# bootphon/abnet3

Measured on AMD Instinct MI355X. Metric: frame-pairs/sec (Siamese train step: fwd both towers + coscos2 + bwd + Adadelta), higher is better.
Workload: dtype f16x2; 1 GPU; C2: SiameseNetwork 40->500x2->100 sigmoid, coscos2(avg=False), Adadelta(0.1), 4096 frame pairs per GPU per step, 40-d N(0,1) frames; pairs_per_gpu=4096, global_pairs=4096, parallelism=dp1, graph_replay=False, dp_gradient_buckets=1

## Files before the change

### abnet3_amd/_lib.py

```python
import ctypes as C
import os

import torch

HERE = os.path.dirname(os.path.abspath(__file__))
LIB_PATH = os.environ.get('ABNET3_HIP_LIB') or os.path.join(HERE, 'lib', 'libabnet3_hip.so')
ABI_VERSION = 20
MAX_LAYERS = 16

ACT = {'none': 0, None: 0, 'sigmoid': 1, 'relu': 2, 'tanh': 3}
LOSS = {'coscos2': 0, 'cosmargin': 1, 'KLLoss': 2}
ACT_SOFTMAX = 4
PRECISION = {'fp32': 0, 'bf16': 1, 'bf16x3': 2, 'f16x2': 3}
OPT = {'sgd': 0, 'adadelta': 1, 'adam': 2, 'adagrad': 3, 'RMSprop': 4}
Y_DTYPE = {torch.int8: 0, torch.int32: 1, torch.int64: 2, torch.float32: 3,
           torch.float64: 4}

_i64, _i32, _f32, _vp = C.c_int64, C.c_int32, C.c_float, C.c_void_p
SYMBOLS = {
    'abn_abi_version': (C.c_int, []),
    'abn_last_error': (C.c_char_p, []),
    'abn_tower_ws_floats': (_i64, [_vp, _i64, _i64]),
    'abn_tower_out_offset': (_i64, [_vp, _i64, _i64]),
    'abn_tower_bwd_scratch_floats': (_i64, [_vp, _i64]),
    'abn_tower_forward': (C.c_int, [_vp, _vp, _vp, _i64, _i64, C.c_int, _vp, _vp]),
    'abn_tower_backward': (C.c_int, [_vp, _vp, _vp, _vp, _i64, _i64, _vp, _vp,
                                      _i64, _vp, _vp]),
    'abn_tower_wpack_floats': (_i64, [_vp]),
    'abn_tower_uses_planes': (C.c_int, [_vp, _i64, _vp, _vp, _vp, C.c_int]),
    'abn_tower_path': (C.c_int, [_vp, _vp, _vp, _i64, _i64, C.c_int, _vp, C.c_int, _vp]),
    'abn_tower_image_offset': (_i64, [_vp, _i64, _i64, C.c_int, C.c_int]),
    'abn_reload_switches': (None, []),
    'abn_rccl_allreduce_f64': (C.c_int, [_vp, _vp, _i64, _vp]),
    'abn_tower_backward_launch': (C.c_int, [_vp, _vp, _vp, _vp, _i64, _i64, _vp, _vp, _i64, C.c_int, _vp]),
    'abn_tower_backward_loss_ws_bytes': (_i64, [_i64]),
    'abn_tower_backward_loss': (C.c_int, [_vp, _vp, _vp, _vp, C.c_int, C.c_int, _f32, C.c_int, _i64, _vp, _vp, _i64, _vp, _vp, _vp, _vp, _vp]),
    'abn_tower_reduce_step': (C.c_int, [_vp, _i64, _vp, _i64, C.c_int, _vp, _vp, _vp, _vp, _i64, _f32, _f32, _f32,
                                         _f32, _i64, _f32, _vp]),
    'abn_linear_forward': (C.c_int, [_vp, _vp, _vp, _i64, _i64, _i64, C.c_int, _vp, _vp]),
    'abn_linear_dgrad': (C.c_int, [_vp, _vp, _i64, _i64, _i64, _vp, C.c_int, _vp, _vp]),
    'abn_linear_wgrad_scratch_floats': (_i64, [_i64, _i64, _i64]),
    'abn_linear_wgrad': (C.c_int, [_vp, _vp, _i64, _i64, _i64, _vp, _vp, _vp, _i64, _vp]),
    'abn_linear_backward': (C.c_int, [_vp, _vp, _vp, _i64, _i64, _i64, C.c_int, _vp, _vp, _vp, _vp, _i64, _vp]),
    'abn_linear_backward_prec': (C.c_int, [_vp, _vp, _vp, _i64, _i64, _i64, C.c_int, C.c_int, _vp, _vp, _vp, _vp, _i64, _vp]),
    'abn_softmax_rows': (C.c_int, [_vp, _i64, _i64, _vp, _vp]),
    'abn_softmax_rows_backward': (C.c_int, [_vp, _vp, _i64, _i64, _vp, _vp]),
    'abn_pair_loss_ws_bytes': (_i64, [_i64]),
    'abn_pair_loss': (C.c_int, [_vp, _vp, _vp, C.c_int, _i64, _i64, C.c_int,
                                 _f32, C.c_int, _vp, _vp, _vp, _vp, _vp]),
    'abn_pair_loss_padded': (C.c_int, [_vp, _vp, _vp, C.c_int, _i64, _i64, C.c_int, _f32, C.c_int, _vp, _vp, _vp, _vp, _vp, _vp, _vp]),
    'abn_pair_loss_dz': (C.c_int, [_vp, _vp, _vp, C.c_int, _i64, _i64, C.c_int, _f32, C.c_int, C.c_int,
                                    _vp, _vp, _vp, _vp, _vp, _vp, _vp]),
    'abn_optimizer_step': (C.c_int, [C.c_int, _vp, _vp, _vp, _vp, _i64, _f32,
                                      _f32, _f32, _f32, _i64, _f32, _vp]),
    'abn_tower_sync_ws_bytes': (_i64, []),
    'abn_oneshot_mail_bytes': (_i64, [_i32, _i64]),
    'abn_allreduce_oneshot': (C.c_int, [_vp, _vp, _i64, _vp]),
    'abn_dtw_ws_bytes': (_i64, [_vp, _vp, _i64, _i64, _i64]),
    'abn_dtw_host_stage_bytes': (_i64, [_vp, _vp, _i64]),
    'abn_dtw_batched': (C.c_int, [_vp, _i64, _vp, _i64, _vp, _vp, _vp, _vp, _i64,
                                   _i64, _vp, _vp, _vp, _i64, _vp, _vp, _i64, _vp,
                                   _i64, _vp]),
    'abn_dtw_batched_overlap': (C.c_int, [_vp, _i64, _vp, _i64, _vp, _vp, _vp, _vp, _i64,
                                           _i64, _vp, _vp, _vp, _i64, _vp, _vp, _i64, _vp,
                                           _i64, _vp, _vp]),
    'abn_dtw_cost_max_n2': (_i64, []),
    'abn_dtw_cost_batched': (C.c_int, [_vp, _i64, _vp, _i64, _vp, _vp, _vp, _vp, _i64, _i64, _vp, _vp, _vp]),
    'abn_kl_tables': (C.c_int, [_vp, _i64, _i64, _f32, _vp, _vp, _vp, _vp]),
    'abn_dtw_cost_kl_batched': (C.c_int, [_vp, _vp, _i64, _vp, _vp, _i64, _vp, _vp, _vp, _vp, _i64, _i64, _vp, _vp, _vp, _vp,
                                           _vp]),
    'abn_abx_score': (C.c_int, [_vp, _i64, _vp, _vp, _vp, _vp, _vp, _i64, _i64, _vp, _vp, _vp, _vp]),
    'abn_cosine_distance': (C.c_int, [_vp, _i64, _vp, _i64, _i64, _vp, _vp, _vp]),
    'abn_cosine_distance_f64': (C.c_int, [_vp, _i64, _vp, _i64, _i64, _vp, _vp, _vp]),
    'abn_arccos_f32': (C.c_int, [_vp, _i64, C.c_int, _vp, _vp]),
    'abn_gather_rows': (C.c_int, [_vp, _vp, _i64, _i64, _vp, _vp]),
    'abn_gather_pairs': (C.c_int, [_vp, _i64, _i64, _vp, _vp, _i64, _i64, _i64, _vp, _i32, _vp, _vp, _vp, _vp]),
    'abn_stack_frames': (C.c_int, [_vp, _i64, _i64, _i32, _vp, _vp]),
    'abn_stack_frames_batched': (C.c_int, [_vp, _vp, _i64, _i64, _i64, _i32, _vp, _vp]),
    'abn_mvn_ws_bytes': (_i64, [_i64, _i64]),
    'abn_mvn_stats': (C.c_int, [_vp, _i64, _i64, C.c_int, _vp, _vp, _vp, _vp]),
    'abn_mvn_apply': (C.c_int, [_vp, _i64, _i64, _vp, _vp, C.c_int, _f32, _vp, _vp]),
    'abn_fbank': (C.c_int, [_vp, C.c_int, _i64, _i32, C.c_double, _i32, _i32,
                             _f32, _vp, _vp, _vp, _i64, _vp, _vp]),
    'abn_fbank_batched': (C.c_int, [_vp, C.c_int, _vp, _vp, _i64, _i32, C.c_double, _i32, _i32,
                                     _f32, _vp, _vp, _vp, _i64, _vp, _vp]),
    'abn_deltas': (C.c_int, [_vp, _i64, _i64, _vp, _vp]),
    'abn_deltas_batched': (C.c_int, [_vp, _i64, _vp, _i64, _i64, _i64, _vp, _i64, _vp]),
    'abn_mfcc': (C.c_int, [_vp, C.c_int, _i64, _i32, C.c_double, _i32, _i32, _i32, _f32, _vp, _vp, _vp, _vp,
                            _i64, _vp, _i64, _vp]),
    'abn_mfcc_batched': (C.c_int, [_vp, C.c_int, _vp, _vp, _i64, _i32, C.c_double, _i32, _i32, _i32, _f32, _vp, _vp,
                                    _vp, _vp, _i64, _vp, _i64, _vp]),
    'abn_mfcc_path': (C.c_int, [_i32, _i32, _i32]),
    'abn_integrate_ws_bytes': (_i64, [_i64]),
    'abn_integrate_forward': (C.c_int, [_vp, _i64, _vp, _i64, _i64, C.c_int, C.c_int, _f32, _f32, _vp, _vp, _vp, _i64,
                                         C.c_int, _vp, _vp, _vp]),
    'abn_integrate_backward': (C.c_int, [_vp, _i64, _vp, _i64, _i64, C.c_int, C.c_int, _f32, _f32, _vp, _vp, _i64,
                                          C.c_int, _vp, _vp, _vp, _vp, _vp, _vp, _vp]),
    'abn_knn_ws_bytes': (_i64, [_i64, _i64, C.c_int]),
    'abn_knn_topk': (C.c_int, [_vp, _i64, _vp, _i64, C.c_int, _vp, _vp, C.c_int, _vp, _vp, _vp, _i64, _vp]),
    'abn_segment_vectors': (C.c_int, [_vp, _i64, _vp, _vp, _i64, C.c_int, _vp, _vp, _vp]),
}
INTEGRATE_MODE = {'sum': 0, 'concat': 1}
W_NONE, W_FIXED, W_SCALAR, W_ATTENTION = range(4)


class TowerDesc(C.Structure):
    _fields_ = [('n_layers', _i32), ('act', _i32), ('last_act', _i32),
                ('batch_norm', _i32), ('dims', _i64 * (MAX_LAYERS + 1))] + [
        (name, _vp * MAX_LAYERS)
        for name in ('W', 'b', 'bn_w', 'bn_b', 'bn_rm', 'bn_rv', 'dW', 'db',
                     'dbn_w', 'dbn_b', 'drop_mask')] + [('precision', _i32), ('d_out_is_dz', _i32), ('defer_reduce', _i32), ('wpack_valid', _i32), ('forward_only', _i32), ('wgrad_part', _i32), ('wpack', _vp), ('drop_seed', _vp), ('drop_p', _f32), ('reserved2_', _i32),
                     ('bn_sync_world', _i32), ('wgrad_split', _i32), ('bn_sync_fn', _vp), ('bn_sync_ctx', _vp), ('n_valid', _vp),
                     ('bn_nbt', _vp * MAX_LAYERS), ('sync_ws', _vp), ('fwd_ws', _vp), ('fwd_calls', _i64), ('source', _vp)]


class StepSource(C.Structure):
    _fields_ = [('table', _vp), ('table_rows', _i64), ('idx1', _vp), ('idx2', _vp), ('labels', _vp), ('steps', _vp), ('step_ctr', _vp)]


class OneShotCtx(C.Structure):
    _fields_ = [('rank', _i32), ('world', _i32), ('mail', _vp * 8), ('cap_floats', _i64)]


class RcclCtx(C.Structure):
    _fields_ = [('comm', _vp), ('all_reduce', _vp), ('calls', _i64)]


ALLREDUCE_FN = C.CFUNCTYPE(C.c_int, C.c_void_p, C.c_void_p, C.c_int64, C.c_void_p)


class HipLibraryError(RuntimeError):
    pass


_lib = None


def load():
    global _lib
    if _lib is not None:
        return _lib
    if not os.path.exists(LIB_PATH):
        raise HipLibraryError(
            'abnet3_amd: %s is missing. Build it with `python -m abnet3_amd.build` '
            '(hipcc, gfx950). There is no CPU fallback.' % LIB_PATH)
    lib = C.CDLL(LIB_PATH)
    for name, (res, args) in SYMBOLS.items():
        try:
            fn = getattr(lib, name)
        except AttributeError:
            raise HipLibraryError('abnet3_amd: %s does not export %s '
                                  '(stale build?)' % (LIB_PATH, name))
        fn.restype = res
        fn.argtypes = args
    if lib.abn_abi_version() != ABI_VERSION:
        raise HipLibraryError('abnet3_amd: ABI version mismatch (library %d, '
                              'binding %d)' % (lib.abn_abi_version(), ABI_VERSION))
    _lib = lib
    return lib


def reload_switches():
    load().abn_reload_switches()


E_ARG = -1
E_WORKSPACE = -3
E_UNSUPPORTED = -4

PATH_PER_LAYER, PATH_FUSED_F32, PATH_PLANES, PATH_PLANES_INFER, PATH_PLANES_INFER_BN, PATH_BN_LAYERS, PATH_WIDE, PATH_BN_TOWER = range(8)
PRECISION_NAMES = {0: 'fp32', 1: 'bf16', 2: 'bf16x3', 3: 'f16x2'}
MFCC_GENERAL, MFCC_WAVE512 = 0, 1

trace_paths = False
last_path = {'forward': -1, 'backward': -1, 'forward_precision': -1, 'backward_precision': -1}


def note_path(desc, x1, x2, rows, n_calls, train, ws, backward):
    if not trace_paths:
        return
    prec = C.c_int32(-1)
    path = load().abn_tower_path(C.byref(desc), ptr(x1), ptr(x2), rows, n_calls, int(train), ptr(ws), int(backward),
                                 C.byref(prec))
    key = 'backward' if backward else 'forward'
    last_path[key] = path
    last_path[key + '_precision'] = prec.value


def last_forward_path():
    return last_path['forward']


def last_backward_path():
    return last_path['backward']


_ON_ERROR = []


def check(rc, what):
    if rc != 0:
        for hook in _ON_ERROR:
            hook()
        msg = load().abn_last_error()
        raise HipLibraryError('%s failed (%d): %s' % (
            what, rc, msg.decode('utf-8', 'replace') if msg else ''))


def require_device(*tensors):
    for t in tensors:
        if t is None:
            continue
        if not t.is_cuda:
            raise HipLibraryError(
                'abnet3_amd: expected a tensor on the MI355X (HIP) device, got '
                'device=%s. The accelerated path has no CPU fallback; move the '
                'module and its inputs to the GPU (.cuda()).' % t.device)
        if not t.is_contiguous():
            raise HipLibraryError('abnet3_amd: tensor must be contiguous')


def ptr(t):
    return C.c_void_p(t.data_ptr()) if t is not None else C.c_void_p(0)


def stream():
    return C.c_void_p(torch.cuda.current_stream().cuda_stream)
```

### abnet3_amd/csrc/tower.hip

```cpp
#include <stdarg.h>
#include <stdlib.h>
#include <string.h>

#include <math.h>
#include <atomic>

#include "common.h"
#include "gemm_f32.h"
#include "opt_rule.h"
#include "tower_fused.h"
#include "tower_planes.h"
#include "tower_bn_persist.h"
#include "tower_wide.h"
#include "tower_wgrad_step.h"

namespace abn {

static thread_local char g_err[512] = "";
void set_error(const char* fmt, ...)
{
    va_list ap;
    va_start(ap, fmt);
    vsnprintf(g_err, sizeof(g_err), fmt, ap);
    va_end(ap);
}

static Switches read_switches()
{
    auto off = [](const char* name) { const char* v = getenv(name); return v && atoi(v) == 0; };
    Switches s;
    s.planes = !off("ABN_PLANES");
    s.fused = !off("ABN_FUSED");
    s.fused_min_rows = getenv("ABN_FUSED_MIN_ROWS") ? atoll(getenv("ABN_FUSED_MIN_ROWS")) : -1;
    s.bn_planes = !off("ABN_BN_PLANES");
    s.bn_persist = !off("ABN_BN_PERSIST");
    s.wgrad_xcd = !off("ABN_WGRAD_XCD");
    s.bf16x3_planes = !off("ABN_BF16X3_PLANES");
    s.bwd_pair = !off("ABN_BWD_PAIR");
    s.gemm_tile = getenv("ABN_GEMM_TILE") ? atoi(getenv("ABN_GEMM_TILE")) : -1;
    s.wgrad_rows_per_slab = getenv("ABN_WGRAD_ROWS_PER_SLAB") ? atoll(getenv("ABN_WGRAD_ROWS_PER_SLAB")) : -1;
    s.wide = !off("ABN_WIDE");
    s.wide_max_rows = getenv("ABN_WIDE_MAX_ROWS") ? atoll(getenv("ABN_WIDE_MAX_ROWS")) : -1;
    s.wide_max_groups = getenv("ABN_WIDE_MAXG") ? atoi(getenv("ABN_WIDE_MAXG")) : WD_MAXG;
    if (s.wide_max_groups < 1 || s.wide_max_groups > WD_MAXG) s.wide_max_groups = WD_MAXG;
    s.dtw_f40 = !off("ABN_DTW_F40");
    s.dtw_pc = !off("ABN_DTW_PC");
    s.wgrad_wgs_heavy = getenv("ABN_WGRAD_WGS_HEAVY") ? atoi(getenv("ABN_WGRAD_WGS_HEAVY")) : 128;
    s.wgrad_wgs_light = getenv("ABN_WGRAD_WGS_LIGHT") ? atoi(getenv("ABN_WGRAD_WGS_LIGHT")) : 128;
    s.wgrad_tile128 = getenv("ABN_WGRAD_TILE128") ? atoi(getenv("ABN_WGRAD_TILE128")) : -1;
    s.dtw_wgs_per_cu = getenv("ABN_DTW_WGS") ? atoi(getenv("ABN_DTW_WGS")) : 6;
    if (s.dtw_wgs_per_cu < 1 || s.dtw_wgs_per_cu > 9) s.dtw_wgs_per_cu = 6;
    s.wgrad_step = !off("ABN_WGRAD_STEP");
    s.dtw_dealt = !off("ABN_DTW_SCHED");
    s.oneshot_wgs = getenv("ABN_ONESHOT_WGS") ? atoi(getenv("ABN_ONESHOT_WGS")) : 32;
    if (s.oneshot_wgs < 1 || s.oneshot_wgs > 256) s.oneshot_wgs = 32;
    s.knn_split = getenv("ABN_KNN_SPLIT") ? atoi(getenv("ABN_KNN_SPLIT")) : 0;
    if (s.knn_split < 0) s.knn_split = 0;
    return s;
}
static Switches g_switches = read_switches();
const Switches& switches() { return g_switches; }
void reload_switches() { g_switches = read_switches(); }

template <int BM, int BN, bool A_KC, bool B_KC, int EPI, bool VEC, int BF16>
static void launch_one(const GemmP& p, int splits, hipStream_t st)
{
    const int tiles = ((p.M + BM - 1) / BM) * ((p.N + BN - 1) / BN);
    constexpr size_t lds = BF16 == 3 ? gemm_lds_bytes3<BM, BN>() : gemm_lds_bytes<BM, BN, A_KC, B_KC>();
    auto k = gemm_f32_kernel<BM, BN, A_KC, B_KC, EPI, VEC, BF16>;
    static bool attr_set[16] = {};
    int dev = 0;
    (void)hipGetDevice(&dev);
    dev = (dev >= 0 && dev < 16) ? dev : 0;
    if (!attr_set[dev]) {
        (void)hipFuncSetAttribute(reinterpret_cast<const void*>(k),
                                  hipFuncAttributeMaxDynamicSharedMemorySize, (int)lds);
        attr_set[dev] = true;
    }
    GemmP q = p;
    q.splits = splits;
    hipLaunchKernelGGL(k, dim3(tiles * splits), dim3(256), lds, st, q);
}

template <int BM, int BN, bool A_KC, bool B_KC, int EPI>
static void launch_cfg(const GemmP& p, int splits, hipStream_t st)
{
    if (p.bf16 == 1) {
        if (p.a_vec && p.b_vec) launch_one<BM, BN, A_KC, B_KC, EPI, true, 1>(p, splits, st);
        else launch_one<BM, BN, A_KC, B_KC, EPI, false, 1>(p, splits, st);
        return;
    }
    if (p.bf16 == 2) {
        const bool planes = switches().bf16x3_planes;
        if (p.a_vec && p.b_vec && planes) launch_one<BM, BN, A_KC, B_KC, EPI, true, 3>(p, splits, st);
        else if (p.a_vec && p.b_vec) launch_one<BM, BN, A_KC, B_KC, EPI, true, 2>(p, splits, st);
        else launch_one<BM, BN, A_KC, B_KC, EPI, false, 2>(p, splits, st);
        return;
    }
    if (p.a_vec && p.b_vec) launch_one<BM, BN, A_KC, B_KC, EPI, true, 0>(p, splits, st);
    else launch_one<BM, BN, A_KC, B_KC, EPI, false, 0>(p, splits, st);
}

template <bool A_KC, bool B_KC, int EPI>
static int prepare_gemm(GemmP& p, int splits)
{
    if (p.M <= 0 || p.N <= 0) return -1;
    if (p.K <= 0) { set_error("gemm: empty reduction"); return -100 + ABN_E_ARG; }
    {
        const int64_t span_a = (int64_t)(A_KC ? p.M : p.K) * p.lda, span_b = (int64_t)(B_KC ? p.N : p.K) * p.ldb;
        if (span_a >= (1LL << 31) || span_b >= (1LL << 31)) { set_error("gemm: operand larger than 2^31 floats"); return -100 + ABN_E_ARG; }
    }
    auto tiles = [&](int bm, int bn) {
        return (int64_t)((p.M + bm - 1) / bm) * ((p.N + bn - 1) / bn) * splits;
    };
    const int64_t want = 2 * 256;
    {
        const bool slab_ok = (EPI != EPI_WGRAD) || (p.slab_stride % 4 == 0);
        p.c_vec = aligned16(p.C) && (p.ldc % 4 == 0) && slab_ok && (!p.bias || aligned16(p.bias)) &&
                  (!p.aux || (aligned16(p.aux) && p.ldaux % 4 == 0)) &&
                  (!p.mask || (aligned16(p.mask) && (EPI == EPI_DGRAD ? p.ldaux : p.ldc) % 4 == 0));
    }
    p.splits = splits;
#ifdef ABN_STAMPS
    p.stamps = getenv("ABN_STAMP_BUF") ? (unsigned long long*)strtoull(getenv("ABN_STAMP_BUF"), nullptr, 0) : nullptr;
#endif
    const int force = switches().gemm_tile;
    if (force >= 0 && force <= 3) return force;
    const int64_t pad_a = (int64_t)((p.M + 127) / 128 * 128) * ((p.N + 63) / 64 * 64);
    const int64_t pad_b = (int64_t)((p.M + 63) / 64 * 64) * ((p.N + 127) / 128 * 128);
    if (p.M > 64 && p.N > 64 && tiles(128, 128) >= want) return 0;
    if (p.M > 64 && tiles(128, 64) >= want && (pad_a <= pad_b || !(p.N > 64 && tiles(64, 128) >= want))) return 1;
    if (p.N > 64 && tiles(64, 128) >= want) return 2;
    return 3;
}

template <bool A_KC, bool B_KC, int EPI>
static int launch_gemm(GemmP p, int splits, hipStream_t st)
{
    const int tile = prepare_gemm<A_KC, B_KC, EPI>(p, splits);
    if (tile == -1) return ABN_OK;
    if (tile < -1) return tile + 100;
    if (tile == 0) launch_cfg<128, 128, A_KC, B_KC, EPI>(p, splits, st);
    else if (tile == 1) launch_cfg<128, 64, A_KC, B_KC, EPI>(p, splits, st);
    else if (tile == 2) launch_cfg<64, 128, A_KC, B_KC, EPI>(p, splits, st);
    else launch_cfg<64, 64, A_KC, B_KC, EPI>(p, splits, st);
    ABN_CHECK_LAUNCH("gemm_f32");
    return ABN_OK;
}

static bool bf16x3_planes()
{
    return switches().bf16x3_planes;
}

template <int WM, int WN, int BF16>
static void launch_pair_one(const GemmP& pw, int n0, const GemmP& pd, int n1, hipStream_t st)
{
    constexpr size_t lw = BF16 == 3 ? gemm_lds_bytes3<WM, WN>() : gemm_lds_bytes<WM, WN, false, false>();
    constexpr size_t ld = BF16 == 3 ? gemm_lds_bytes3<128, 64>() : gemm_lds_bytes<128, 64, true, false>();
    constexpr size_t lds = lw > ld ? lw : ld;
    auto k = gemm_bwd_pair_kernel<WM, WN, BF16>;
    static bool attr_set[16] = {};
    int dev = 0;
    (void)hipGetDevice(&dev);
// ... 1043 lines not shown
{
    const int nl = t->n_layers;
    const int np = planes_of(t);
    const int64_t rpc = rows / n_calls;
    ABN_REQUIRE(aligned16(d_out) && aligned16(scratch) && (!dx || aligned16(dx)), "tower_backward: d_out / scratch / dx must be 16-byte aligned");
    ABN_REQUIRE(!t->d_out_is_dz || loss, "tower_backward: d_out_is_dz cannot be combined with batch_norm");
    ABN_REQUIRE(!loss || n_calls == 2, "tower_backward_loss: two forward_once calls");
    BwdLayout B = B0;
    for (int l = 0; l < nl; ++l) B.splits[l] = B0.psplits[l];
    const PackLayout PL = make_pack_layout(t);
    const char* const image = t->wpack ? reinterpret_cast<const char*>(t->wpack) : reinterpret_cast<const char*>(ws + L.wpack);
    static bool attr_set[16] = {};
    int dev = 0;
    (void)hipGetDevice(&dev);
    dev = (dev >= 0 && dev < 16) ? dev : 0;
    if (!attr_set[dev]) {
        PL_LDS_ATTR(bn_bwd_layer_kernel, pl_lds_bytes);
        PL_LDS_ATTR(wgrad_planes_kernel, wgrad_lds_of);
        attr_set[dev] = true;
    }
    const int wgs_per_call = (int)bn_wgs_per_call(rows, n_calls);
    const dim3 cgrid((unsigned)(n_calls * wgs_per_call));
    const int64_t tp_steps = 2 * n_calls * wgs_per_call;
    float* const part = scratch + B.bn_wg;
    float* const s1 = scratch + B.bn_s1, * const s2 = scratch + B.bn_s2;
    const bool sync = bn_sync_on(t);
    ABN_REQUIRE(!sync || t->bn_sync_fn, "tower_backward: bn_sync_world = %d without bn_sync_fn", t->bn_sync_world);
    ABN_REQUIRE(!loss || !loss->n_valid || !t->n_valid || loss->n_valid == t->n_valid, "tower_backward_loss: two different n_valid");
    const int32_t* const nvp = t->n_valid ? t->n_valid : (loss ? loss->n_valid : nullptr);
    if (sync && nvp) { set_error("tower_backward: n_valid (a padded batch) cannot be combined with cross-replica BatchNorm statistics"); return ABN_E_UNSUPPORTED; }
    double* const sums = reinterpret_cast<double*>(scratch + B.bn_part);
    auto finish_sums = [&](int C, float* dgamma, float* dbeta) -> int {
        hipLaunchKernelGGL(bn_bwd_finish_wg_kernel, dim3((unsigned)((C + 63) / 64)), dim3(64 * BN_WG_GROUPS), 0, st, part, wgs_per_call, C,
                           (int)n_calls, s1, s2, dgamma, dbeta, sync ? sums : static_cast<double*>(nullptr));
        if (!sync) return ABN_OK;
        if (t->bn_sync_fn(t->bn_sync_ctx, sums, n_calls * 2 * C, st) != 0) { set_error("tower_backward: bn_sync_fn failed"); return ABN_E_LAUNCH; }
        hipLaunchKernelGGL(bn_bwd_from_sums_kernel, dim3(grid_for(n_calls * C)), dim3(256), 0, st, sums, C, (int)n_calls, s1, s2);
        return ABN_OK;
    };
    if (bn_persist_path(t, rows, n_calls)) {
        static bool bt_attr_set[16] = {};
        if (!bt_attr_set[dev]) {
            PL_LDS_ATTR(bn_bwd_tower_kernel, bnp_lds_bytes);
            bt_attr_set[dev] = true;
        }
        BnBwdTowerP q = {};
        q.n_layers = nl; q.rows = (int)rows; q.rows_call = (int)rpc; q.n_calls = (int)n_calls;
        for (int l = 0; l <= nl; ++l) q.dims[l] = (int)t->dims[l];
        for (int l = 0; l < nl; ++l) {
            q.act[l] = (l == nl - 1) ? t->last_act : t->act;
            q.z[l] = ws + L.xhat[l];
            q.mean[l] = ws + L.mean[l]; q.invstd[l] = ws + L.invstd[l];
            q.gamma[l] = t->bn_w[l]; q.beta[l] = t->bn_b[l];
            q.dgamma[l] = t->dbn_w[l]; q.dbeta[l] = t->dbn_b[l];
            q.mask[l] = t->drop_mask[l];
            q.wpt[l] = image + PL.wpt[l];
            q.dzp[l] = reinterpret_cast<char*>(scratch + B.dzp[l]);
            q.amax_dz[l] = B.amax_dz[l] >= 0 ? scratch + B.amax_dz[l] : nullptr;
        }
        q.drop_seed = reinterpret_cast<const unsigned long long*>(t->drop_seed);
        q.drop_p = t->drop_p;
        q.wbase = image; q.wbytes = PL.bytes;
        q.tp_steps = tp_steps;
        q.dx = dx;
        q.d_out = loss ? nullptr : d_out;
        q.a_top = ws + L.a[nl - 1];
        q.sync_ws = t->sync_ws;
        q.sync_bytes = bnp_sync_bytes(BNP_MAX_WGS);
        q.n_valid = nvp;
        q.n_stat = (float)rpc;
        q.loss_kind = -1;
        if (loss) {
            q.loss_kind = loss->kind; q.y = loss->y; q.y_dtype = loss->y_dtype;
            q.margin = (double)loss->margin;
            q.scale = loss->avg ? 1.0 / (double)rpc : 1.0;
            q.loss_counter = reinterpret_cast<unsigned*>(loss->ws);
            q.loss_partial = reinterpret_cast<double*>(reinterpret_cast<char*>(loss->ws) + 8);
            q.loss_out = loss->loss_out;
            q.loss_accum = loss->loss_accum;
        }
        PL_LAUNCH(np, bn_bwd_tower_kernel, cgrid, dim3(PL_NT), bnp_lds_bytes(np), st, q);
    } else {
    const float* da_top = d_out;
    {
        const int N = (int)t->dims[nl];
        BnLossP lp = {};
        lp.n_valid = nvp;
        if (loss) {
            lp.y = loss->y; lp.y_dtype = loss->y_dtype; lp.kind = loss->kind; lp.B = (int)rpc;
            lp.margin = (double)loss->margin;
            lp.scale = loss->avg ? 1.0 / (double)rpc : 1.0;
            lp.loss_counter = reinterpret_cast<unsigned*>(loss->ws);
            lp.loss_partial = reinterpret_cast<double*>(reinterpret_cast<char*>(loss->ws) + 8);
            lp.loss_out = loss->loss_out;
            lp.loss_accum = loss->loss_accum;
            lp.a_top = ws + L.a[nl - 1];
            lp.da_out = scratch + B.dz[0];
            da_top = lp.da_out;
            hipLaunchKernelGGL(bn_bwd_sums_wg_kernel<true>, cgrid, dim3(512), 0, st, static_cast<const float*>(nullptr), ws + L.xhat[nl - 1],
                               ws + L.mean[nl - 1], ws + L.invstd[nl - 1], t->bn_w[nl - 1], t->bn_b[nl - 1], t->last_act, N, rpc, part, lp);
        } else {
            hipLaunchKernelGGL(bn_bwd_sums_wg_kernel<false>, cgrid, dim3(512), 0, st, d_out, ws + L.xhat[nl - 1], ws + L.mean[nl - 1],
                               ws + L.invstd[nl - 1], t->bn_w[nl - 1], t->bn_b[nl - 1], t->last_act, N, rpc, part, lp);
        }
        const int rc = finish_sums(N, t->dbn_w[nl - 1], t->dbn_b[nl - 1]);
        if (rc != ABN_OK) return rc;
    }
    int cur = 0;
    for (int l = nl - 1; l >= 0; --l) {
        BnBwdP q = {};
        q.l = l; q.rows = (int)rows; q.rows_call = (int)rpc;
        q.n_stat = (float)rpc;
        q.n_stat_dev = sync ? ws + L.bn_nstat + 8 * l : nullptr;
        q.N = (int)t->dims[l + 1]; q.K = (int)t->dims[l];
        q.act_l = (l == nl - 1) ? t->last_act : t->act;
        q.act_prev = t->act;
        q.da = (l == nl - 1) ? da_top : scratch + B.dz[cur];
        q.z = ws + L.xhat[l];
        q.mean = ws + L.mean[l];
        q.invstd = ws + L.invstd[l];
        q.gamma = t->bn_w[l]; q.beta = t->bn_b[l];
        q.s1 = s1; q.s2 = s2;
        q.mask = t->drop_mask[l];
        q.drop_seed = reinterpret_cast<const unsigned long long*>(t->drop_seed);
        q.drop_p = t->drop_p;
        q.dzp = reinterpret_cast<char*>(scratch + B.dzp[l]);
        q.amax_dz = B.amax_dz[l] >= 0 ? scratch + B.amax_dz[l] : nullptr;
        q.tp_steps = tp_steps;
        q.wpt = (l >= 1 || dx) ? image + PL.wpt[l] : nullptr;
        q.da_prev = l >= 1 ? scratch + B.dz[cur ^ 1] : dx;
        if (l >= 1) { q.z_prev = ws + L.xhat[l - 1]; q.mean_prev = ws + L.mean[l - 1]; q.invstd_prev = ws + L.invstd[l - 1];
                      q.gamma_prev = t->bn_w[l - 1]; q.beta_prev = t->bn_b[l - 1]; q.part_out = part; }
        q.n_valid = nvp;
        PL_LAUNCH(np, bn_bwd_layer_kernel, cgrid, dim3(PL_NT), pl_lds_bytes(np), st, q);
        if (l >= 1) {
            const int rc = finish_sums(q.K, t->dbn_w[l - 1], t->dbn_b[l - 1]);
            if (rc != ABN_OK) return rc;
            cur ^= 1;
        }
    }
    }
    int n_wg = 0;
    WgradP w = make_wgrad(t, rows, L, B, ws, scratch, &n_wg);
    w.tp_steps = tp_steps;
    launch_wgrad(np, w, n_wg, st);
    ABN_CHECK_LAUNCH("tower_backward (BatchNorm, planes)");
    if (t->defer_reduce) return ABN_OK;
    const ReduceTable rt = make_reduce_table(t, B);
    hipLaunchKernelGGL(slab_reduce_kernel, dim3(grid_for((rt.total + 3) / 4)), dim3(256), 0, st, scratch + B.slabs, rt);
    ABN_CHECK_LAUNCH("slab_reduce");
    return ABN_OK;
}

enum { PLANES_BWD_ALL = 0, PLANES_BWD_DGRAD = 1, PLANES_BWD_WGRAD = 2 };
static int planes_backward(const abn_tower_desc* t, const float* d_out, const LossArgs* loss, int64_t rows, const Layout& L,
                           const BwdLayout& B, const float* ws, float* scratch, float* dx, hipStream_t st, int part = PLANES_BWD_ALL)
{
    const int nl = t->n_layers;
    const int np = planes_of(t);
    PlanesBwdP b = {};
#ifdef ABN_STAMPS
    b.stamps = getenv("ABN_DSTAMP_BUF") ? (unsigned long long*)strtoull(getenv("ABN_DSTAMP_BUF"), nullptr, 0) : nullptr;
#endif
    b.n_layers = nl;
    b.rows = (int)rows;
    b.d_out = d_out;
    b.d_out_is_dz = t->d_out_is_dz;
    b.tp_steps = pl_row_steps(rows);
    ABN_REQUIRE((loss || t->wgrad_part == 2 || aligned16(d_out)) && aligned16(scratch) && (!dx || aligned16(dx)),
                "tower_backward: d_out / scratch / dx must be 16-byte aligned");
    b.loss_kind = -1;
    b.B = (int)rows;
    if (loss) {
        b.loss_kind = loss->kind;
        b.y = loss->y; b.y_dtype = loss->y_dtype;
        b.B = (int)(rows / 2);
        b.margin = (double)loss->margin;
        b.scale = loss->avg ? 1.0 / (double)(rows / 2) : 1.0;
        b.loss_counter = reinterpret_cast<unsigned*>(loss->ws);
        b.loss_partial = reinterpret_cast<double*>(reinterpret_cast<char*>(loss->ws) + 8);
        b.loss_out = loss->loss_out;
        b.n_valid = loss->n_valid;
        b.loss_accum = loss->loss_accum;
    }
    b.a_top = ws + L.a[nl - 1];
    b.dx = dx;
    b.drop_seed = reinterpret_cast<const unsigned long long*>(t->drop_seed);
    b.drop_p = t->drop_p;
    const PackLayout PL = make_pack_layout(t);
    const char* const image = t->wpack ? reinterpret_cast<const char*>(t->wpack) : reinterpret_cast<const char*>(ws + L.wpack);
    for (int l = 0; l <= nl; ++l) b.dims[l] = (int)t->dims[l];
    for (int l = 0; l < nl; ++l) {
        b.act[l] = (l == nl - 1) ? t->last_act : t->act;
        b.tp[l] = reinterpret_cast<const char*>(ws + L.tp[l]);
        b.mask[l] = t->drop_mask[l];
        b.wpt[l] = image + PL.wpt[l];
        b.dzp[l] = reinterpret_cast<char*>(scratch + B.dzp[l]);
        b.amax_dz[l] = B.amax_dz[l] >= 0 ? scratch + B.amax_dz[l] : nullptr;
    }
    b.wbase = image; b.wbytes = PL.bytes;
    int l_first, l_end;
    { const int rc = wgrad_range(t, &l_first, &l_end); if (rc != ABN_OK) return rc; }
    if (t->wgrad_part == 2) part = PLANES_BWD_WGRAD;
    int n_wg = 0;
    const WgradP w = make_wgrad(t, rows, L, B, ws, scratch, &n_wg, l_first, l_end);
    static bool bw_attr_set[16] = {};
    int dev = 0;
    (void)hipGetDevice(&dev);
    dev = (dev >= 0 && dev < 16) ? dev : 0;
    if (!bw_attr_set[dev]) {
        PL_LDS_ATTR(tower_dgrad_planes_kernel, pl_lds_bytes);
        PL_LDS_ATTR(wgrad_planes_kernel, wgrad_lds_of);
        bw_attr_set[dev] = true;
    }
    const dim3 cgrid((unsigned)((rows + PL_ROWS - 1) / PL_ROWS));
    const bool do_dgrad = part != PLANES_BWD_WGRAD, do_wgrad = part != PLANES_BWD_DGRAD;
    if (do_dgrad) PL_LAUNCH(np, tower_dgrad_planes_kernel, cgrid, dim3(PL_NT), pl_lds_bytes(np), st, b);
    if (do_wgrad && n_wg > 0) launch_wgrad(np, w, n_wg, st);
    ABN_CHECK_LAUNCH("tower_backward (planes)");
    if (t->defer_reduce) return ABN_OK;
    ReduceTable rt = make_reduce_table(t, B);
    reduce_range(rt, t, B, l_first, l_end);
    if (rt.total > rt.begin)
        hipLaunchKernelGGL(slab_reduce_kernel, dim3(grid_for((rt.total - rt.begin + 3) / 4)), dim3(256), 0, st, scratch + B.slabs, rt);
    ABN_CHECK_LAUNCH("slab_reduce");
    return ABN_OK;
}

static bool wgrad_step_small_ok(const abn_tower_desc* t, int64_t rows, int64_t n_calls)
{
    if (!switches().wgrad_step || !t->defer_reduce || !t->fwd_ws || t->batch_norm || t->wgrad_part != 0 || planes_of(t) != 2) return false;
    if (n_calls < 1 || rows % n_calls != 0 || !aligned16(t->fwd_ws)) return false;
    const int64_t vrows = bn_vrows(rows, n_calls);
    if (wide_groups_for(t, vrows) <= 0 || !planes_shape_ok(t)) return false;
    return vrows <= 2048;
}

static int wide_backward(const abn_tower_desc* t, const float* d_out, const LossArgs* loss, int64_t rows, int64_t n_calls,
                         const Layout& L, const BwdLayout& B, const float* ws, float* scratch, float* dx, hipStream_t st)
{
    const int nl = t->n_layers, top = nl - 1;
    const int np = planes_of(t);
    ABN_REQUIRE((loss || t->wgrad_part == 2 || aligned16(d_out)) && aligned16(scratch) && (!dx || aligned16(dx)),
                "tower_backward: d_out / scratch / dx must be 16-byte aligned");
    ABN_REQUIRE(!loss || n_calls == 2, "tower_backward_loss: two forward_once calls");
    const PackLayout PL = make_pack_layout(t);
    const char* const image = t->wpack ? reinterpret_cast<const char*>(t->wpack) : reinterpret_cast<const char*>(ws + L.wpack);
    static bool attr_set[16] = {};
    int dev = 0;
    (void)hipGetDevice(&dev);
    dev = (dev >= 0 && dev < 16) ? dev : 0;
    if (!attr_set[dev]) {
        PL_LDS_ATTR(wide_dgrad_layer_kernel, wd_lds_bytes);
        PL_LDS_ATTR(wgrad_planes_kernel, wgrad_lds_of);
        attr_set[dev] = true;
    }
    const int64_t rpc = rows / n_calls;
    const int64_t wpc = bn_wgs_per_call(rows, n_calls), nrb = n_calls * wpc;
    const int G = wide_groups_for(t, nrb * PL_ROWS);
    ABN_REQUIRE(G > 0, "tower_backward: too many rows for the layer-per-launch kernels");
    int l_first, l_end;
    { const int rc = wgrad_range(t, &l_first, &l_end); if (rc != ABN_OK) return rc; }
    const int last = dx ? 0 : 1;
    int cur = 0;
    for (int l = top; (l >= last || l == top) && t->wgrad_part != 2; --l) {
        WideBwdP q = {};
        q.l = l; q.top = top;
        q.N = (int)t->dims[l + 1]; q.K = (int)t->dims[l];
        q.act_prev = t->act;
        q.rows_call = (int)rpc; q.n_calls = (int)n_calls; q.wpc = (int)wpc;
        const int nblk = pl_blocks(q.K);
        q.G = G < nblk ? G : nblk;
        q.dz_in = l < top ? scratch + B.dz[cur] : nullptr;
        q.wpt = (l >= 1 || dx) ? image + PL.wpt[l] : nullptr;
        q.a_prev = l >= 1 ? ws + L.a[l - 1] : nullptr;
        q.dz_out = (l >= 1 && l - 1 >= last) ? scratch + B.dz[cur ^ 1] : nullptr;
        q.dzp_top = reinterpret_cast<char*>(scratch + B.dzp[top]);
        q.dzp_out = l >= 1 ? reinterpret_cast<char*>(scratch + B.dzp[l - 1]) : nullptr;
        if (np == 2) { q.amax_top = scratch + B.amax_dz[top]; q.amax_out = l >= 1 ? scratch + B.amax_dz[l - 1] : nullptr; }
        q.tp_steps = 2 * nrb;
        q.dx = dx;
        q.drop_seed = reinterpret_cast<const unsigned long long*>(t->drop_seed);
        q.drop_p = t->drop_p;
        if (l == top) {
            q.d_out = loss ? nullptr : d_out;
            q.d_out_is_dz = t->d_out_is_dz;
            q.a_top = ws + L.a[top];
            q.act_top = t->last_act;
            if (loss) {
                q.loss_kind = loss->kind; q.y_dtype = loss->y_dtype; q.y = loss->y;
                q.margin = (double)loss->margin;
                q.scale = loss->avg ? 1.0 / (double)rpc : 1.0;
                q.loss_counter = reinterpret_cast<unsigned*>(loss->ws);
                q.loss_partial = reinterpret_cast<double*>(reinterpret_cast<char*>(loss->ws) + 8);
                q.loss_out = loss->loss_out;
                q.n_valid = loss->n_valid;
                q.loss_accum = loss->loss_accum;
                if (t->source) {
                    q.y = t->source->labels;
                    q.g_steps = t->source->steps; q.g_ctr = t->source->step_ctr;
                }
            }
        }
        const dim3 grid((unsigned)(nrb * q.G));
        PL_LAUNCH(np, wide_dgrad_layer_kernel, grid, dim3(PL_NT), wd_lds_bytes(np), st, q);
        if (l < top || q.dz_out) cur ^= (q.dz_out ? 1 : 0);
        if (l == 0) break;
    }
    if (wgrad_step_small_ok(t, rows, n_calls)) {
        ABN_REQUIRE(t->fwd_ws == ws && t->fwd_calls == n_calls, "tower_backward: abn_tower_desc.fwd_ws / fwd_calls are not this call's");
        ABN_CHECK_LAUNCH("tower_backward (layer per launch)");
        return ABN_OK;
    }
    int n_wg = 0;
    WgradP w = make_wgrad(t, rows, L, B, ws, scratch, &n_wg, l_first, l_end);
    w.tp_steps = 2 * nrb;
    if (n_wg > 0) launch_wgrad(np, w, n_wg, st);
    ABN_CHECK_LAUNCH("tower_backward (layer per launch)");
    if (t->defer_reduce) return ABN_OK;
    ReduceTable rt = make_reduce_table(t, B);
    reduce_range(rt, t, B, l_first, l_end);
    if (rt.total > rt.begin)
        hipLaunchKernelGGL(slab_reduce_kernel, dim3(grid_for((rt.total - rt.begin + 3) / 4)), dim3(256), 0, st, scratch + B.slabs, rt);
    ABN_CHECK_LAUNCH("slab_reduce");
    return ABN_OK;
}

}

using namespace abn;

extern "C" {

int abn_abi_version(void) { return ABN_ABI_VERSION; }
const char* abn_last_error(void) { return abn::g_err; }

int64_t abn_tower_ws_floats(const abn_tower_desc* t, int64_t rows, int64_t n_calls)
{
    if (check_desc(t, rows, n_calls) != ABN_OK) return -1;
    return make_layout(t, rows, n_calls).total;
}

int64_t abn_tower_out_offset(const abn_tower_desc* t, int64_t rows, int64_t n_calls)
{
    if (check_desc(t, rows, n_calls) != ABN_OK) return -1;
    return make_layout(t, rows, n_calls).a[t->n_layers - 1];
}

int64_t abn_tower_image_offset(const abn_tower_desc* t, int64_t rows, int64_t n_calls, int which, int l)
{
    if (check_desc(t, rows, n_calls) != ABN_OK || l < 0 || l >= t->n_layers) return -1;
    if (which == 3) return make_bwd_layout(t, rows).dzp[l];
    const Layout L = make_layout(t, rows, n_calls);
    if (which == 2) return L.tp[l];
    if (which == 4) return L.xhat[l];
    if (which == 5) return L.a[l];
    if (which != 0 && which != 1) return -1;
    const PackLayout P = make_pack_layout(t);
    return (t->wpack ? 0 : L.wpack) + (which == 0 ? P.wp[l] : P.wpt[l]) / 4;
}

static bool fused_f32_ok(const abn_tower_desc* t, const float* x1, const float* x2, int64_t rows, int train, const float* ws)
{
    const int64_t fused_min_rows = switches().fused_min_rows >= 0 ? switches().fused_min_rows : 6144;
    bool fusable = switches().fused && rows >= fused_min_rows && !t->batch_norm && aligned16(x1) && (!x2 || aligned16(x2)) &&
                   aligned16(ws);
    for (int l = 0; l <= t->n_layers && fusable; ++l)
        fusable = t->dims[l] >= 4 && t->dims[l] <= FUSED_MAXW && t->dims[l] % 4 == 0;
    for (int l = 0; l < t->n_layers && fusable; ++l)
        fusable = aligned16(t->W[l]) && (!t->drop_mask[l] || !train || aligned16(t->drop_mask[l]));
    return fusable;
}
static int forward_path(const abn_tower_desc* t, const float* x1, const float* x2, int64_t rows, int64_t n_calls, int train,
                        const float* ws)
{
    const bool bn_train = train && bn_train_planes_path(t, rows, n_calls, x1, x2, ws);
    const int kind = planes_kind(t, rows, n_calls, x1, x2, ws, train ? PLANES_TRAIN : PLANES_EVAL_FORWARD);
    if (!bn_train && kind == PLANES_WIDE) return ABN_PATH_WIDE;
    if (bn_train) return bn_persist_path(t, rows, n_calls) ? ABN_PATH_BN_TOWER : ABN_PATH_BN_LAYERS;
    if (kind != PLANES_NONE) {
        if (t->batch_norm) return ABN_PATH_PLANES_INFER_BN;
        return (t->forward_only && !(train && t->drop_seed) && !train) ? ABN_PATH_PLANES_INFER : ABN_PATH_PLANES;
    }
    return fused_f32_ok(t, x1, x2, rows, train, ws) ? ABN_PATH_FUSED_F32 : ABN_PATH_PER_LAYER;
}
static int backward_path(const abn_tower_desc* t, const float* x1, const float* x2, int64_t rows, int64_t n_calls, const float* ws)
{
    const int kind = planes_kind(t, rows, n_calls, x1, x2, ws);
    if (kind == PLANES_WIDE) return ABN_PATH_WIDE;
    if (kind == PLANES_CHAIN) return ABN_PATH_PLANES;
    if (bn_train_planes_path(t, rows, n_calls, x1, x2, ws)) return bn_persist_path(t, rows, n_calls) ? ABN_PATH_BN_TOWER : ABN_PATH_BN_LAYERS;
    return ABN_PATH_PER_LAYER;
}

int abn_tower_path(const abn_tower_desc* t, const float* x1, const float* x2, int64_t rows, int64_t n_calls, int train,
                   const float* ws, int backward, int32_t* precision_out)
{
    if (check_desc(t, rows, n_calls) != ABN_OK) return -1;
    const int path = backward ? backward_path(t, x1, x2, rows, n_calls, ws) : forward_path(t, x1, x2, rows, n_calls, train, ws);
    if (precision_out) *precision_out = (path == ABN_PATH_PER_LAYER || path == ABN_PATH_FUSED_F32) ? gemm_prec(t->precision) : t->precision;
    return path;
}

int abn_tower_uses_planes(const abn_tower_desc* t, int64_t rows, const float* x1, const float* x2, const float* ws, int train)
{
    if (check_desc(t, rows, 1) != ABN_OK) return -1;
    if (train && t->batch_norm) return bn_train_planes_path(t, rows, 1, x1, x2, ws) ? 1 : 0;
    return planes_path(t, rows, x1, x2, ws, train ? PLANES_TRAIN : PLANES_EVAL_FORWARD) ? 1 : 0;
}

int64_t abn_tower_sync_ws_bytes(void) { return bnp_sync_bytes(BNP_MAX_WGS); }

int64_t abn_tower_wpack_floats(const abn_tower_desc* t)
{
    if (check_desc(t, 0, 1) != ABN_OK) return -1;
    return make_pack_layout(t).bytes / 4;
}

int64_t abn_tower_bwd_scratch_floats(const abn_tower_desc* t, int64_t rows)
{
    if (check_desc(t, rows, 1) != ABN_OK) return -1;
    return make_bwd_layout(t, rows).total;
}

int abn_tower_forward(const abn_tower_desc* t, const float* x1, const float* x2, int64_t rows,
                      int64_t n_calls, int train, float* ws, void* stream)
{
    int rc = check_desc(t, rows, n_calls);
    if (rc != ABN_OK) return rc;
    ABN_REQUIRE(x1 && ws, "tower_forward: null input/workspace");
    ABN_REQUIRE(x2 == nullptr || n_calls == 2, "tower_forward: x2 given but n_calls=%lld", (long long)n_calls);
    ABN_REQUIRE(n_calls <= 8, "tower_forward: at most 8 calls per launch");
    if (rows == 0) return ABN_OK;
    hipStream_t st = (hipStream_t)stream;
    const Layout L = make_layout(t, rows, n_calls);
    const int64_t rpc = rows / n_calls;

    const int path = forward_path(t, x1, x2, rows, n_calls, train, ws);
    const bool fusable = path == ABN_PATH_FUSED_F32;
    const int pmode = train ? PLANES_TRAIN : PLANES_EVAL_FORWARD;
    const bool bn_train = train && bn_train_planes_path(t, rows, n_calls, x1, x2, ws);
    if (train && t->batch_norm && bn_sync_on(t) && !bn_train) {
        set_error("tower_forward: cross-replica BatchNorm statistics (bn_sync_world) need the operand-plane launches");
        return ABN_E_UNSUPPORTED;
    }
    if (train && t->batch_norm && t->n_valid && !bn_train) {
        set_error("tower_forward: a padded batch (n_valid) through a BatchNorm tower in training needs the BatchNorm layer launches");
        return ABN_E_UNSUPPORTED;
    }
    const int kind = planes_kind(t, rows, n_calls, x1, x2, ws, pmode);
    if (t->source && !(train && !bn_train && kind == PLANES_WIDE && n_calls == 2 && x2 && !t->forward_only)) {
        set_error("tower_forward: a step source (abn_tower_desc.source) needs the layer-per-launch kernels in training, two calls");
        return ABN_E_UNSUPPORTED;
    }
    if (t->source) ABN_REQUIRE(t->source->table && t->source->idx1 && t->source->idx2 && t->source->steps && t->source->step_ctr &&
                                   aligned16(t->source->table) && t->dims[0] % 4 == 0,
                               "tower_forward: abn_step_source: null or misaligned array");
    if (t->drop_seed && train && !bn_train && kind == PLANES_NONE) {
        for (int l = 0; l < t->n_layers; ++l)
            if (!t->drop_mask[l]) { set_error("tower_forward: in-kernel dropout (drop_seed) needs the operand-plane kernels: pass drop_mask tensors"); return ABN_E_UNSUPPORTED; }
    }
    if (bn_train || kind != PLANES_NONE) {
        const int np = planes_of(t);
        PackTable pk = {};
        PlanesFwdP f = {};
        f.n_layers = t->n_layers;
        f.rows = (int)rows;
        f.rows_call = (int)rpc;
        f.x1 = x1; f.x2 = x2;
        f.x_copy = nullptr;
        const PackLayout PL = make_pack_layout(t);
        char* const image = t->wpack ? reinterpret_cast<char*>(t->wpack) : reinterpret_cast<char*>(ws + L.wpack);
        const bool repack = !(t->wpack && t->wpack_valid);
        ABN_REQUIRE(aligned16(image), "tower_forward: wpack must be 16-byte aligned");
        pk.base = image;
        f.wbase = image; f.wbytes = PL.bytes;
        for (int l = 0; l <= t->n_layers; ++l) f.dims[l] = (int)t->dims[l];
        for (int l = 0; l < t->n_layers; ++l) {
            f.act[l] = (l == t->n_layers - 1) ? t->last_act : t->act;
            f.b[l] = t->b[l];
            f.mask[l] = train ? t->drop_mask[l] : nullptr;
            f.out[l] = l == t->n_layers - 1 ? ws + L.a[l] : nullptr;
            f.wp[l] = image + PL.wp[l];
            PackJob& J = pk.job[pk.n_jobs++];
            J.W = t->W[l]; J.N = (int)t->dims[l + 1]; J.K = (int)t->dims[l]; J.transposed = 0;
            J.nblk = pl_blocks(J.N); J.nsteps = pl_steps(J.K);
            J.tile0 = pk.n_tiles; J.dst = PL.wp[l];
            J.blk0 = pk.n_blocks;
            pk.n_tiles += J.nblk * J.nsteps;
            pk.n_blocks += J.nblk;
            {
                PackJob& T = pk.job[pk.n_jobs++];
                T.W = t->W[l]; T.N = J.N; T.K = J.K; T.transposed = 1;
                T.nblk = pl_blocks(T.K); T.nsteps = pl_steps(T.N);
                T.tile0 = pk.n_tiles; T.dst = PL.wpt[l];
                T.blk0 = pk.n_blocks;
                pk.n_tiles += T.nblk * T.nsteps;
                pk.n_blocks += T.nblk;
            }
            f.tp[l] = (t->forward_only || t->batch_norm) ? nullptr : reinterpret_cast<char*>(ws + L.tp[l]);
            f.amax[l] = f.tp[l] && L.amax[l] >= 0 ? ws + L.amax[l] : nullptr;
            if (t->batch_norm) { f.bn_rm[l] = t->bn_rm[l]; f.bn_rv[l] = t->bn_rv[l]; f.bn_w[l] = t->bn_w[l]; f.bn_b[l] = t->bn_b[l]; }
        }
        f.tp_steps = pl_row_steps(rows);
        f.drop_seed = train ? reinterpret_cast<const unsigned long long*>(t->drop_seed) : nullptr;
        f.drop_p = t->drop_p;
        f.bn_eps = BN_EPS;
#ifdef ABN_STAMPS
        f.stamps = getenv("ABN_STAMP_BUF") ? (unsigned long long*)strtoull(getenv("ABN_STAMP_BUF"), nullptr, 0) : nullptr;
#endif
        static bool pl_attr_set[16] = {};
        int dev = 0;
        (void)hipGetDevice(&dev);
        dev = (dev >= 0 && dev < 16) ? dev : 0;
        const dim3 pgrid((unsigned)((pk.n_tiles + 3) / 4));
        const dim3 fgrid((unsigned)((rows + PL_ROWS - 1) / PL_ROWS));
        if (repack) {
            if (np == 3) hipLaunchKernelGGL(pack_planes_kernel<3>, pgrid, dim3(256), 0, st, pk);
            else if (np == 2) hipLaunchKernelGGL(pack_planes_scaled_kernel, dim3((unsigned)pk.n_blocks), dim3(PL_NT), 0, st, pk);
            else hipLaunchKernelGGL(pack_planes_kernel<1>, pgrid, dim3(256), 0, st, pk);
        }
        if (!bn_train && kind == PLANES_WIDE) {
            static bool wd_attr_set[16] = {};
            if (!wd_attr_set[dev]) {
                PL_LDS_ATTR(wide_fwd_layer_kernel, wd_lds_bytes);
                wd_attr_set[dev] = true;
            }
            const int nl = t->n_layers;
            const int64_t wpc = bn_wgs_per_call(rows, n_calls), nrb = n_calls * wpc;
            const int G = wide_groups_for(t, nrb * PL_ROWS);
            const bool keep = !t->forward_only;
            for (int l = 0; l < nl; ++l) {
                WideFwdP q = {};
                q.l = l; q.last = l == nl - 1;
                q.K = (int)t->dims[l]; q.N = (int)t->dims[l + 1];
                q.act = f.act[l];
                q.rows_call = (int)rpc; q.n_calls = (int)n_calls; q.wpc = (int)wpc;
                const int nblk = pl_blocks(q.N);
                q.G = G < nblk ? G : nblk;
                q.x1 = x1; q.x2 = x2;
                q.a_prev = l >= 1 ? ws + L.a[l - 1] : nullptr;
                q.wp = f.wp[l];
                q.b = t->b[l];
                q.a_out = q.last ? nullptr : ws + L.a[l];
                q.out = q.last ? ws + L.a[l] : nullptr;
                q.tp_in = keep && l == 0 ? reinterpret_cast<char*>(ws + L.tp[0]) : nullptr;
                q.tp_out = keep && !q.last ? reinterpret_cast<char*>(ws + L.tp[l + 1]) : nullptr;
                if (np == 2 && keep) { q.amax_in = ws + L.amax[0]; q.amax_out = q.last ? nullptr : ws + L.amax[l + 1]; }
                q.tp_steps = 2 * nrb;
                q.drop_seed = f.drop_seed; q.drop_p = f.drop_p;
                if (t->source && l == 0) {
                    q.g_table = t->source->table; q.g_rows = t->source->table_rows;
                    q.g_idx1 = t->source->idx1; q.g_idx2 = t->source->idx2;
                    q.g_steps = t->source->steps; q.g_ctr = t->source->step_ctr;
                }
#ifdef ABN_STAMPS
                q.stamps = getenv("ABN_STAMP_BUF") ? (unsigned long long*)strtoull(getenv("ABN_STAMP_BUF"), nullptr, 0) : nullptr;
#endif
                const dim3 wgrid((unsigned)(nrb * q.G));
                PL_LAUNCH(np, wide_fwd_layer_kernel, wgrid, dim3(PL_NT), wd_lds_bytes(np), st, q);
            }
            ABN_CHECK_LAUNCH("tower_forward (layer per launch)");
            return ABN_OK;
        }
        if (bn_train) {
            static bool bn_attr_set[16] = {};
            if (!bn_attr_set[dev]) {
                PL_LDS_ATTR(bn_fwd_layer_kernel, pl_lds_bytes);
                bn_attr_set[dev] = true;
            }
            f.bn_part = ws + L.bn_wg;
            const int nl = t->n_layers;
            const int64_t wpc = bn_wgs_per_call(rows, n_calls);
            const dim3 bgrid((unsigned)(n_calls * wpc));
            f.tp_steps = 2 * n_calls * wpc;
            if (bn_persist_path(t, rows, n_calls)) {
                static bool bt_attr_set[16] = {};
                if (!bt_attr_set[dev]) {
                    PL_LDS_ATTR(bn_fwd_tower_kernel, bnp_lds_bytes);
                    bt_attr_set[dev] = true;
                }
                PlanesFwdP fl = f;
                BnPersistP q = {};
                for (int l = 0; l < nl; ++l) {
                    fl.tp[l] = reinterpret_cast<char*>(ws + L.tp[l]);
                    fl.amax[l] = L.amax[l] >= 0 ? ws + L.amax[l] : nullptr;
                    fl.out[l] = nullptr;
                    q.z[l] = ws + L.xhat[l];
                    q.mean[l] = ws + L.mean[l]; q.invstd[l] = ws + L.invstd[l]; q.var[l] = ws + L.var[l];
                    q.rm[l] = t->bn_rm[l]; q.rv[l] = t->bn_rv[l];
                    q.nbt[l] = reinterpret_cast<long long*>(t->bn_nbt[l]);
                }
                q.sync_ws = t->sync_ws;
                q.sync_bytes = bnp_sync_bytes(BNP_MAX_WGS);
                q.n_valid = t->n_valid;
                q.n_calls = (int)n_calls;
                q.a_top = ws + L.a[nl - 1];
                PL_LAUNCH(np, bn_fwd_tower_kernel, bgrid, dim3(PL_NT), bnp_lds_bytes(np), st, fl, q);
                ABN_CHECK_LAUNCH("tower_forward (BatchNorm, resident tower)");
                return ABN_OK;
            }
            for (int l = 0; l < nl; ++l) {
                PlanesFwdP fl = f;
                for (int i = 0; i < nl; ++i) { fl.tp[i] = nullptr; fl.out[i] = nullptr; }
                fl.tp[l] = reinterpret_cast<char*>(ws + L.tp[l]);
                fl.amax[l] = L.amax[l] >= 0 ? ws + L.amax[l] : nullptr;
                fl.act[l] = ACT_NONE;
                fl.out[l] = ws + L.xhat[l];
                BnTrainP q = {};
                q.l = l;
                if (l > 0) { q.mean = ws + L.mean[l - 1]; q.invstd = ws + L.invstd[l - 1]; q.z_prev = ws + L.xhat[l - 1]; q.a_prev = nullptr; }
                q.n_valid = t->n_valid;
                PL_LAUNCH(np, bn_fwd_layer_kernel, bgrid, dim3(PL_NT), pl_lds_bytes(np), st, fl, q);
                const int N = (int)t->dims[l + 1];
                const bool sync = bn_sync_on(t);
                ABN_REQUIRE(!sync || t->bn_sync_fn, "tower_forward: bn_sync_world = %d without bn_sync_fn", t->bn_sync_world);
                if (sync && t->n_valid) { set_error("tower_forward: n_valid (a padded batch) cannot be combined with cross-replica BatchNorm statistics"); return ABN_E_UNSUPPORTED; }
                double* const sums = reinterpret_cast<double*>(ws + L.bn_part);
                hipLaunchKernelGGL(bn_stats_finish_wg_kernel, dim3((unsigned)((N + 63) / 64)), dim3(64 * BN_WG_GROUPS), 0, st, ws + L.bn_wg,
                                   (int)wpc, rpc, N, (int)n_calls, ws + L.mean[l], ws + L.invstd[l], ws + L.var[l],
                                   t->bn_rm[l], t->bn_rv[l], sync ? sums : static_cast<double*>(nullptr), t->n_valid);
                if (sync) {
                    if (t->bn_sync_fn(t->bn_sync_ctx, sums, n_calls * 2 * N + n_calls, st) != 0) { set_error("tower_forward: bn_sync_fn failed"); return ABN_E_LAUNCH; }
                    hipLaunchKernelGGL(bn_stats_from_sums_kernel, dim3((unsigned)((N + 255) / 256)), dim3(256), 0, st, sums,
                                       N, (int)n_calls, ws + L.mean[l], ws + L.invstd[l], ws + L.var[l],
                                       t->bn_rm[l], t->bn_rv[l], ws + L.bn_nstat + 8 * l);
                }
            }
            const int N = (int)t->dims[nl];
            const float* z = ws + L.xhat[nl - 1];
            hipLaunchKernelGGL(bn_apply_kernel, dim3(grid_for(rows * N)), dim3(256), 0, st, z, rows, rpc, N, ws + L.mean[nl - 1],
                               ws + L.invstd[nl - 1], t->bn_rm[nl - 1], t->bn_rv[nl - 1], 1, t->bn_w[nl - 1], t->bn_b[nl - 1],
                               t->last_act, static_cast<float*>(nullptr), ws + L.a[nl - 1], t->n_valid);
            launch_nbt(t, n_calls, st);
            ABN_CHECK_LAUNCH("tower_forward (BatchNorm, planes)");
            return ABN_OK;
        }
        const bool infer = t->batch_norm || (t->forward_only && !f.drop_seed && !train);
        const int mode = t->batch_norm ? PL_INFER_BN : infer ? PL_INFER : PL_TRAIN;
        const size_t lds = t->batch_norm ? pl_lds_bytes_bn(np) : pl_lds_bytes_stag(np);
        const void* kernels[3][3] = {
            {reinterpret_cast<const void*>(tower_fwd_planes_kernel<1, PL_TRAIN>), reinterpret_cast<const void*>(tower_fwd_planes_kernel<1, PL_INFER>),
             reinterpret_cast<const void*>(tower_fwd_planes_kernel<1, PL_INFER_BN>)},
            {reinterpret_cast<const void*>(tower_fwd_planes_kernel<2, PL_TRAIN>), reinterpret_cast<const void*>(tower_fwd_planes_kernel<2, PL_INFER>),
             reinterpret_cast<const void*>(tower_fwd_planes_kernel<2, PL_INFER_BN>)},
            {reinterpret_cast<const void*>(tower_fwd_planes_kernel<3, PL_TRAIN>), reinterpret_cast<const void*>(tower_fwd_planes_kernel<3, PL_INFER>),
             reinterpret_cast<const void*>(tower_fwd_planes_kernel<3, PL_INFER_BN>)}};
        if (!pl_attr_set[dev]) {
            for (int a = 0; a < 3; ++a)
                for (int m = 0; m < 3; ++m)
                    if (kernels[a][m])
                        (void)hipFuncSetAttribute(kernels[a][m], hipFuncAttributeMaxDynamicSharedMemorySize,
                                                  (int)(m == PL_INFER_BN ? pl_lds_bytes_bn(a + 1) : pl_lds_bytes_stag(a + 1)));
            pl_attr_set[dev] = true;
        }
        void* kargs[] = {&f};
        (void)hipLaunchKernel(kernels[np - 1][mode], fgrid, dim3(PL_NT), kargs, lds, st);
        ABN_CHECK_LAUNCH("tower_fwd_planes");
        return ABN_OK;
    }
    if (fusable) {
        FusedFwdP f = {};
        f.n_layers = t->n_layers;
        f.rows = (int)rows;
        f.rows_call = (int)rpc;
        f.bf16 = gemm_prec(t->precision);
        f.x1 = x1; f.x2 = x2;
        f.x_copy = x2 ? ws + L.x : nullptr;
        for (int l = 0; l <= t->n_layers; ++l) f.dims[l] = (int)t->dims[l];
        for (int l = 0; l < t->n_layers; ++l) {
            f.act[l] = (l == t->n_layers - 1) ? t->last_act : t->act;
            f.W[l] = t->W[l]; f.b[l] = t->b[l];
            f.mask[l] = train ? t->drop_mask[l] : nullptr;
            f.out[l] = ws + L.a[l];
// ... 125 lines not shown
        const int N = (int)t->dims[nl];
        const float* a = ws + L.a[nl - 1];
        float* dz = scratch + B.dz[cur];
        if (t->d_out_is_dz) {
            ABN_REQUIRE(!t->batch_norm, "tower_backward: d_out_is_dz cannot be combined with batch_norm");
            dz_in = d_out;
        } else if (!t->batch_norm) {
            hipLaunchKernelGGL(act_bwd_kernel, dim3(grid_for(rows * N)), dim3(256), 0, st, a, d_out,
                               t->drop_mask[nl - 1], dz, rows * N, t->last_act);
        } else {
            const int nch = bn_chunks(rpc);
            double* part = reinterpret_cast<double*>(scratch + B.bn_part);
            hipLaunchKernelGGL(bn_partial_kernel<true>, dim3((N + 63) / 64, nch, (int)n_calls), dim3(256), 0, st, d_out, a,
                               ws + L.xhat[nl - 1], rpc, N, bn_chunk_rows(rpc), t->last_act, part);
            hipLaunchKernelGGL(bn_bwd_finish_kernel, dim3((unsigned)((n_calls * N + 63) / 64)), dim3(64), 0, st, part,
                               nch, N, (int)n_calls, scratch + B.bn_s1, scratch + B.bn_s2);
            hipLaunchKernelGGL(bn_bwd_apply_kernel, dim3(grid_for(rows * N)), dim3(256), 0, st, a, d_out,
                               ws + L.xhat[nl - 1], rows, rpc, N, t->last_act, t->bn_w[nl - 1],
                               ws + L.invstd[nl - 1], scratch + B.bn_s1, scratch + B.bn_s2, (int)n_calls,
                               t->drop_mask[nl - 1], dz, t->dbn_w[nl - 1], t->dbn_b[nl - 1]);
        }
        ABN_CHECK_LAUNCH("output-layer dz");
    }

    float* slabs = scratch + B.slabs;
    for (int l = nl - 1; l >= 0; --l) {
        const int Kin = (int)t->dims[l], Nout = (int)t->dims[l + 1];
        const float* dz = (l == nl - 1 && dz_in) ? dz_in : scratch + B.dz[cur];
        const float* a_in = (l == 0) ? xin : ws + L.a[l - 1];
        GemmP pw = {};
        pw.A = dz; pw.lda = Nout;
        pw.B = a_in; pw.ldb = Kin;
        pw.C = slabs + B.off[l]; pw.ldc = Kin;
        pw.C2 = slabs + B.off[l] + (int64_t)Nout * Kin;
        pw.slab_stride = B.slab_stride;
        pw.M = Nout; pw.N = Kin + 1; pw.K = (int)rows;
        pw.k_chunk = (int)align_up((rows + B.splits[l] - 1) / B.splits[l], BK);
        pw.ones_col = Kin;
        pw.bf16 = gemm_prec(t->precision);
        pw.a_vec = aligned16(dz) && (Nout % 4 == 0);
        pw.b_vec = aligned16(a_in) && (Kin % 4 == 0);
        if (!(l > 0 || dx)) {
            rc = launch_gemm<false, false, EPI_WGRAD>(pw, B.splits[l], st);
            if (rc != ABN_OK) return rc;
        }
        if (l > 0 || dx) {
            float* dst = (l == 0) ? dx : scratch + B.dz[cur ^ 1];
            GemmP p = {};
            p.A = dz; p.lda = Nout;
            p.B = t->W[l]; p.ldb = Kin;
            p.C = dst; p.ldc = Kin;
            p.M = (int)rows; p.N = Kin; p.K = Nout; p.k_chunk = Nout;
            p.a_vec = aligned16(dz) && (Nout % 4 == 0);
            p.b_vec = aligned16(t->W[l]) && (Kin % 4 == 0);
            p.ones_col = -1;
            p.bf16 = gemm_prec(t->precision);
            if (l > 0 && !t->batch_norm) { p.aux = ws + L.a[l - 1]; p.ldaux = Kin; p.act = t->act; p.mask = t->drop_mask[l - 1]; }
            rc = launch_bwd_pair(pw, B.splits[l], p, st);
            if (rc != ABN_OK) return rc;
            if (l > 0 && t->batch_norm) {
                const float* a = ws + L.a[l - 1];
                const int nch = bn_chunks(rpc);
                double* part = reinterpret_cast<double*>(scratch + B.bn_part);
                hipLaunchKernelGGL(bn_partial_kernel<true>, dim3((Kin + 63) / 64, nch, (int)n_calls), dim3(256), 0, st,
                                   dst, a, ws + L.xhat[l - 1], rpc, Kin, bn_chunk_rows(rpc), t->act, part);
                hipLaunchKernelGGL(bn_bwd_finish_kernel, dim3((unsigned)((n_calls * Kin + 63) / 64)), dim3(64), 0, st,
                                   part, nch, Kin, (int)n_calls, scratch + B.bn_s1, scratch + B.bn_s2);
                hipLaunchKernelGGL(bn_bwd_apply_kernel, dim3(grid_for(rows * Kin)), dim3(256), 0, st, a, dst,
                                   ws + L.xhat[l - 1], rows, rpc, Kin, t->act, t->bn_w[l - 1], ws + L.invstd[l - 1],
                                   scratch + B.bn_s1, scratch + B.bn_s2, (int)n_calls, t->drop_mask[l - 1], dst,
                                   t->dbn_w[l - 1], t->dbn_b[l - 1]);
                ABN_CHECK_LAUNCH("batch_norm backward");
            }
            cur ^= 1;
        }
    }
    if (t->defer_reduce) return ABN_OK;
    const ReduceTable rt = make_reduce_table(t, B);
    hipLaunchKernelGGL(slab_reduce_kernel, dim3(grid_for((rt.total + 3) / 4)), dim3(256), 0, st, slabs, rt);
    ABN_CHECK_LAUNCH("slab_reduce");
    return ABN_OK;
}

int abn_tower_backward_launch(const abn_tower_desc* t, const float* x1, const float* x2, const float* d_out,
                                  int64_t rows, int64_t n_calls, const float* ws, float* scratch,
                                  int64_t scratch_floats, int part, void* stream)
{
    int rc = check_desc(t, rows, n_calls);
    if (rc != ABN_OK) return rc;
    ABN_REQUIRE(x1 && d_out && ws && scratch && (part == PLANES_BWD_DGRAD || part == PLANES_BWD_WGRAD), "tower_backward_launch: bad argument");
    if (rows == 0 || planes_kind(t, rows, n_calls, x1, x2, ws) != PLANES_CHAIN) { set_error("tower_backward_launch: single-launch operand-plane towers only"); return ABN_E_UNSUPPORTED; }
    const Layout L = make_layout(t, rows, n_calls);
    const BwdLayout B = make_bwd_layout(t, rows);
    if (scratch_floats < B.total) { set_error("tower_backward_launch: scratch too small"); return ABN_E_WORKSPACE; }
    abn_tower_desc u = *t;
    u.defer_reduce = 1;
    return planes_backward(&u, d_out, nullptr, rows, L, B, ws, scratch, nullptr, (hipStream_t)stream, part);
}

void abn_reload_switches(void) { abn::reload_switches(); }

int abn_rccl_allreduce_f64(void* ctx, void* device_doubles, int64_t n, void* stream)
{
    typedef int (*all_reduce_t)(const void*, void*, size_t, int, int, void*, hipStream_t);
    abn_rccl_ctx* c = static_cast<abn_rccl_ctx*>(ctx);
    if (!c || !c->comm || !c->all_reduce || !device_doubles || n < 0) { set_error("rccl_allreduce_f64: null context / buffer"); return 1; }
    constexpr int NCCL_FLOAT64 = 8, NCCL_SUM = 0;
    const int rc = reinterpret_cast<all_reduce_t>(c->all_reduce)(device_doubles, device_doubles, (size_t)n, NCCL_FLOAT64, NCCL_SUM, c->comm,
                                                                  (hipStream_t)stream);
    if (rc != 0) { set_error("rccl_allreduce_f64: ncclAllReduce returned %d", rc); return 1; }
    ++c->calls;
    return 0;
}

int64_t abn_tower_backward_loss_ws_bytes(int64_t rows) { return 8 + ((rows + PL_ROWS - 1) / PL_ROWS + 2) * (int64_t)sizeof(double); }

int abn_tower_backward_loss(const abn_tower_desc* t, const float* x1, const float* x2, const void* y, int y_dtype,
                            int loss_kind, float margin, int avg, int64_t rows, const float* ws, float* scratch,
                            int64_t scratch_floats, float* loss_out, void* loss_ws, const int32_t* n_valid, double* loss_accum,
                            void* stream)
{
    if (loss_kind == ABN_LOSS_KL) {
        set_error("tower_backward_loss: ABN_LOSS_KL is not computed inside the backward: use abn_pair_loss_dz + abn_tower_backward");
        return ABN_E_UNSUPPORTED;
    }
    int rc = check_desc(t, rows, 2);
    if (rc != ABN_OK) return rc;
    ABN_REQUIRE(x1 && y && ws && scratch && loss_out && loss_ws, "tower_backward_loss: null pointer");
    ABN_REQUIRE(loss_kind == ABN_LOSS_COSCOS2 || loss_kind == ABN_LOSS_COSMARGIN, "tower_backward_loss: unknown loss kind %d", loss_kind);
    ABN_REQUIRE(y_dtype >= ABN_Y_I8 && y_dtype <= ABN_Y_F64, "tower_backward_loss: unknown label dtype %d", y_dtype);
    ABN_REQUIRE(loss_kind != ABN_LOSS_COSMARGIN || (margin >= 0.0f && margin <= 1.0f), "tower_backward_loss: margin outside [0,1]");
    for (int l = 0; l < t->n_layers; ++l) ABN_REQUIRE(t->dW[l] && t->db[l], "tower_backward_loss: layer %d has null gradient buffers", l);
    const bool bn = rows > 0 && t->batch_norm && bn_train_planes_path(t, rows, 2, x1, x2, ws) && !bn_sync_on(t) && t->wgrad_part == 0 &&
                    t->dims[t->n_layers] % 4 == 0;
    const int kind = rows == 0 || t->batch_norm ? PLANES_NONE : planes_kind(t, rows, 2, x1, x2, ws);
    if (kind == PLANES_NONE && !bn) {
        set_error("tower_backward_loss: only for towers the operand-plane kernels take (the split arithmetics, "
                  "widths <= 512 and multiples of 4, enough rows; BatchNorm without cross-replica statistics): use abn_pair_loss_dz + abn_tower_backward");
        return ABN_E_UNSUPPORTED;
    }
    if (t->source && (kind != PLANES_WIDE || bn || !t->source->labels)) {
        set_error("tower_backward_loss: a step source (abn_tower_desc.source) needs the layer-per-launch kernels and its labels");
        return ABN_E_UNSUPPORTED;
    }
    const Layout L = make_layout(t, rows, 2);
    const BwdLayout B = make_bwd_layout(t, rows);
    if (scratch_floats < B.total) { set_error("tower_backward_loss: scratch too small"); return ABN_E_WORKSPACE; }
    LossArgs la = {y, y_dtype, loss_kind, avg, margin, loss_out, loss_ws, n_valid, loss_accum};
    if (bn) return bn_planes_backward(t, nullptr, &la, rows, 2, L, B, ws, scratch, nullptr, (hipStream_t)stream);
    if (kind == PLANES_WIDE) return wide_backward(t, nullptr, &la, rows, 2, L, B, ws, scratch, nullptr, (hipStream_t)stream);
    return planes_backward(t, nullptr, &la, rows, L, B, ws, scratch, nullptr, (hipStream_t)stream);
}

int abn_tower_reduce_step(const abn_tower_desc* t, int64_t rows, const float* scratch, int64_t scratch_floats, int kind,
                          float* params, float* grads, float* state1, float* state2, int64_t n, float lr, float hp0,
                          float hp1, float eps, int64_t step, float grad_scale, void* stream)
{
    int rc = check_desc(t, rows, 1);
    if (rc != ABN_OK) return rc;
    ABN_REQUIRE(kind >= ABN_OPT_SGD && kind <= ABN_OPT_RMSPROP, "tower_reduce_step: unknown optimizer %d", kind);
    ABN_REQUIRE(scratch && params && grads && state1, "tower_reduce_step: null pointer");
    ABN_REQUIRE(state2 || (kind != ABN_OPT_ADADELTA && kind != ABN_OPT_ADAM), "tower_reduce_step: state2 required");
    ABN_REQUIRE(step >= 1 && n >= 1, "tower_reduce_step: bad n/step");
    const BwdLayout B = make_bwd_layout(t, rows);
    if (scratch_floats < B.total) { set_error("tower_reduce_step: scratch too small"); return ABN_E_WORKSPACE; }
    if (t->defer_reduce && wgrad_step_small_ok(t, rows, t->fwd_calls)) {
        const Layout L = make_layout(t, rows, t->fwd_calls);
        const int64_t nrb = t->fwd_calls * bn_wgs_per_call(rows, t->fwd_calls);
        WgsP w = {};
        w.n_layers = t->n_layers;
        w.tp_steps = (int)(2 * nrb);
        int n_wg = 0;
        for (int l = 0; l < t->n_layers; ++l) {
            WgsLayer& W = w.L[l];
            W.N = (int)t->dims[l + 1]; W.K = (int)t->dims[l];
            W.nblk = pl_blocks(W.N); W.kblk = pl_blocks(W.K + 1);
            ABN_REQUIRE(t->dW[l] && t->db[l] && t->dW[l] >= grads && t->dW[l] + (int64_t)W.N * W.K <= grads + n && t->db[l] >= grads &&
                            t->db[l] + W.N <= grads + n,
                        "tower_reduce_step: layer %d's gradients are not inside the flat buffer", l);
            ABN_REQUIRE(B.amax_dz[l] >= 0 && L.amax[l] >= 0, "tower_reduce_step: the images' maxima are missing");
            W.dzp = reinterpret_cast<const char*>(scratch + B.dzp[l]);
            W.ap = reinterpret_cast<const char*>(t->fwd_ws + L.tp[l]);
            W.amax_dz = scratch + B.amax_dz[l];
            W.amax_a = t->fwd_ws + L.amax[l];
            W.tiles_k = (W.kblk + 1) / 2;
            W.first_wg = n_wg;
            W.w_off = t->dW[l] - grads; W.b_off = t->db[l] - grads;
            n_wg += ((W.nblk + 1) / 2) * W.tiles_k;
        }
        w.n_tiles = n_wg;
        w.per_xcd = (n_wg + 7) / 8;
        n_wg = 8 * w.per_xcd;
        w.o = make_optp(kind, lr, hp0, hp1, eps, step, grad_scale);
        w.params = params; w.grads = grads; w.s1 = state1; w.s2 = state2;
        w.fail_word = nullptr;
        w.step_ctr = t->source ? t->source->step_ctr : nullptr;
        static bool wgs_attr[16] = {};
        int dev = 0;
        (void)hipGetDevice(&dev);
        dev = (dev >= 0 && dev < 16) ? dev : 0;
        if (!wgs_attr[dev]) {
            if (hipFuncSetAttribute(reinterpret_cast<const void*>(wgrad_step_small_kernel), hipFuncAttributeMaxDynamicSharedMemorySize, (int)WGS_LDS_BYTES) != hipSuccess) {
                set_error("tower_reduce_step: cannot reserve %zu bytes of LDS", WGS_LDS_BYTES);
                return ABN_E_LAUNCH;
            }
            wgs_attr[dev] = true;
        }
        hipLaunchKernelGGL(wgrad_step_small_kernel, dim3((unsigned)n_wg), dim3(WGS_NT), WGS_LDS_BYTES, (hipStream_t)stream, w);
        ABN_CHECK_LAUNCH("tower_reduce_step (weight gradients + step)");
        return ABN_OK;
    }
    ReduceTable rt = make_reduce_table(t, B);
    for (int l = 0; l < t->n_layers; ++l) {
        ABN_REQUIRE(t->dW[l] && t->db[l] && t->dW[l] >= grads && t->dW[l] + rt.nW[l] <= grads + n && t->db[l] >= grads &&
                        t->db[l] + rt.nb[l] <= grads + n,
                    "tower_reduce_step: layer %d's gradients are not inside the flat buffer", l);
        if (t->batch_norm) {
            ABN_REQUIRE(t->dbn_w[l] && t->dbn_b[l] && t->dbn_w[l] >= grads && t->dbn_w[l] + rt.nb[l] <= grads + n &&
                            t->dbn_b[l] >= grads && t->dbn_b[l] + rt.nb[l] <= grads + n,
                        "tower_reduce_step: layer %d's BatchNorm gradients are not inside the flat buffer", l);
            rt.extra_off[rt.n_extra] = t->dbn_w[l] - grads; rt.extra_n[rt.n_extra++] = (int32_t)rt.nb[l];
            rt.extra_off[rt.n_extra] = t->dbn_b[l] - grads; rt.extra_n[rt.n_extra++] = (int32_t)rt.nb[l];
        }
    }
    hipLaunchKernelGGL(slab_reduce_step_kernel, dim3(grid_for((rt.total + 3) / 4)), dim3(256), 0, (hipStream_t)stream,
                       scratch + B.slabs, rt, make_optp(kind, lr, hp0, hp1, eps, step, grad_scale), params, grads, state1,
                       state2, t->batch_norm && t->sync_ws ? reinterpret_cast<const unsigned*>(t->sync_ws) + 16 : nullptr,
                       t->source ? t->source->step_ctr : nullptr);
    ABN_CHECK_LAUNCH("tower_reduce_step");
    return ABN_OK;
}


int abn_linear_forward(const float* x, const float* W, const float* b, int64_t rows, int64_t in_dim,
                       int64_t out_dim, int act, float* y, void* stream)
{
    ABN_REQUIRE(x && W && y, "linear_forward: null pointer");
    ABN_REQUIRE(rows >= 0 && rows < (1LL << 30) && in_dim >= 1 && out_dim >= 1 && in_dim < (1 << 24) && out_dim < (1 << 24),
                "linear_forward: bad shape");
    ABN_REQUIRE(act >= ABN_ACT_NONE && act <= ABN_ACT_TANH, "linear_forward: unsupported activation %d", act);
    GemmP p = {};
    p.A = x; p.lda = in_dim;
    p.B = W; p.ldb = in_dim;
    p.C = y; p.ldc = out_dim;
    p.M = (int)rows; p.N = (int)out_dim; p.K = (int)in_dim; p.k_chunk = (int)in_dim;
    p.bias = b; p.act = act; p.ones_col = -1;
    p.a_vec = aligned16(x) && (in_dim % 4 == 0);
    p.b_vec = aligned16(W) && (in_dim % 4 == 0);
    return launch_gemm<true, true, EPI_FWD>(p, 1, (hipStream_t)stream);
}

int abn_linear_dgrad(const float* dz, const float* W, int64_t rows, int64_t in_dim, int64_t out_dim,
                     const float* a_prev, int act_prev, float* dx, void* stream)
{
    ABN_REQUIRE(dz && W && dx, "linear_dgrad: null pointer");
    ABN_REQUIRE(rows >= 0 && rows < (1LL << 30) && in_dim >= 1 && out_dim >= 1 && in_dim < (1 << 24) && out_dim < (1 << 24),
                "linear_dgrad: bad shape");
    ABN_REQUIRE(act_prev >= ABN_ACT_NONE && act_prev <= ABN_ACT_TANH, "linear_dgrad: unsupported activation %d", act_prev);
    GemmP p = {};
    p.A = dz; p.lda = out_dim;
    p.B = W; p.ldb = in_dim;
    p.C = dx; p.ldc = in_dim;
    p.M = (int)rows; p.N = (int)in_dim; p.K = (int)out_dim; p.k_chunk = (int)out_dim;
    p.aux = a_prev; p.ldaux = in_dim; p.act = act_prev; p.ones_col = -1;
    p.a_vec = aligned16(dz) && (out_dim % 4 == 0);
    p.b_vec = aligned16(W) && (in_dim % 4 == 0);
    return launch_gemm<true, false, EPI_DGRAD>(p, 1, (hipStream_t)stream);
}

int64_t abn_linear_wgrad_scratch_floats(int64_t rows, int64_t in_dim, int64_t out_dim)
{
    if (rows < 0 || in_dim < 1 || out_dim < 1) return -1;
    return align_up(out_dim * in_dim + out_dim, 64) * split_count(rows, out_dim, in_dim);
}

int abn_linear_wgrad(const float* dz, const float* a_in, int64_t rows, int64_t in_dim, int64_t out_dim, float* dW,
                     float* db, float* scratch, int64_t scratch_floats, void* stream)
{
    ABN_REQUIRE(dz && a_in && dW && db && scratch, "linear_wgrad: null pointer");
    ABN_REQUIRE(rows >= 1 && rows < (1LL << 30) && in_dim >= 1 && out_dim >= 1 && in_dim < (1 << 24) && out_dim < (1 << 24),
                "linear_wgrad: bad shape");
    const int splits = split_count(rows, out_dim, in_dim);
    const int64_t stride = align_up(out_dim * in_dim + out_dim, 64);
    if (scratch_floats < stride * splits) { set_error("linear_wgrad: scratch too small"); return ABN_E_WORKSPACE; }
    hipStream_t st = (hipStream_t)stream;
    GemmP p = {};
    p.A = dz; p.lda = out_dim;
    p.B = a_in; p.ldb = in_dim;
    p.C = scratch; p.ldc = in_dim;
    p.C2 = scratch + out_dim * in_dim;
    p.slab_stride = stride;
    p.M = (int)out_dim; p.N = (int)in_dim + 1; p.K = (int)rows;
    p.k_chunk = (int)align_up((rows + splits - 1) / splits, BK);
    p.ones_col = (int)in_dim;
    p.a_vec = aligned16(dz) && (out_dim % 4 == 0);
    p.b_vec = aligned16(a_in) && (in_dim % 4 == 0);
    int rc = launch_gemm<false, false, EPI_WGRAD>(p, splits, st);
    if (rc != ABN_OK) return rc;
    ReduceTable rt = {};
    rt.n_layers = 1; rt.splits[0] = splits; rt.slab_stride = stride;
    rt.off[0] = 0; rt.nW[0] = out_dim * in_dim; rt.nb[0] = out_dim; rt.dW[0] = dW; rt.db[0] = db;
    rt.total = out_dim * in_dim + out_dim;
    hipLaunchKernelGGL(slab_reduce_kernel, dim3(grid_for((rt.total + 3) / 4)), dim3(256), 0, st, scratch, rt);
    ABN_CHECK_LAUNCH("linear_wgrad");
    return ABN_OK;
}
// ... 62 lines not shown
```

### abnet3_amd/csrc/tower_planes.h

```cpp
#pragma once
#include <type_traits>

#include "gemm_f32.h"

namespace abn {

typedef int v4i __attribute__((ext_vector_type(4)));

constexpr int PL_ROWS = 32;
constexpr int PL_WAVES = 8;
constexpr int PL_NT = 64 * PL_WAVES;
constexpr int PL_MAXW = 512;
constexpr int PL_MAXSTEPS = PL_MAXW / 16;
#ifdef PL_DEPTH_OVERRIDE
constexpr int PL_DEPTH = PL_DEPTH_OVERRIDE;
#else
constexpr int PL_DEPTH = 4;
#endif
constexpr int PL_PART_BYTES = 4 * 16 * 64 * 4;
constexpr int PL_SC_BYTES = PL_WAVES * 64 * 4 + PL_WAVES * 32 * 4;
constexpr int PL_AMAX = 32;

__host__ __device__ inline int pl_steps(int64_t contraction) { return ((int)((contraction + 15) / 16) + PL_DEPTH - 1) / PL_DEPTH * PL_DEPTH; }
__host__ __device__ inline int pl_blocks(int64_t features) { return (int)((features + 31) / 32); }
// ... 1239 lines not shown
    const int blk0 = ws.blk0;

    f32x16 acc[BPW];
#pragma unroll
    for (int j = 0; j < BPW; ++j)
#pragma unroll
        for (int q = 0; q < 16; ++q) acc[j][q] = 0.0f;
    float cinv[BPW];
#pragma unroll
    for (int j = 0; j < BPW; ++j) cinv[j] = NP == 2 && ws.active ? packed_inv(p.wpt[l], nblk, nsteps, blk0 + j) * ainv : 1.0f;
    {
        bool chain_next = false;
        int nblk2 = 1, nsteps2 = 0, ioff2 = 0;
        if constexpr (PL_HANDOVER && NP <= 2 && BPW == 2 && KS == 1) {
            if (l - 1 >= (p.dx ? 0 : 1)) {
                nblk2 = (p.dims[l - 1] + 31) / 32;
                nsteps2 = pl_steps(K);
                ioff2 = (int)(p.wpt[l - 1] - p.wbase);
                chain_next = nblk2 > PL_WAVES;
            }
        }
        if (!ws.active) ring.filled = false;
        const int ioff = (int)(p.wpt[l] - p.wbase);
        int wv[BPW], dnext[BPW];
#pragma unroll
        for (int j = 0; j < BPW; ++j) {
            const int blk = blk0 + j < nblk ? blk0 + j : nblk - 1;
            const int o = ioff + (blk * nsteps + ws.s_first) * (NP * 1024);
            const int blk2 = blk0 + j < nblk2 ? blk0 + j : nblk2 - 1;
            wv[j] = o + lane * 16;
            dnext[j] = ioff2 + blk2 * nsteps2 * (NP * 1024) - o;
        }
        if (ws.active) ring_kloop<NP, BPW>(acc, ring, wv, dnext, chain_next, img, ws.s_first, ws.my_steps, lane);
    }
    DSTAMP(4 + 4 * (p.n_layers - 1 - l));

    const float* __restrict__ mask = l >= 1 ? p.mask[l - 1] : nullptr;
    const DropGen drop = make_drop(l >= 1 && !mask ? p.drop_seed : nullptr, p.drop_p, l - 1);
    const bool masked = mask || drop.on;
    const int gr = row0 + r;
    const bool row_ok = gr < p.rows;
    const int grc = row_ok ? gr : p.rows - 1;
    f32x4 av[BPW][4], mv[BPW][4];
    if (ws.active && ws.khalf == 0 && l >= 1) {
        const int row_off = tgather_row_offset<NP>(r);
#pragma unroll
        for (int j = 0; j < BPW; ++j) {
            const int blk = blk0 + j < nblk ? blk0 + j : nblk - 1;
            const char* tile = p.tp[l] + ((int64_t)blk * p.tp_steps + 2 * blockIdx.x) * tile_bytes<NP>();
#pragma unroll
            for (int g = 0; g < 4; ++g) {
#pragma unroll
                for (int e = 0; e < 4; ++e) av[j][g][e] = tgather<NP>(tile, row_off, 8 * g + 4 * h + e);
                const int k = 32 * (blk0 + j) + 4 * h + 8 * g;
                if (mask) mv[j][g] = *reinterpret_cast<const f32x4*>(mask + (int64_t)grc * K + (k < K ? k : K - 4));
                else if (drop.on) mv[j][g] = drop4(drop, gr, k);
            }
        }
    }
    auto finish = [&]() {
        if constexpr (NP == 2) {
#pragma unroll
            for (int j = 0; j < BPW; ++j)
#pragma unroll
                for (int q = 0; q < 16; ++q) acc[j][q] *= cinv[j];
        }
        if (l == 0) return;
        with_act(p.act[l - 1], [&](auto tag) {
            constexpr int ACT = decltype(tag)::value;
#pragma unroll
            for (int j = 0; j < BPW; ++j)
#pragma unroll
                for (int g = 0; g < 4; ++g) {
                    const bool live = 32 * (blk0 + j) + 4 * h + 8 * g < K;
#pragma unroll
                    for (int e = 0; e < 4; ++e) {
                        float v = acc[j][4 * g + e] * act_grad(av[j][g][e], ACT);
                        if (masked) v *= mv[j][g][e];
                        acc[j][4 * g + e] = live ? v : 0.0f;
                    }
                }
        });
    };
    float* const sc = part + PL_PART_BYTES / 4;
    const bool rescale = NP == 2 && l >= 1;
    auto park_max = [&]() {
        float m = 0.0f;
        if (ws.active && ws.khalf == 0) {
#pragma unroll
            for (int j = 0; j < BPW; ++j)
#pragma unroll
                for (int q = 0; q < 16; ++q) m = fmaxf(m, fabsf(acc[j][q]));
        }
        sc[wave * 64 + lane] = m;
    };
    if (KS == 1) {
        if (ws.active) finish();
        if (rescale) park_max();
    } else if (ws.active && ws.khalf == 1) {
#pragma unroll
        for (int q = 0; q < 16; ++q) part[((wave & 3) * 16 + q) * 64 + lane] = acc[0][q];
    }
    DSTAMP(5 + 4 * (p.n_layers - 1 - l));
    __syncthreads();
    DSTAMP(6 + 4 * (p.n_layers - 1 - l));
    if (KS == 2 && ws.active && ws.khalf == 0) {
#pragma unroll
        for (int q = 0; q < 16; ++q) acc[0][q] += part[(wave * 16 + q) * 64 + lane];
        finish();
    }
    float osc = 1.0f;
    if (rescale) {
        if (KS == 2) { park_max(); __syncthreads(); }
        float oinv;
        const float m = row_scales(sc, wave, lane, osc, oinv);
        ainv = oinv;
        if (wave == 0) store_amax_rows(p.amax_dz[l - 1] + (int64_t)blockIdx.x * PL_AMAX, m, 0.0f, lane);
    }
    const float* const inv_tab = sc + PL_WAVES * 64 + wave * 32;
    if (ws.active && ws.khalf == 0) {
#pragma unroll
        for (int j = 0; j < BPW; ++j) {
            const int blk = blk0 + j;
            if (blk < nblk) {
                Frag<NP> f[2];
#pragma unroll
                for (int t2 = 0; t2 < 2; ++t2) {
                    const f32x4 v0 = {acc[j][8 * t2], acc[j][8 * t2 + 1], acc[j][8 * t2 + 2], acc[j][8 * t2 + 3]};
                    const f32x4 v1 = {acc[j][8 * t2 + 4], acc[j][8 * t2 + 5], acc[j][8 * t2 + 6], acc[j][8 * t2 + 7]};
                    if (l == 0) {
                        const int k = 32 * blk + 16 * t2 + 4 * h;
                        if (row_ok && k < K) *reinterpret_cast<f32x4*>(p.dx + (int64_t)gr * K + k) = v0;
                        if (row_ok && k + 8 < K) *reinterpret_cast<f32x4*>(p.dx + (int64_t)gr * K + k + 8) = v1;
                    } else {
                        f[t2] = make_frag<NP>(v0, v1, osc);
                        store_frag<NP>(img + (int64_t)(2 * blk + t2) * (NP * 1024) + lane * 16, f[t2]);
                    }
                }
                if (l >= 1) emit_planes<NP>(p.dzp[l - 1] + ((int64_t)blk * p.tp_steps + 2 * blockIdx.x) * tile_bytes<NP>(), f, idf, lane, -1, 0, inv_tab);
            }
        }
    }
    if (l - 1 >= 1 || (l == 1 && p.dx)) {
        const int next_steps = pl_steps(K);
        const bf16x8 z = {};
        for (int s = 2 * nblk + wave; s < next_steps; s += PL_WAVES)
#pragma unroll
            for (int pl = 0; pl < NP; ++pl) *reinterpret_cast<bf16x8*>(img + ((int64_t)s * NP + pl) * 1024 + lane * 16) = z;
    }
    __syncthreads();
    DSTAMP(7 + 4 * (p.n_layers - 1 - l));
}

template <int NP>
__global__ __launch_bounds__(PL_NT) void tower_dgrad_planes_kernel(PlanesBwdP p)
{
    extern __shared__ __attribute__((aligned(16))) char pl_smem[];
    char* const img = pl_smem;
    float* const part = reinterpret_cast<float*>(pl_smem + PL_MAXSTEPS * NP * 1024);
    const int lane = threadIdx.x & 63;
    const int wave = __builtin_amdgcn_readfirstlane(threadIdx.x >> 6);
    const int r = lane & 31, h = lane >> 5;
    const int row0 = blockIdx.x * PL_ROWS;
    const int top = p.n_layers - 1;
    const int NT = p.dims[top + 1];
    bf16x8 idf[2];
    make_identity<NP>(idf, lane);
#ifdef PL_EXP_PRIO
    if ((PL_EXP_PRIO == 1) == (wave >= 4)) __builtin_amdgcn_s_setprio(1);
#endif
    DSTAMP(0);

    double* const coef = reinterpret_cast<double*>(part);
    double* const term_s = coef + 64;
    int* const is_last_s = reinterpret_cast<int*>(term_s + 32);
    const bool with_loss = p.loss_kind >= 0;
    if (with_loss) {
        const int B = p.B;
        const int Bv = p.n_valid ? *p.n_valid : B;
        const double lscale = p.n_valid && p.scale != 1.0 ? 1.0 / (double)(Bv > 0 ? Bv : 1) : p.scale;
#pragma unroll
        for (int it = 0; it < 2; ++it) {
            const int lr = 4 * wave + 2 * it + (lane >> 5), l = lane & 31;
            const int g = row0 + lr;
            double inv = 0.0, kself = 0.0, term = 0.0;
            const int tower = g < p.rows && g >= B ? 1 : 0, pi_ = g < p.rows ? g - tower * B : 0;
            const bool ok = g < p.rows && pi_ < Bv;
            const float* a = p.a_top + (int64_t)pi_ * NT;
            const float* b = p.a_top + (int64_t)(B + pi_) * NT;
            double dot = 0.0, s11 = 0.0, s22 = 0.0;
            for (int c = l; c < NT / 4; c += 32) {
                const float4 u = reinterpret_cast<const float4*>(a)[c];
                const float4 v = reinterpret_cast<const float4*>(b)[c];
                dot += (double)u.x * v.x + (double)u.y * v.y + (double)u.z * v.z + (double)u.w * v.w;
                s11 += (double)u.x * u.x + (double)u.y * u.y + (double)u.z * u.z + (double)u.w * u.w;
                s22 += (double)v.x * v.x + (double)v.y * v.y + (double)v.z * v.z + (double)v.w * v.w;
            }
#pragma unroll
            for (int o = 16; o >= 1; o >>= 1) {
                dot += __shfl_xor(dot, o, 64);
                s11 += __shfl_xor(s11, o, 64);
                s22 += __shfl_xor(s22, o, 64);
            }
            if (ok) {
                constexpr double EPS = 1e-6;
                const double n1 = sqrt(s11), n2 = sqrt(s22);
                const double c1 = n1 > EPS ? n1 : EPS, c2 = n2 > EPS ? n2 : EPS;
                const double cs = dot / (c1 * c2);
                double v = 0.0;
                switch (p.y_dtype) {
                    case ABN_Y_I8: v = ((const int8_t*)p.y)[pi_]; break;
                    case ABN_Y_I32: v = ((const int32_t*)p.y)[pi_]; break;
                    case ABN_Y_I64: v = (double)((const int64_t*)p.y)[pi_]; break;
                    case ABN_Y_F32: v = ((const float*)p.y)[pi_]; break;
                    default: v = ((const double*)p.y)[pi_]; break;
                }
                const int code = v == 1.0 ? 1 : (v == -1.0 ? -1 : 0);
                double dcos;
                if (p.loss_kind == ABN_LOSS_COSCOS2) {
                    if (code == 1) { term = (1.0 - cs) * 0.5; dcos = -0.5; }
                    else if (code == -1) { term = cs * cs; dcos = 2.0 * cs; }
                    else { term = cs; dcos = 1.0; }
                } else {
                    if (code == 1) { term = 1.0 - cs; dcos = -1.0; }
                    else if (code == -1) { const double hh = cs - p.margin; term = hh > 0.0 ? hh : 0.0; dcos = hh >= 0.0 ? 1.0 : 0.0; }
                    else { term = cs; dcos = 1.0; }
                }
                dcos *= lscale;
                inv = dcos / (c1 * c2);
                const double k1 = n1 > 0.0 ? dcos * cs / (c1 * n1) : 0.0;
                const double k2 = n2 > 0.0 ? dcos * cs / (c2 * n2) : 0.0;
                kself = tower ? k2 : k1;
                if (tower) term = 0.0;
            }
            if (l == 0) { coef[2 * lr] = inv; coef[2 * lr + 1] = kself; term_s[lr] = term; }
        }
        __syncthreads();
        if (threadIdx.x == 0) {
            double sum = 0.0;
            for (int i = 0; i < 32; ++i) sum += term_s[i];
            *is_last_s = abn_ticket_publish(&p.loss_partial[blockIdx.x], sum, p.loss_counter, gridDim.x);
        }
        __syncthreads();
        if (*is_last_s && wave == 0) {
            double sum = 0.0;
            for (int i = lane; i < (int)gridDim.x; i += 64) sum += abn_ticket_partial(&p.loss_partial[i]);
#pragma unroll
            for (int o = 32; o >= 1; o >>= 1) sum += __shfl_xor(sum, o, 64);
            if (lane == 0) {
                const float lv = (float)(sum * lscale);
                *p.loss_out = lv;
                if (p.loss_accum) *p.loss_accum += (double)lv;
                __hip_atomic_store(p.loss_counter, 0u, __ATOMIC_RELAXED, __HIP_MEMORY_SCOPE_AGENT);
            }
        }
    }

    DSTAMP(1);
    const int steps_t = pl_steps(NT), blocks_t = steps_t / 2;
    const int gr = row0 + r;
    const bool row_ok = gr < p.rows;
    const float* __restrict__ mask = p.mask[top];
    const DropGen drop_top = make_drop(mask ? nullptr : p.drop_seed, p.drop_p, top);
    const int my_tower = gr >= p.B ? 1 : 0;
    const float* const self_row = p.a_top + (int64_t)(row_ok ? gr : 0) * NT;
    const float* const partner_row = p.a_top + (int64_t)(row_ok && with_loss ? (my_tower ? gr - p.B : gr + p.B) : 0) * NT;
    const double my_inv = with_loss ? coef[2 * r] : 0.0, my_k = with_loss ? coef[2 * r + 1] : 0.0;
    auto top_step = [&](int s, f32x4* v) {
        v[0] = v[1] = f32x4{0.f, 0.f, 0.f, 0.f};
#pragma unroll
        for (int u = 0; u < 2; ++u) {
            const int c = 16 * s + 4 * h + 8 * u;
            if (row_ok && c < NT) {
                if (with_loss) {
                    const f32x4 es = *reinterpret_cast<const f32x4*>(self_row + c);
                    const f32x4 ep = *reinterpret_cast<const f32x4*>(partner_row + c);
#pragma unroll
                    for (int e = 0; e < 4; ++e) {
                        float o = (float)(ep[e] * my_inv - es[e] * my_k);
                        if (p.act[top] != ACT_NONE) o *= act_grad(es[e], p.act[top]);
                        v[u][e] = o;
                    }
                    if (mask || drop_top.on) {
                        const f32x4 m = mask ? *reinterpret_cast<const f32x4*>(mask + (int64_t)gr * NT + c) : drop4(drop_top, gr, c);
#pragma unroll
                        for (int e = 0; e < 4; ++e) v[u][e] *= m[e];
                    }
                } else {
                    v[u] = *reinterpret_cast<const f32x4*>(p.d_out + (int64_t)gr * NT + c);
                    if (!p.d_out_is_dz) {
                        const f32x4 a = *reinterpret_cast<const f32x4*>(p.a_top + (int64_t)gr * NT + c);
#pragma unroll
                        for (int e = 0; e < 4; ++e) v[u][e] *= act_grad(a[e], p.act[top]);
                        if (mask || drop_top.on) {
                            const f32x4 m = mask ? *reinterpret_cast<const f32x4*>(mask + (int64_t)gr * NT + c) : drop4(drop_top, gr, c);
#pragma unroll
                            for (int e = 0; e < 4; ++e) v[u][e] *= m[e];
                        }
                    }
                }
            }
        }
    };
    float ainv = 1.0f;
    if constexpr (NP == 2) {
        float* const sc = part + PL_PART_BYTES / 4;
        f32x4 v[2][2][2];
        float m = 0.0f;
#pragma unroll
        for (int u = 0; u < 2; ++u)
#pragma unroll
            for (int t2 = 0; t2 < 2; ++t2) {
                const int kb = wave + PL_WAVES * u;
                v[u][t2][0] = v[u][t2][1] = f32x4{0.f, 0.f, 0.f, 0.f};
                if (kb < blocks_t) top_step(2 * kb + t2, v[u][t2]);
                m = fmaxf(m, absmax8(v[u][t2][0], v[u][t2][1]));
            }
        sc[wave * 64 + lane] = m;
        __syncthreads();
        float osc;
        m = row_scales(sc, wave, lane, osc, ainv);
        if (wave == 0) store_amax_rows(p.amax_dz[top] + (int64_t)blockIdx.x * PL_AMAX, m, 0.0f, lane);
#pragma unroll
        for (int u = 0; u < 2; ++u) {
            const int kb = wave + PL_WAVES * u;
            if (kb < blocks_t) {
                Frag<NP> f[2];
#pragma unroll
                for (int t2 = 0; t2 < 2; ++t2) {
                    f[t2] = make_frag<NP>(v[u][t2][0], v[u][t2][1], osc);
                    store_frag<NP>(img + (int64_t)(2 * kb + t2) * (NP * 1024) + lane * 16, f[t2]);
                }
                if (kb < pl_blocks(NT))
                    emit_planes<NP>(p.dzp[top] + ((int64_t)kb * p.tp_steps + 2 * blockIdx.x) * tile_bytes<NP>(), f, idf, lane, -1, 0,
                                    sc + PL_WAVES * 64 + wave * 32);
            }
        }
    } else {
        for (int kb = wave; kb < blocks_t; kb += PL_WAVES) {
            Frag<NP> f[2];
#pragma unroll
            for (int t2 = 0; t2 < 2; ++t2) {
                f32x4 v[2];
                top_step(2 * kb + t2, v);
                f[t2] = make_frag<NP>(v[0], v[1]);
                store_frag<NP>(img + (int64_t)(2 * kb + t2) * (NP * 1024) + lane * 16, f[t2]);
            }
            if (kb < pl_blocks(NT))
                emit_planes<NP>(p.dzp[top] + ((int64_t)kb * p.tp_steps + 2 * blockIdx.x) * tile_bytes<NP>(), f, idf, lane, -1, 0);
        }
    }
    __syncthreads();
    DSTAMP(2);

    WeightRing<NP> ring;
    ring_open(ring, p.wbase, p.wbytes);
    for (int l = top; l >= (p.dx ? 0 : 1); --l) {
        const int nblk = (p.dims[l] + 31) / 32;
        if (nblk > PL_WAVES) planes_dgrad_layer<NP, 2, 1>(p, l, img, part, idf, wave, lane, row0, ainv, ring);
        else if (nblk > PL_WAVES / 2 || pl_steps(p.dims[l + 1]) % (2 * PL_DEPTH) != 0) planes_dgrad_layer<NP, 1, 1>(p, l, img, part, idf, wave, lane, row0, ainv, ring);
        else planes_dgrad_layer<NP, 1, 2>(p, l, img, part, idf, wave, lane, row0, ainv, ring);
    }
}

struct BnBwdP {
    int l, rows, rows_call;
    float n_stat;
    const float* n_stat_dev;
    int N, K;
    int act_l, act_prev;
    const float* da;
    const float* z;
    const float* mean;
    const float* invstd;
    const float* gamma;
    const float* beta;
    const float* s1;
    const float* s2;
    const float* mask;
    const unsigned long long* drop_seed;
    float drop_p;
    char* dzp;
    float* amax_dz;
    int64_t tp_steps;
    const char* wpt;
    float* da_prev;
    const float* z_prev;
    const float* mean_prev;
    const float* invstd_prev;
    const float* gamma_prev;
    const float* beta_prev;
    float* part_out;
    const int* n_valid;
};

template <int NP, int BPW, int KS>
__device__ __forceinline__ void bn_dgrad_product(const BnBwdP& q, char* __restrict__ img, float* __restrict__ part, int wave,
                                                 int lane, int row0, int row_end, int call, float ainv)
{
    const int N = q.N, K = q.K;
    const int nsteps = pl_steps(N), nblk = (K + 31) / 32;
    const int r = lane & 31, h = lane >> 5;
    const WaveShare<BPW, KS> ws(wave, nblk, nsteps);
    const int blk0 = ws.blk0;
    f32x16 acc[BPW];
#pragma unroll
    for (int j = 0; j < BPW; ++j)
#pragma unroll
        for (int x = 0; x < 16; ++x) acc[j][x] = 0.0f;
    if (ws.active) planes_kloop<NP, BPW>(acc, q.wpt, nblk, nsteps, img, blk0, ws.s_first, ws.my_steps, lane);
    if (KS == 2 && ws.active && ws.khalf == 1) {
#pragma unroll
        for (int x = 0; x < 16; ++x) part[((wave & 3) * 16 + x) * 64 + lane] = acc[0][x];
    }
    if (KS == 2) __syncthreads();
    if (!(ws.active && ws.khalf == 0)) return;
    if (KS == 2) {
#pragma unroll
        for (int x = 0; x < 16; ++x) acc[0][x] += part[(wave * 16 + x) * 64 + lane];
    }
    if constexpr (NP == 2) {
#pragma unroll
        for (int j = 0; j < BPW; ++j) {
            const float cinv = packed_inv(q.wpt, nblk, nsteps, blk0 + j) * ainv;
#pragma unroll
            for (int x = 0; x < 16; ++x) acc[j][x] *= cinv;
        }
    }
    const int gr = row0 + r;
    const bool row_ok = gr < row_end;
    const int grc = row_ok ? gr : row0;
    float* const orow = q.da_prev + (int64_t)grc * K;
    float* const pw = q.l >= 1 ? q.part_out + (int64_t)blockIdx.x * (2 * PL_MAXW) : nullptr;
    with_act(q.act_prev, [&](auto tag) {
        constexpr int ACT = decltype(tag)::value;
#pragma unroll
        for (int j = 0; j < BPW; ++j)
#pragma unroll
            for (int g = 0; g < 4; ++g) {
                const int n = 32 * (blk0 + j) + 8 * g + 4 * h;
                const bool live = n < K;
                const f32x4 d4 = {acc[j][4 * g], acc[j][4 * g + 1], acc[j][4 * g + 2], acc[j][4 * g + 3]};
                if (live && row_ok) *reinterpret_cast<f32x4*>(orow + n) = d4;
                if (q.l >= 1) {
                    const int nc = live ? n : K - 4;
                    const f32x4 z4 = *reinterpret_cast<const f32x4*>(q.z_prev + (int64_t)grc * K + nc);
                    const f32x4 mu = *reinterpret_cast<const f32x4*>(q.mean_prev + (int64_t)call * K + nc);
                    const f32x4 is = *reinterpret_cast<const f32x4*>(q.invstd_prev + (int64_t)call * K + nc);
                    f32x4 xh;
#pragma unroll
                    for (int e = 0; e < 4; ++e) xh[e] = (z4[e] - mu[e]) * is[e];
                    const f32x4 ga = *reinterpret_cast<const f32x4*>(q.gamma_prev + nc), be = *reinterpret_cast<const f32x4*>(q.beta_prev + nc);
                    f32x4 sd, sq;
#pragma unroll
                    for (int e = 0; e < 4; ++e) {
                        const float a = act_apply(xh[e] * ga[e] + be[e], ACT);
                        const float dy = live && row_ok ? d4[e] * act_grad(a, ACT) : 0.0f;
                        sd[e] = dy;
                        sq[e] = dy * xh[e];
                    }
                    half_wave_sum4(sd);
                    half_wave_sum4(sq);
                    if (r == 16 && live) {
                        *reinterpret_cast<f32x4*>(pw + n) = sd;
                        *reinterpret_cast<f32x4*>(pw + PL_MAXW + n) = sq;
                    }
                }
            }
    });
}

template <int NP>
__global__ __launch_bounds__(PL_NT) void bn_bwd_layer_kernel(BnBwdP q)
{
    extern __shared__ __attribute__((aligned(16))) char pl_smem[];
    char* const img = pl_smem;
    float* const part = reinterpret_cast<float*>(pl_smem + PL_MAXSTEPS * NP * 1024);
    const int lane = threadIdx.x & 63;
    const int wave = __builtin_amdgcn_readfirstlane(threadIdx.x >> 6);
    const int r = lane & 31, h = lane >> 5;
    const int wpc = (q.rows_call + PL_ROWS - 1) / PL_ROWS;
    const int call = blockIdx.x / wpc;
    const int row0 = call * q.rows_call + (blockIdx.x - call * wpc) * PL_ROWS;
    const int nv = q.n_valid ? min(max(*q.n_valid, 0), q.rows_call) : q.rows_call;
    const int row_end = call * q.rows_call + nv;
    const int N = q.N;
    bf16x8 idf[2];
    make_identity<NP>(idf, lane);

    const float nf = q.n_valid ? (float)(nv > 0 ? nv : 1) : (q.n_stat_dev ? q.n_stat_dev[call] : q.n_stat);
    float* const k_s = part, * const ga_s = part + PL_MAXW, * const be_s = part + 2 * PL_MAXW, * const s1_s = part + 3 * PL_MAXW,
               * const s2_s = part + 4 * PL_MAXW, * const mu_s = part + 5 * PL_MAXW, * const is_s = part + 6 * PL_MAXW;
    for (int c = threadIdx.x; c < N; c += PL_NT) {
        const float ga = q.gamma[c];
        k_s[c] = ga * q.invstd[(int64_t)call * N + c] / nf;
        mu_s[c] = q.mean[(int64_t)call * N + c];
        is_s[c] = q.invstd[(int64_t)call * N + c];
        ga_s[c] = ga;
        be_s[c] = q.beta[c];
        s1_s[c] = q.s1[(int64_t)call * N + c];
        s2_s[c] = q.s2[(int64_t)call * N + c];
    }
    __syncthreads();
    const int steps = pl_steps(N), blocks = steps / 2;
    const int gr = row0 + r;
    const bool row_ok = gr < row_end;
// ... 480 lines not shown
```

### abnet3_amd/model.py

```python
import os

import torch
import torch.nn as nn

from . import _lib

activation_functions = {'relu': nn.ReLU,
                        'sigmoid': nn.Sigmoid,
                        'tanh': nn.Tanh,
                        'softmax': nn.Softmax,
                        }

init_functions = {'xavier_uni': nn.init.xavier_uniform_,
                  'xavier_normal': nn.init.xavier_normal_,
                  'orthogonal': nn.init.orthogonal_}

_ALIGN = 64


class NetworkBuilder(nn.Module):

    def __init__(self, *args, **kwargs):
        super(NetworkBuilder, self).__init__()

# ... 437 lines not shown

    def _init_hip_state(self):
        self._flat = None
        self._last_grad_flat = None
        self._offsets = None
        self._segs = None
        self._mask_override = None
        self._generation = getattr(self, '_generation', 0)
        self._live_cache = None
        self.precision = os.environ.get('ABNET3_PRECISION', 'f16x2')
        assert self.precision in _lib.PRECISION, self.precision

    def _segments(self):
        raise NotImplementedError

    def _segment_list(self):
        if self._segs is None:
            self._segs = self._segments()
        return self._segs

    def _blocks(self):
        return [b for seg in self._segment_list() for b in seg.blocks]

    def _bn_modules(self):
        return [bn for _, bn in self._blocks() if bn is not None]

    def live_parameters(self):
        return [p for seg in self._segment_list() for p in seg.params]

    def flatten_parameters(self):
        params = self.live_parameters()
        dev = params[0].device
        offs, o = [], 0
        for p in params:
            offs.append(o)
            o += (p.numel() + _ALIGN - 1) // _ALIGN * _ALIGN
        flat = torch.zeros(o, dtype=torch.float32, device=dev)
        for p, off in zip(params, offs):
            flat[off:off + p.numel()].copy_(p.data.reshape(-1))
            p.data = flat[off:off + p.numel()].view(p.shape)
        self._flat = flat
        self._offsets = offs
        self._live_cache = params
        return flat

    def _apply(self, fn, *args, **kwargs):
        out = super(_HipNetwork, self)._apply(fn, *args, **kwargs)
        if getattr(self, '_flat', None) is not None and self._live_cache is not None \
                and self._flat.device == self._live_cache[0].device and self._is_flat(full=True):
            return out
        self._flat = None
        self._generation = getattr(self, '_generation', 0) + 1
        return out

    def _is_flat(self, full=False):
        if self._flat is None:
            return False
        base = self._flat.data_ptr()
        params = self._live_cache
        if full:
            return all(p.data_ptr() == base + 4 * off for p, off in zip(params, self._offsets))
        return (params[0].data_ptr() == base + 4 * self._offsets[0] and
                params[-1].data_ptr() == base + 4 * self._offsets[-1])

    def flat_parameters(self):
        if not self._is_flat():
            self.flatten_parameters()
        return self._flat

    def grads_in_flat_buffer(self):
        buf = getattr(self, '_last_grad_flat', None)
        if buf is None or not self._is_flat():
            return False
        base = buf.data_ptr()
        return all(p.grad is not None and p.grad.data_ptr() == base + 4 * off
                   for p, off in zip(self.live_parameters(), self._offsets))

    def flat_grad(self):
        if self.grads_in_flat_buffer():
            return self._last_grad_flat
        self.flat_parameters()
        buf = torch.zeros_like(self._flat)
        for p, off in zip(self.live_parameters(), self._offsets):
            if p.grad is not None:
                buf[off:off + p.numel()].copy_(p.grad.reshape(-1))
                p.grad = buf[off:off + p.numel()].view(p.shape)
        self._last_grad_flat = buf
        return buf

    def _draw_dropout_masks(self, rows, device):
        if self._mask_override is not None:
            return self._mask_override
        p = float(self.p_dropout)
        if p <= 0.0:
            return None
        if os.environ.get('ABN_DROPOUT_IN_KERNEL') != '0':
            return _DropoutInKernel(p, self)
        return self._draw_mask_tensors(rows, device)

    def _draw_mask_tensors(self, rows, device):
        p = float(self.p_dropout)
        widths = [lin.out_features for lin, _ in self._blocks()]
        offs, o = [], 0
        for w in widths:
            offs.append(o)
            o += (rows * w + _ALIGN - 1) // _ALIGN * _ALIGN
        flat = torch.empty(o, dtype=torch.float32, device=device)
        if p < 1.0:
            flat.bernoulli_(1.0 - p).mul_(1.0 / (1.0 - p))
        else:
            flat.zero_()
        return [flat[off:off + rows * w].view(rows, w) for off, w in zip(offs, widths)]

    def resident_tower_failed(self):
        words = [(seg, seg.sync_fail_word()) for seg in self._segment_list()]
        words = [(seg, w) for seg, w in words if w is not None and not getattr(seg, '_sync_disabled', False)]
        if not words:
            return 0
        got = torch.cat([w for _, w in words]).cpu()
        hit = 0
        for (seg, _), v in zip(words, got.tolist()):
            if v != 0:
                seg.recover_sync()
                hit += 1
        if hit:
            import warnings
            warnings.warn('abnet3_amd: a resident BatchNorm tower launch gave up on a hand-over between workgroups (the '
                          'GPU is shared with another process, stream or resident kernel?).  The steps since were dropped '
                          '-- no parameter changed, their losses are not numbers --; the sync buffer is cleared and this '
                          'network trains on one launch per layer from here on (ABN_BN_PERSIST=0 does so from the start).',
                          RuntimeWarning, stacklevel=2)
        return hit

    def weights_changed_behind_torch(self):
        self._weights_epoch = getattr(self, '_weights_epoch', 0) + 1
        for seg in (getattr(self, '_segs', None) or ()):
            seg._wpack_key = None

    _weights_rewritten = weights_changed_behind_torch

    def _run(self, seg, grad_pass, masks, x1, x2, n_calls, split):
        if x1.shape[0] == 0:
            _lib.require_device(x1)
            if x1.dim() != 2 or x1.shape[1] != seg.input_dim:
                raise ValueError('abnet3_amd: expected input of shape [n, %d], got %s'
                                 % (seg.input_dim, tuple(x1.shape)))
            empty = x1.new_zeros((0, seg.output_dim))
            return (empty, empty.clone()) if split else empty
        return _TowerFunction.apply(seg, grad_pass, masks, n_calls, split, not torch.is_grad_enabled(), x1, x2,
                                    *seg.params)

    _HIP_STATE = ('_flat', '_last_grad_flat', '_offsets', '_segs', '_mask_override',
                  '_generation', '_live_cache', '_weights_epoch', '_pending_reduce', '_fused_loss_refused',
                  '_pending_lower', 'bn_sync', '_bn_sync_agreed')

    def whoami(self):
        params = {k: v for k, v in self.__dict__.items() if k not in self._HIP_STATE}
        return {'params': params, 'class_name': self.__class__.__name__}

    def load_network(self, network_path=None):
        self.load_state_dict(torch.load(network_path))


class SiameseNetwork(_HipNetwork):

    def __init__(self, input_dim=None, num_hidden_layers=None, hidden_dim=None,
                 output_dim=None, p_dropout=0.1, batch_norm=False,
                 type_init='xavier_uni', activation_layer=None,
                 output_path=None, last_non_linearity="default"):
        super(SiameseNetwork, self).__init__()
        assert activation_layer in ('relu', 'sigmoid', 'tanh')
        assert type_init in ('xavier_uni', 'xavier_normal', 'orthogonal')
        assert type(input_dim) == int, 'input dim should be int'
        assert type(hidden_dim) == int, 'hidden dim should be int'
        assert type(num_hidden_layers) == int, 'num hidden lay should be int'
        assert type(output_dim) == int, 'output dim should be int'
        assert num_hidden_layers + 2 <= _lib.MAX_LAYERS, 'too many layers'

        self.input_dim = input_dim
        self.num_hidden_layers = num_hidden_layers
        self.hidden_dim = hidden_dim
        self.output_dim = output_dim
        self.activation_layer = activation_layer
        self.batch_norm = batch_norm
        self.type_init = type_init
        self.last_non_linearity = last_non_linearity
        self.p_dropout = p_dropout

        activation = activation_functions[activation_layer]

        input_layer = [nn.Linear(input_dim, hidden_dim), nn.Dropout(p=p_dropout)]
        if self.batch_norm:
            input_layer.append(nn.BatchNorm1d(hidden_dim))
        input_layer.append(activation())
        self.input_emb = nn.Sequential(*input_layer)

        hidden = []
        for idx in range(self.num_hidden_layers):
            hidden.append(nn.Linear(hidden_dim, hidden_dim))
            hidden.append(nn.Dropout(p=p_dropout))
            if self.batch_norm:
                hidden.append(nn.BatchNorm1d(hidden_dim))
            hidden.append(activation())
        self.hidden_layers = nn.Sequential(*hidden)

        output_layer = [nn.Linear(hidden_dim, output_dim), nn.Dropout(p=p_dropout)]
        if self.batch_norm:
            output_layer.append(nn.BatchNorm1d(output_dim))
        if self.last_non_linearity == "default":
            output_layer.append(activation())
            self._last_act = activation_layer
        elif self.last_non_linearity is None:
            self._last_act = 'none'
        else:
            output_layer.append(activation_functions[self.last_non_linearity]())
            self._last_act = self.last_non_linearity
        self.output_layer = nn.Sequential(*output_layer)
        self.output_path = output_path
        self.apply(self.init_weight_method)
        self._init_hip_state()

    def init_weight_method(self, layer):
        if isinstance(layer, nn.Linear):
            init_func = init_functions[self.type_init]
            init_func(layer.weight.data,
                      gain=nn.init.calculate_gain(self.activation_layer))
            layer.bias.data.fill_(0.0)
            self._weights_rewritten()

    def _segments(self):
        last = 'none' if self._last_act == 'softmax' else self._last_act
        return [_Segment(self, _blocks_of(self.input_emb, self.hidden_layers, self.output_layer),
                         0, self.activation_layer, last, self.batch_norm)]

    def _run_tower(self, x1, x2, n_calls, split):
        seg = self._segment_list()[0]
        rows = x1.shape[0] * (2 if x2 is not None else 1)
        masks = self._draw_dropout_masks(rows, x1.device) if self.training else None
        out = self._run(seg, _GradPass(self), masks, x1, x2, n_calls, split)
        if self._last_act == 'softmax':
            out = tuple(_SoftmaxRows.apply(o) for o in out) if split else _SoftmaxRows.apply(out)
        return out

    def direct_ok(self, loss_type=None):
        if loss_type is None:
            return self._last_act != 'softmax'
        from .loss import coscos2, cosmargin, KLLoss
        if self._last_act == 'softmax':
            return loss_type is KLLoss
        return loss_type in (coscos2, cosmargin)

    def direct_forward(self, x1, x2, forward_only=False, n_valid=None, source=None):
        seg = self._segment_list()[0]
        rows = 2 * x1.shape[0]
        masks = self._draw_dropout_masks(rows, x1.device) if self.training else None
        out, sv = _segment_forward(seg, masks, 2, x1, x2, forward_only=forward_only, n_valid=n_valid, source=source)
        return out, (seg, sv, _GradPass(self))

    def takes_padded_batch_norm(self, x12, npad):
        seg = self._segment_list()[0]
        desc = seg.descriptor(with_grads=False)
        lib = _lib.load()
        return lib.abn_tower_path(_lib.C.byref(desc), _lib.ptr(x12[:npad]), _lib.ptr(x12[npad:]), 2 * npad, 2, 1, _lib.ptr(x12), 0,
                                  None) in (_lib.PATH_BN_LAYERS, _lib.PATH_BN_TOWER)

    def direct_dz_info(self, state):
        seg, sv, _ = state
        if seg.batch_norm or os.environ.get('ABN_LOSS_DZ') == '0':
            return None
        masks = None
        if isinstance(sv.masks, _DropSeed):
            return None
        if sv.masks is not None:
            m = sv.masks[-1]
            half = m.shape[0] // 2
            masks = (m[:half], m[half:])
        return seg.last_act, masks

    def direct_logits_info(self, state):
        if self._last_act != 'softmax':
            return None
        seg, sv, _ = state
        if seg.batch_norm or isinstance(sv.masks, _DropSeed):
            return None, False
        if sv.masks is None:
            return None, True
        m = sv.masks[-1]
        half = m.shape[0] // 2
        return (m[:half], m[half:]), True

    def can_defer_reduce(self, state):
        seg = state[0]
        return (os.environ.get('ABN_FUSED_STEP') != '0'
                and len(seg.params) == len(self.live_parameters()))

    def direct_backward(self, state, d_out, d_out_is_dz=False, defer_reduce=False):
        seg, sv, grad_pass = state
        self._pending_reduce = None
        if defer_reduce:
            grads, _, self._pending_reduce = _segment_backward(seg, sv, d_out, grad_pass, False, d_out_is_dz, True)
        else:
            grads, _ = _segment_backward(seg, sv, d_out, grad_pass, False, d_out_is_dz)
        for p, g in zip(seg.params, grads):
            p.grad = g

    def direct_backward_loss(self, state, y, loss_kind, margin, avg, defer_reduce=False, n_valid=None, loss_accum=None, loss_ws=None,
                             wgrad_split=None):
        if loss_kind not in ('coscos2', 'cosmargin'):
            return None
        seg, sv, grad_pass = state
        rows = sv.rows
        if (sv.n_calls != 2 or os.environ.get('ABN_LOSS_IN_BACKWARD') == '0'
                or self._fused_loss_refused == (rows, self.precision)):
            return None
        from .loss import _scratch
        lib = _lib.load()
        y = y.contiguous()
        _lib.require_device(y)
        source = getattr(sv, 'source', None)
        if y.dtype not in _lib.Y_DTYPE or (y.numel() * 2 != rows and source is None):
            return None
        grad_buf, grads = grad_pass.views(seg)
        desc = seg.descriptor(with_grads=True, grad_buf=grad_buf, masks=sv.masks, d_out_is_dz=True, defer_reduce=defer_reduce)
        if source is not None:
            desc.source = _lib.C.addressof(source)
        if wgrad_split is not None:
            desc.wgrad_part, desc.wgrad_split = 1, int(wgrad_split)
        elif defer_reduce:
            _lend_forward_workspace(desc, sv, rows)
        if sv.n_valid is not None:
            desc.n_valid = sv.n_valid.data_ptr()
            if n_valid is None:
                n_valid = sv.n_valid
        scratch_floats = lib.abn_tower_bwd_scratch_floats(_lib.C.byref(desc), rows)
        scratch = torch.empty(max(scratch_floats, 1), dtype=torch.float32, device=y.device)
        loss = torch.empty((), dtype=torch.float32, device=y.device)
        need = lib.abn_tower_backward_loss_ws_bytes(rows)
        lws = loss_ws if loss_ws is not None and loss_ws.numel() >= need else _scratch(need, y.device)
        rc = lib.abn_tower_backward_loss(
            _lib.C.byref(desc), _lib.ptr(sv.x1), _lib.ptr(sv.x2), _lib.ptr(y), _lib.Y_DTYPE[y.dtype], _lib.LOSS[loss_kind],
            float(margin), int(bool(avg)), rows, _lib.ptr(sv.ws), _lib.ptr(scratch), scratch_floats, _lib.ptr(loss),
            _lib.ptr(lws), _lib.ptr(n_valid), _lib.ptr(loss_accum), _lib.stream())
        if rc == _lib.E_UNSUPPORTED:
            self._fused_loss_refused = (rows, self.precision)
            grad_pass.buf = None
            grad_pass.used.discard(id(seg))
            return None
        _lib.check(rc, 'abn_tower_backward_loss')
        _lib.note_path(desc, sv.x1, sv.x2, rows, sv.n_calls, True, sv.ws, backward=True)
        self._pending_reduce = (desc, rows, scratch, scratch_floats, grad_buf, seg) if defer_reduce else None
        self._pending_lower = (desc, rows, scratch, scratch_floats, sv) if wgrad_split is not None else None
        for p, g in zip(seg.params, grads):
            p.grad = g
        return loss

    _fused_loss_refused = None

    def direct_backward_lower(self):
        desc, rows, scratch, scratch_floats, sv = self._pending_lower
        self._pending_lower = None
        desc.wgrad_part = 2
        _lib.check(_lib.load().abn_tower_backward(
            _lib.C.byref(desc), _lib.ptr(sv.x1), _lib.ptr(sv.x2), _lib.ptr(None), rows,
            sv.n_calls, _lib.ptr(sv.ws), _lib.ptr(scratch), scratch_floats, _lib.ptr(None), _lib.stream()), 'abn_tower_backward')

    def grad_split_offset(self, state, layer):
        seg = state[0]
        offs = seg.offsets()
        per_layer = len(seg.params) // len(seg.blocks)
        return int(offs[layer * per_layer])

    def take_pending_reduce(self):
        pending = getattr(self, '_pending_reduce', None)
        self._pending_reduce = None
        return pending

    def forward_once(self, x):
        return self._run_tower(x, None, 1, False)

    def forward(self, input1, input2):
        return self._run_tower(input1, input2, 2, True)

    def forward_pair_rows(self, x12):
        if x12.shape[0] % 2:
            raise ValueError('abnet3_amd: forward_pair_rows needs an even number of rows')
        return self._run_tower(x12, None, 2, True)

    def save_network(self, epoch=''):
        torch.save(self.state_dict(), self.output_path + str(epoch) + '.pth')

    def load_network(self, network_path=None):
        self.load_state_dict(torch.load(network_path))


class SiameseMultitaskNetwork(_HipNetwork):

    def __init__(self, input_dim=None, num_hidden_layers_shared=None,
                 num_hidden_layers_spk=None,
                 num_hidden_layers_phn=None,
                 hidden_dim=None,
                 output_dim=None, p_dropout=0.1, batch_norm=False,
                 type_init='xavier_uni', activation_layer=None,
                 output_path=None):
        super(SiameseMultitaskNetwork, self).__init__()
        assert activation_layer in ('relu', 'sigmoid', 'tanh')
        assert type_init in ('xavier_uni', 'xavier_normal', 'orthogonal')
        assert type(input_dim) == int, 'input dim should be int'
        assert type(hidden_dim) == int, 'hidden dim should be int'
        assert type(num_hidden_layers_shared) == int
        assert type(num_hidden_layers_spk) == int
        assert type(num_hidden_layers_phn) == int
        assert type(output_dim) == int, 'output dim should be int'
        assert num_hidden_layers_shared + 1 <= _lib.MAX_LAYERS, 'too many layers'

        self.input_dim = input_dim
        self.num_hidden_layers_shared = num_hidden_layers_shared
        self.num_hidden_layers_spk = num_hidden_layers_spk
        self.num_hidden_layers_phn = num_hidden_layers_phn
        self.hidden_dim = hidden_dim
        self.output_dim = output_dim
        self.activation_layer = activation_layer
        self.batch_norm = batch_norm
        self.type_init = type_init
        self.p_dropout = p_dropout

        activation = activation_functions[activation_layer]

        def block(n_in, n_out):
            layers = [nn.Linear(n_in, n_out), nn.Dropout(p=p_dropout)]
            if self.batch_norm:
                layers.append(nn.BatchNorm1d(n_out))
            layers.append(activation())
            return layers

        def stack(n):
            layers = []
            for idx in range(n):
                layers += block(hidden_dim, hidden_dim)
            return layers

        self.input_emb = nn.Sequential(*block(input_dim, hidden_dim))
        shared = stack(self.num_hidden_layers_shared)
        spk = stack(self.num_hidden_layers_spk)
        phn = stack(self.num_hidden_layers_phn)
        self.hidden_layers_shared = nn.Sequential(*shared)
        self.hidden_layers_spk = nn.Sequential(*spk)
        self.hidden_layers_phn = nn.Sequential(*phn)
        self.output_layer_spk = nn.Sequential(*block(hidden_dim, output_dim))
        self.output_layer_phn = nn.Sequential(*block(hidden_dim, output_dim))

        self.output_path = output_path
        self.apply(self.init_weight_method)
        self._init_hip_state()

    def init_weight_method(self, layer):
        if isinstance(layer, nn.Linear):
            init_func = init_functions[self.type_init]
            init_func(layer.weight.data,
                      gain=nn.init.calculate_gain(self.activation_layer))
            layer.bias.data.fill_(0.0)
            self._weights_rewritten()

    def _segments(self):
        act, bn = self.activation_layer, self.batch_norm
        trunk = _blocks_of(self.input_emb, self.hidden_layers_shared)
        return [_Segment(self, trunk, 0, act, act, bn),
                _Segment(self, _blocks_of(self.output_layer_spk), len(trunk), act, act, bn),
                _Segment(self, _blocks_of(self.output_layer_phn), len(trunk) + 1, act, act, bn)]

    def _forward(self, x1, x2):
        trunk, head_spk, head_phn = self._segment_list()
        n_calls = 1 if x2 is None else 2
        rows = x1.shape[0] * n_calls
        gp = _GradPass(self)
        masks = self._draw_dropout_masks(rows, x1.device) if self.training else None
        h = self._run(trunk, gp, masks, x1, x2, n_calls, False)
        split = x2 is not None
        return (self._run(head_spk, gp, masks, h, None, n_calls, split),
                self._run(head_phn, gp, masks, h, None, n_calls, split))

    def forward_once(self, x):
        return self._forward(x, None)

    def forward(self, input1, input2):
        (spk1, spk2), (phn1, phn2) = self._forward(input1, input2)
        return spk1, phn1, spk2, phn2

    def save_network(self, epoch=''):
        torch.save(self.state_dict(), self.output_path + epoch + '.pth')



class _WeightsHolder(object):
    __slots__ = ('w',)

    def __init__(self):
        self.w = None


class MultimodalSiameseNetwork(_HipNetwork):

    def __init__(self, integration_unit=None,
                 pre_integration_net_params=None,
                 post_integration_net_params=None,
                 attention_lr=None,
                 asynchronous_integration_index=None,
                 p_dropout=0, batch_norm=False,
                 type_init='xavier_uni', activation_layer=None,
                 output_path=None, *args, **kwargs):
# ... 245 lines not shown
```

### abnet3_amd/trainer.py

```python
import copy
import gc
import os
import pickle
import time
import warnings
from pathlib import Path

import torch
import torch.optim as optim

import weakref

import numpy as np

from . import _lib, parallel
from .loss import unit_grad
from .model import NetworkBuilder, SiameseMultitaskNetwork

try:
    from tensorboardX import SummaryWriter
except Exception:
    class SummaryWriter(object):
        def __init__(self, log_dir=None):
            self.log_dir = log_dir
# ... 169 lines not shown
        else:
            self.optimizer = FlatOptimizer(self.network, optimizer_type, self.lr,
                                           self.momentum)
        if self.dp:
            parallel.broadcast_parameters(self.network.flat_parameters())
            if hasattr(self.network, 'weights_changed_behind_torch'):
                self.network.weights_changed_behind_torch()
            parallel.seed_all(self.seed)
            if os.environ.get('ABN_ONESHOT_ALLREDUCE') == '1':
                try:
                    self.oneshot = parallel.OneShotAllReduce(self.network.flat_parameters().numel())
                except (RuntimeError, OSError, AttributeError) as e:
                    warnings.warn('abnet3_amd: ABN_ONESHOT_ALLREDUCE: falling back to torch.distributed.all_reduce (%s)' % (e,))
            if sync_batch_norm and getattr(self.network, 'batch_norm', False):
                self.network.bn_sync = parallel.bn_sync()
        self.sync_batch_norm = bool(sync_batch_norm)

    def params(self):
        return None

    def whoami(self):
        parts = {'network': self.network, 'loss': self.loss, 'dataloader': self.dataloader}
        if self.feature_generator is not None:
            parts['feature_generator'] = self.feature_generator
        description = {name: part.whoami() for name, part in parts.items()}
        description['params'] = self.params()
        description['class_name'] = type(self).__name__
        return description

    def save_whoami(self):
        with open(self.network.output_path + '.params', 'wb') as fh:
            pickle.dump(self.whoami(), fh)

    def optimize_model(self, do_training=True):
        raise NotImplementedError('Unimplemented optimize_model for class:',
                                  self.__class__.__name__)

    def _keep_best(self, epoch):
        if self.rank != 0:
            return
        print('Saving best model so far, epoch {}... '.format(epoch + 1), end='', flush=True)
        if self.checkpoints:
            self.network.save_network(epoch=epoch + 1)
        self.network.save_network()
        self.save_whoami()
        print('Done.')

    def train(self):
        master = self.rank == 0
        self.patience_dev, self.best_dev = 0, None
        self.train_losses, self.dev_losses = [], []
        self.num_batches_train = self.num_batches_dev = 0
        curves = {'train': SummaryWriter(log_dir=str(self.log_dir / 'train_loss')),
                  'dev': SummaryWriter(log_dir=str(self.log_dir / 'dev_loss'))}

        def plot(step):
            curves['train'].add_scalar('loss', self.train_losses[-1], step)
            curves['dev'].add_scalar('loss', self.dev_losses[-1], step)

        self.network.eval()
        if master:
            self.network.save_network()
        self.optimize_model(do_training=False)
        plot(0)
        if self.checkpoints and master:
            self.network.save_network(epoch=0)
        self.statistics_training = dict.fromkeys(self.statistics_training, 0)

        for epoch in range(self.num_epochs):
            dev_loss = self.optimize_model(do_training=True)
            plot(epoch + 1)
            if self.best_dev is None or dev_loss < self.best_dev:
                self.best_dev, self.best_epoch, self.patience_dev = dev_loss, epoch, 0
                self._keep_best(epoch)
                continue
            self.patience_dev += 1
            if self.patience_dev > self.patience:
                if master:
                    print('No improvements after {} iterations, stopping now'.format(self.patience))
                    print('Finished Training')
                break
        if master:
            print('Saving best checkpoint network')

    def plot_summary_statistics(self):
        print(" ***** Statistics for the training step ***** ")
        for key in self.statistics_training.keys():
            stats = self.statistics_training[key]
            print(" Number of {} pairs seen: {} \t\t".format(key, stats))

    def pretty_print_losses(self, train_loss, dev_loss):
        if self.rank == 0:
            print("  training loss:\t\t{:.6f}".format(train_loss))
            print("  dev loss:\t\t\t{:.6f}".format(dev_loss))


class TrainerSiamese(TrainerBuilder):

    def __init__(self, *args, **kwargs):
        super(TrainerSiamese, self).__init__(*args, **kwargs)
        assert isinstance(self.network, NetworkBuilder)

    def give_batch_to_network(self, batch):
        X_batch1, X_batch2, y_batch = batch
        X_batch1 = X_batch1.cuda(non_blocking=True)
        X_batch2 = X_batch2.cuda(non_blocking=True)
        y_batch = y_batch.cuda(non_blocking=True)
        emb_batch1, emb_batch2 = self.network(X_batch1, X_batch2)
        return self.loss(emb_batch1, emb_batch2, y_batch)

    def _direct_ok(self):
        if not getattr(self, 'direct_steps', True):
            return False
        ok = getattr(self, '_direct_cache', None)
        if ok is None:
            from .loss import coscos2, cosmargin, KLLoss
            from .model import SiameseNetwork
            ok = self._direct_cache = (
                type(self.network) is SiameseNetwork and type(self.loss) in (coscos2, cosmargin, KLLoss)
                and self.network.direct_ok(type(self.loss))
                and isinstance(self.optimizer, FlatOptimizer)
                and type(self).give_batch_to_network is TrainerSiamese.give_batch_to_network)
        return ok

    @staticmethod
    def _backward(loss_value):
        if loss_value.dim() == 0 and loss_value.dtype == torch.float32 and loss_value.is_cuda:
            torch.autograd.backward(loss_value, grad_tensors=unit_grad(loss_value.device))
        else:
            loss_value.backward()

    overlap_allreduce = True
    oneshot = None

    def _overlap_split(self, state):
        net = self.network
        seg = state[0]
        if not self.overlap_allreduce or self.oneshot is not None or getattr(net, 'batch_norm', False) or len(seg.blocks) < 3:
            return None
        one = getattr(self, '_one_segment', None)
        if one is None or one[0] is not seg:
            one = self._one_segment = (seg, len(seg.params) == 2 * len(seg.blocks) and len(list(net.parameters())) == len(seg.params))
        return (len(seg.blocks) + 1) // 2 if one[1] else None

    def _loss_is_mean(self):
        return bool(getattr(self.loss, 'avg', False))

    def train_step(self, batch, do_training=True):
        if do_training and self._direct_ok() and batch[0].shape[0] > 0:
            X_batch1, X_batch2, y_batch = batch
            X_batch1 = X_batch1.cuda(non_blocking=True)
            X_batch2 = X_batch2.cuda(non_blocking=True)
            y_batch = y_batch.cuda(non_blocking=True)
            emb, state = self.network.direct_forward(X_batch1, X_batch2)
            n = X_batch1.shape[0]
            info = self.network.direct_dz_info(state)
            self.optimizer.zero_grad()
            defer = not self.dp and self.network.can_defer_reduce(state)
            split = self._overlap_split(state) if self.dp else None
            loss_value = self.network.direct_backward_loss(
                state, y_batch, type(self.loss).__name__, getattr(self.loss, 'margin', 0.0), self.loss.avg, defer_reduce=defer,
                wgrad_split=split)
            if loss_value is not None and split is not None:
                flat = self.network.flat_grad()
                cut = self.network.grad_split_offset(state, split)
                work = [torch.distributed.all_reduce(flat[cut:], op=torch.distributed.ReduceOp.SUM, async_op=True)]
                self.network.direct_backward_lower()
                work.append(torch.distributed.all_reduce(flat[:cut], op=torch.distributed.ReduceOp.SUM, async_op=True))
                for w in work:
                    w.wait()
                self.optimizer.grad_scale = 1.0 / self.world_size if self._loss_is_mean() else 1.0
                self.optimizer.step()
                return loss_value.detach()
            logits = self.network.direct_logits_info(state)
            if loss_value is not None:
                pass
            elif logits is not None:
                loss_value, dz = self.loss.value_and_dz(emb[:n], emb[n:], y_batch, 'softmax', logits[0])
                self.network.direct_backward(state, dz.view(2 * n, -1), d_out_is_dz=logits[1], defer_reduce=defer)
            elif info is not None:
                loss_value, dz = self.loss.value_and_dz(emb[:n], emb[n:], y_batch, info[0], info[1])
                self.network.direct_backward(state, dz.view(2 * n, -1), d_out_is_dz=True, defer_reduce=defer)
            else:
                loss_value, de = self.loss.value_and_grad(emb[:n], emb[n:], y_batch)
                self.network.direct_backward(state, de.view(2 * n, -1), defer_reduce=defer)
            if self.dp:
                if split is not None:
                    flat = self.network.flat_grad()
                    cut = self.network.grad_split_offset(state, split)
                    torch.distributed.all_reduce(flat[cut:], op=torch.distributed.ReduceOp.SUM)
                    torch.distributed.all_reduce(flat[:cut], op=torch.distributed.ReduceOp.SUM)
                    self.optimizer.grad_scale = 1.0 / self.world_size if self._loss_is_mean() else 1.0
                else:
                    self.optimizer.grad_scale = parallel.all_reduce_gradients(
                        self.network.flat_grad(), self._loss_is_mean(), self.oneshot)
            self.optimizer.step()
        elif do_training:
            loss_value = self.give_batch_to_network(batch)
            self.optimizer.zero_grad()
            self._backward(loss_value)
            if self.dp:
                self.optimizer.grad_scale = parallel.all_reduce_gradients(
                    self.network.flat_grad(), self._loss_is_mean(), self.oneshot)
            self.optimizer.step()
        else:
            with torch.no_grad():
                loss_value = self.give_batch_to_network(batch)
            self.optimizer.zero_grad()
        return loss_value.detach()

    def make_graphed_step(self, example_batch, warmup=3):
        bs = getattr(self.network, 'bn_sync', None)
        if bs is not None and type(bs).__name__ != 'RcclBatchNormSync':
            raise NotImplementedError('abnet3_amd: a step with cross-replica BatchNorm statistics through the Python callback '
                                      '(parallel.BatchNormSync) calls back to the host between launches and cannot be captured '
                                      'into a graph')
        static, fwd_loss = self._graph_inputs(example_batch)
        opt = self.optimizer
        capture_opt = (not self.dp and isinstance(opt, FlatOptimizer)
                       and opt.kind != 'adam')
        side = torch.cuda.Stream()
        side.wait_stream(torch.cuda.current_stream())
        with torch.cuda.stream(side):
            for _ in range(max(1, warmup)):
                warmup_loss = self.train_step(tuple(static), True)
        torch.cuda.current_stream().wait_stream(side)
        torch.cuda.synchronize()
        graph = torch.cuda.CUDAGraph()
        steps_before = getattr(opt, 'step_count', 0)
        gc_was_enabled = gc.isenabled()
        gc.disable()
        try:
            with torch.cuda.graph(graph, capture_error_mode=_capture_mode()):
                loss_value = fwd_loss()
                opt.zero_grad()
                self._backward(loss_value)
                if capture_opt:
                    opt.step()
        finally:
            if gc_was_enabled:
                gc.enable()
        if capture_opt:
            opt.step_count = steps_before
        static_loss = loss_value.detach()
        net = self.network
        live = list(net.live_parameters()) if hasattr(net, 'live_parameters') else list(net.parameters())
        captured_grads = [p.grad for p in live]
        captured_flat = getattr(net, '_last_grad_flat', None)

        blob = getattr(self, '_static_blob', None)
        self._static_blob = None

        def step(batch):
            if isinstance(batch, torch.Tensor):
                blob.copy_(batch, non_blocking=True)
            else:
                for dst, src in zip(static, batch):
                    dst.copy_(src, non_blocking=True)
            graph.replay()
            if hasattr(net, 'weights_changed_behind_torch'):
                net.weights_changed_behind_torch()
            for p, g in zip(live, captured_grads):
                p.grad = g
            if captured_flat is not None:
                net._last_grad_flat = captured_flat
            if capture_opt:
                opt.step_count += 1
            else:
                if self.dp:
                    opt.grad_scale = parallel.all_reduce_gradients(
                        self.network.flat_grad(), self._loss_is_mean(), self.oneshot)
                opt.step()
            return static_loss
        step.graph = graph
        step.warmup_loss = warmup_loss
        step.flat_ptr = self.network.flat_parameters().data_ptr()
        return step

    GRAPH_AFTER = 3
    MAX_GRAPHS = 4

    def train_step_auto(self, batch):
        if (not getattr(self, 'graph_steps', False) or not isinstance(self.optimizer, FlatOptimizer)
                or getattr(self.network, 'bn_sync', None) is not None):
            return self.train_step(batch, True)
        if not hasattr(self, '_graphs'):
            self._graphs, self._shape_seen = {}, {}
        key = tuple((tuple(t.shape), str(t.dtype)) for t in batch)
        step = self._graphs.get(key)
        if step is not None:
            if step.flat_ptr == self.network.flat_parameters().data_ptr() and self.network.training:
                return step(batch)
            del self._graphs[key]
        n = self._shape_seen[key] = self._shape_seen.get(key, 0) + 1
        if n < self.GRAPH_AFTER or len(self._graphs) >= self.MAX_GRAPHS or batch[0].shape[0] == 0:
            return self.train_step(batch, True)
        step = self.make_graphed_step(batch, warmup=1)
        self._graphs[key] = step
        return step.warmup_loss

    BUCKET = 32
    MIN_BUCKET = 32
    MAX_BUCKET_GRAPHS = 96

    def _planned(self, train_mode):
        dl = self.dataloader
        if not getattr(self, 'planned_passes', True) or not hasattr(dl, 'plan'):
            return None
        if not self._direct_ok():
            return None
        if type(self.loss).__name__ == 'KLLoss':
            return None
        if getattr(self.network, 'batch_norm', False) and getattr(self.network, 'bn_sync', None) is not None:
            return None
        if getattr(self, '_plan_refused', False):
            return None
        return dl.plan(train_mode)

    def _bucket(self, n):
        return max(self.MIN_BUCKET, (n + self.BUCKET - 1) // self.BUCKET * self.BUCKET)

    def _bucket_state(self, npad, plan):
        st = getattr(self, '_buckets', None)
        flat_ptr = self.network.flat_parameters().data_ptr()
        if st is not None and self._bucket_flat_ptr != flat_ptr:
            st = None
        if st is None:
            self._bucket_flat_ptr = flat_ptr
            st = self._buckets = {}
            self._bucket_pool = torch.cuda.graph_pool_handle()
            self._loss_acc = torch.zeros((), dtype=torch.float64, device=plan.table.device)
            self._loss_ws = torch.zeros(1 << 16, dtype=torch.uint8, device=plan.table.device)
            _PLANNED_TRAINERS.add(self)
        key = (npad, plan.table.shape[1], plan.labels.dtype)
        b = st.get(key)
        if b is None:
            dev, D = plan.table.device, plan.table.shape[1]
            b = st[key] = dict(x12=torch.zeros(2 * npad, D, dtype=torch.float32, device=dev),
                               y=torch.zeros(npad, dtype=plan.labels.dtype, device=dev),
                               nv=torch.zeros(1, dtype=torch.int32, device=dev), graph=None, npad=npad)
        return b

    def _bucket_body(self, b):
        net, opt, npad = self.network, self.optimizer, b['npad']
        x12 = b['x12']
        src = b.get('source')
        emb, state = net.direct_forward(x12[:npad], x12[npad:], n_valid=b['nv'] if getattr(net, 'batch_norm', False) else None,
                                        source=src['src'] if src is not None else None)
        opt.zero_grad()
        defer = not self.dp and net.can_defer_reduce(state)
        loss_value = net.direct_backward_loss(state, src['labels'] if src is not None else b['y'], type(self.loss).__name__,
                                              getattr(self.loss, 'margin', 0.0), self.loss.avg, defer_reduce=defer, n_valid=b['nv'],
                                              loss_accum=self._loss_acc, loss_ws=self._loss_ws)
        return loss_value

    def _step_source(self, plan):
        opt = self.optimizer
        if (self.dp or os.environ.get('ABN_STEP_SOURCE') == '0' or not isinstance(opt, FlatOptimizer) or opt.kind == 'adam'
                or getattr(self.network, 'batch_norm', False) or not plan.order):
            return None
        key = (plan.table.data_ptr(), plan.idx1.data_ptr(), plan.idx2.data_ptr(), plan.labels.data_ptr(), plan.table.shape[0])
        st = getattr(self, '_src', None)
        if st is None or st['key'] != key or st['steps'].shape[0] < len(plan.order):
            if st is not None:
                self._forget_captured_steps()
            dev = plan.table.device
            steps = torch.zeros(max(len(plan.order), 1024), 2, dtype=torch.int64, device=dev)
            ctr = torch.zeros(1, dtype=torch.int32, device=dev)
            src = _lib.StepSource()
            src.table, src.table_rows = plan.table.data_ptr(), plan.table.shape[0]
            src.idx1, src.idx2, src.labels = plan.idx1.data_ptr(), plan.idx2.data_ptr(), plan.labels.data_ptr()
            src.steps, src.step_ctr = steps.data_ptr(), ctr.data_ptr()
            st = self._src = dict(key=key, steps=steps, ctr=ctr, src=src, labels=plan.labels, plan_arrays=(plan.table, plan.idx1, plan.idx2))
        spans = np.array([plan.span(b) for b in plan.order], dtype=np.int64).reshape(-1, 2)
        st['steps'][:len(spans)].copy_(torch.from_numpy(spans), non_blocking=False)
        st['ctr'].zero_()
        return st

    def _bucket_finish(self):
        opt = self.optimizer
        if self.dp:
            opt.grad_scale = parallel.all_reduce_gradients(self.network.flat_grad(), self._loss_is_mean(), self.oneshot)
        opt.step()

    def _planned_step(self, plan, bid, source=None):
        lib = _lib.load()
        first, n = plan.span(bid)
        if n == 0:
            self._loss_acc.add_(self.train_step(plan.materialise(bid), True))
            return 1
        b = self._bucket_state(self._bucket(n), plan)
        if 'source' not in b:
            b['source'] = None
            if source is not None:
                probe = self.network._segment_list()[0].descriptor(with_grads=False)
                x12 = b['x12']
                if lib.abn_tower_path(_lib.C.byref(probe), _lib.ptr(x12[:b['npad']]), _lib.ptr(x12[b['npad']:]), 2 * b['npad'], 2, 1,
                                      _lib.ptr(x12), 0, None) == _lib.PATH_WIDE and plan.table.shape[1] % 4 == 0:
                    b['source'] = source
        if b['source'] is not None and b['source'] is not source:
            return 0
        sourced = b['source'] is not None
        if not sourced:
            _lib.check(lib.abn_gather_pairs(_lib.ptr(plan.table), plan.table.shape[0], plan.table.shape[1], _lib.ptr(plan.idx1), _lib.ptr(plan.idx2),
                                            first, n, b['npad'], _lib.ptr(plan.labels), plan.labels.element_size(),
                                            _lib.ptr(b['x12']), _lib.ptr(b['y']), _lib.ptr(b['nv']), _lib.stream()),
                       'abn_gather_pairs')
        done = 2 if sourced else 1
        opt = self.optimizer
        in_graph_opt = not self.dp and opt.kind != 'adam'
        if b['graph'] is not None:
            g, grads, flat, pending = b['graph']
            g.replay()
            net = self.network
            net.weights_changed_behind_torch()
            for p_, g_ in zip(net.live_parameters(), grads):
                p_.grad = g_
            net._last_grad_flat = flat
            if in_graph_opt:
                opt.step_count += 1
            else:
                net._pending_reduce = pending
                self._bucket_finish()
            return done
        if getattr(self.network, 'batch_norm', False) and not self.network.takes_padded_batch_norm(b['x12'], b['npad']):
            return 0
        if self._bucket_body(b) is None:
            return 0
        self._bucket_finish()
        if len([1 for v in self._buckets.values() if v['graph'] is not None]) >= self.MAX_BUCKET_GRAPHS:
            return done
        steps_before = opt.step_count
        graph = torch.cuda.CUDAGraph()
        gc_was_enabled = gc.isenabled()
        gc.disable()
        try:
            torch.cuda.synchronize()
            with torch.cuda.graph(graph, pool=self._bucket_pool, capture_error_mode=_capture_mode()):
                self._bucket_body(b)
                pending = getattr(self.network, '_pending_reduce', None)
                if in_graph_opt:
                    opt.step()
        finally:
            if gc_was_enabled:
                gc.enable()
        opt.step_count = steps_before
        net = self.network
        b['graph'] = (graph, [p_.grad for p_ in net.live_parameters()], getattr(net, '_last_grad_flat', None), pending)
        return done

    def _planned_eval(self, plan, bid):
        lib = _lib.load()
        first, n = plan.span(bid)
        if n == 0:
            with torch.no_grad():
                self._loss_acc.add_(self.give_batch_to_network(plan.materialise(bid)))
            return
        b = self._bucket_state(self._bucket(n), plan)
        _lib.check(lib.abn_gather_pairs(_lib.ptr(plan.table), plan.table.shape[0], plan.table.shape[1], _lib.ptr(plan.idx1), _lib.ptr(plan.idx2),
                                        first, n, b['npad'], _lib.ptr(plan.labels), plan.labels.element_size(),
                                        _lib.ptr(b['x12']), _lib.ptr(b['y']), _lib.ptr(b['nv']), _lib.stream()),
                   'abn_gather_pairs')
        key = 'eval_train' if self.network.training else 'eval'
        if b.get(key) is not None:
            b[key].replay()
            return

        def body():
            net, npad = self.network, b['npad']
            emb, _ = net.direct_forward(b['x12'][:npad], b['x12'][npad:], forward_only=True)
            loss_value = torch.empty((), dtype=torch.float32, device=emb.device)
            D = emb.shape[1]
            _lib.check(lib.abn_pair_loss_padded(
                _lib.ptr(emb), _lib.ptr(emb[npad:]), _lib.ptr(b['y']), _lib.Y_DTYPE[b['y'].dtype], npad, D,
                _lib.LOSS[type(self.loss).__name__], float(getattr(self.loss, 'margin', 0.0)), int(bool(self.loss.avg)),
                _lib.ptr(b['nv']), _lib.ptr(loss_value), _lib.ptr(self._loss_acc), None, None, _lib.ptr(self._loss_ws),
                _lib.stream()), 'abn_pair_loss_padded')
        with torch.no_grad():
            body()
            if sum(1 for v in self._buckets.values() for k in ('graph', 'eval', 'eval_train') if v.get(k) is not None) >= 3 * self.MAX_BUCKET_GRAPHS:
                return
            graph = torch.cuda.CUDAGraph()
            gc_was_enabled = gc.isenabled()
            gc.disable()
            try:
                torch.cuda.synchronize()
                with torch.cuda.graph(graph, pool=self._bucket_pool, capture_error_mode=_capture_mode()):
                    body()
            finally:
                if gc_was_enabled:
                    gc.enable()
        b[key] = graph

    def _run_planned_eval(self, plan, loss_sum):
        if not plan.order:
            return 0
        self._bucket_state(self._bucket(plan.span(plan.order[0])[1]), plan)
        self._loss_acc.zero_()
        for bid in plan.order:
# ... 239 lines not shown
```

### include/abnet3_hip.h

```cpp
#ifndef ABNET3_HIP_H
#define ABNET3_HIP_H

#include <stdint.h>

#ifdef __cplusplus
extern "C" {
#endif

#define ABN_ABI_VERSION 20
#define ABN_MAX_LAYERS 16

enum { ABN_OK = 0, ABN_E_ARG = -1, ABN_E_LAUNCH = -2, ABN_E_WORKSPACE = -3,
       ABN_E_UNSUPPORTED = -4 };

enum { ABN_ACT_NONE = 0, ABN_ACT_SIGMOID = 1, ABN_ACT_RELU = 2, ABN_ACT_TANH = 3, ABN_ACT_SOFTMAX = 4 };

enum { ABN_LOSS_COSCOS2 = 0, ABN_LOSS_COSMARGIN = 1, ABN_LOSS_KL = 2 };

enum { ABN_Y_I8 = 0, ABN_Y_I32 = 1, ABN_Y_I64 = 2, ABN_Y_F32 = 3, ABN_Y_F64 = 4 };

enum { ABN_OPT_SGD = 0, ABN_OPT_ADADELTA = 1, ABN_OPT_ADAM = 2,
       ABN_OPT_ADAGRAD = 3, ABN_OPT_RMSPROP = 4 };

enum { ABN_PREC_F32 = 0, ABN_PREC_BF16 = 1, ABN_PREC_BF16X3 = 2, ABN_PREC_F16X2 = 3 };

typedef int (*abn_allreduce_fn)(void* ctx, void* device_doubles, int64_t n, void* stream);

int abn_abi_version(void);
const char* abn_last_error(void);

typedef struct abn_tower_desc {
    int32_t n_layers;
    int32_t act;
    int32_t last_act;
    int32_t batch_norm;
    int64_t dims[ABN_MAX_LAYERS + 1];
    const float* W[ABN_MAX_LAYERS];
    const float* b[ABN_MAX_LAYERS];
    const float* bn_w[ABN_MAX_LAYERS];
    const float* bn_b[ABN_MAX_LAYERS];
    float* bn_rm[ABN_MAX_LAYERS];
    float* bn_rv[ABN_MAX_LAYERS];
    float* dW[ABN_MAX_LAYERS];
    float* db[ABN_MAX_LAYERS];
    float* dbn_w[ABN_MAX_LAYERS];
    float* dbn_b[ABN_MAX_LAYERS];
    const float* drop_mask[ABN_MAX_LAYERS];
    int32_t precision;
    int32_t d_out_is_dz;
    int32_t defer_reduce;
    int32_t wpack_valid;
    int32_t forward_only;
    int32_t wgrad_part;
    void* wpack;
    const void* drop_seed;
    float drop_p;
    int32_t reserved2_;
    int32_t bn_sync_world;
    int32_t wgrad_split;
    abn_allreduce_fn bn_sync_fn;
    void* bn_sync_ctx;
    const int32_t* n_valid;
    void* bn_nbt[ABN_MAX_LAYERS];
    void* sync_ws;
    const float* fwd_ws;
    int64_t fwd_calls;
    const struct abn_step_source* source;
} abn_tower_desc;

typedef struct abn_step_source {
    const float* table;
    int64_t table_rows;
    const int64_t* idx1;
    const int64_t* idx2;
    const void* labels;
    const int64_t* steps;
    int32_t* step_ctr;
} abn_step_source;

typedef struct abn_rccl_ctx {
    void* comm;
    void* all_reduce;
    int64_t calls;
} abn_rccl_ctx;
int abn_rccl_allreduce_f64(void* ctx, void* device_doubles, int64_t n, void* stream);

int64_t abn_tower_ws_floats(const abn_tower_desc* t, int64_t rows, int64_t n_calls);
int64_t abn_tower_out_offset(const abn_tower_desc* t, int64_t rows, int64_t n_calls);
int64_t abn_tower_bwd_scratch_floats(const abn_tower_desc* t, int64_t rows);
int64_t abn_tower_sync_ws_bytes(void);
int64_t abn_tower_wpack_floats(const abn_tower_desc* t);
int abn_tower_uses_planes(const abn_tower_desc* t, int64_t rows, const float* x1, const float* x2,
                          const float* ws, int train);

enum {
    ABN_PATH_PER_LAYER = 0,
    ABN_PATH_FUSED_F32 = 1,
    ABN_PATH_PLANES = 2,
    ABN_PATH_PLANES_INFER = 3,
    ABN_PATH_PLANES_INFER_BN = 4,
    ABN_PATH_BN_LAYERS = 5,
    ABN_PATH_WIDE = 6,
    ABN_PATH_BN_TOWER = 7
};
int abn_tower_path(const abn_tower_desc* t, const float* x1, const float* x2, int64_t rows,
                   int64_t n_calls, int train, const float* ws, int backward,
                   int32_t* precision_out);

int64_t abn_tower_image_offset(const abn_tower_desc* t, int64_t rows, int64_t n_calls, int which,
                               int l);

void abn_reload_switches(void);

int abn_tower_forward(const abn_tower_desc* t, const float* x1, const float* x2,
                      int64_t rows, int64_t n_calls, int train, float* ws,
                      void* stream);

int abn_tower_backward(const abn_tower_desc* t, const float* x1, const float* x2,
                       const float* d_out, int64_t rows, int64_t n_calls,
                       const float* ws, float* scratch, int64_t scratch_floats,
                       float* dx, void* stream);

int abn_tower_backward_launch(const abn_tower_desc* t, const float* x1, const float* x2,
                              const float* d_out, int64_t rows, int64_t n_calls, const float* ws,
                              float* scratch, int64_t scratch_floats, int part, void* stream);

int64_t abn_tower_backward_loss_ws_bytes(int64_t rows);
int abn_tower_backward_loss(const abn_tower_desc* t, const float* x1, const float* x2, const void* y,
                            int y_dtype, int loss_kind, float margin, int avg, int64_t rows,
                            const float* ws, float* scratch, int64_t scratch_floats,
                            float* loss_out, void* loss_ws, const int32_t* n_valid,
                            double* loss_accum, void* stream);

int abn_tower_reduce_step(const abn_tower_desc* t, int64_t rows, const float* scratch,
                          int64_t scratch_floats, int kind, float* params, float* grads,
                          float* state1, float* state2, int64_t n, float lr, float hp0,
                          float hp1, float eps, int64_t step, float grad_scale, void* stream);

#define ABN_ONESHOT_MAX_RANKS 8
typedef struct abn_oneshot_ctx {
    int32_t rank, world;
    void* mail[ABN_ONESHOT_MAX_RANKS];
    int64_t cap_floats;
} abn_oneshot_ctx;
int64_t abn_oneshot_mail_bytes(int32_t world, int64_t cap_floats);
int abn_allreduce_oneshot(const abn_oneshot_ctx* ctx, float* buf, int64_t n, void* stream);

int abn_linear_forward(const float* x, const float* W, const float* b, int64_t rows,
                       int64_t in_dim, int64_t out_dim, int act, float* y, void* stream);
int abn_linear_dgrad(const float* dz, const float* W, int64_t rows, int64_t in_dim,
                     int64_t out_dim, const float* a_prev, int act_prev, float* dx,
                     void* stream);
int64_t abn_linear_wgrad_scratch_floats(int64_t rows, int64_t in_dim, int64_t out_dim);
int abn_linear_wgrad(const float* dz, const float* a_in, int64_t rows, int64_t in_dim,
                     int64_t out_dim, float* dW, float* db, float* scratch,
                     int64_t scratch_floats, void* stream);
int abn_linear_backward(const float* dz, const float* W, const float* a_in, int64_t rows,
                        int64_t in_dim, int64_t out_dim, int act_prev, float* dW,
                        float* db, float* dx, float* scratch, int64_t scratch_floats,
                        void* stream);
int abn_linear_backward_prec(const float* dz, const float* W, const float* a_in, int64_t rows,
                             int64_t in_dim, int64_t out_dim, int act_prev, int precision,
                             float* dW, float* db, float* dx, float* scratch,
                             int64_t scratch_floats, void* stream);

int64_t abn_pair_loss_ws_bytes(int64_t B);
int abn_pair_loss(const float* e1, const float* e2, const void* y, int y_dtype,
                  int64_t B, int64_t D, int kind, float margin, int avg,
                  float* loss_out, float* de1, float* de2, void* ws,
                  void* stream);
int abn_pair_loss_padded(const float* e1, const float* e2, const void* y, int y_dtype,
                         int64_t B, int64_t D, int kind, float margin, int avg,
                         const int32_t* n_valid, float* loss_out, double* loss_accum,
                         float* de1, float* de2, void* ws, void* stream);
int abn_pair_loss_dz(const float* e1, const float* e2, const void* y, int y_dtype,
                     int64_t B, int64_t D, int kind, float margin, int avg, int act,
                     const float* mask1, const float* mask2, float* loss_out,
                     float* dz1, float* dz2, void* ws, void* stream);

int abn_optimizer_step(int kind, float* params, const float* grads, float* state1,
                       float* state2, int64_t n, float lr, float hp0, float hp1,
                       float eps, int64_t step, float grad_scale, void* stream);

int64_t abn_dtw_ws_bytes(const int32_t* n1_host, const int32_t* n2_host,
                         int64_t npairs, int64_t rows1, int64_t rows2);
int64_t abn_dtw_host_stage_bytes(const int32_t* n1_host, const int32_t* n2_host,
                                 int64_t npairs);
int abn_dtw_batched(const float* feats1, int64_t rows1, const float* feats2,
                    int64_t rows2, const int64_t* off1_host, const int32_t* n1_host,
                    const int64_t* off2_host, const int32_t* n2_host, int64_t npairs,
                    int64_t D, int32_t* path1, int32_t* path2, int32_t* path_len,
                    int64_t path_stride, double* total_cost, void* ws,
                    int64_t ws_bytes, void* host_stage, int64_t host_stage_bytes,
                    void* stream);
int abn_dtw_batched_overlap(const float* feats1, int64_t rows1, const float* feats2,
                            int64_t rows2, const int64_t* off1_host, const int32_t* n1_host,
                            const int64_t* off2_host, const int32_t* n2_host, int64_t npairs,
                            int64_t D, int32_t* path1, int32_t* path2, int32_t* path_len,
                            int64_t path_stride, double* total_cost, void* ws,
                            int64_t ws_bytes, void* host_stage, int64_t host_stage_bytes,
                            void* stream, void* side_stream);
#define ABN_DTW_COST_MAX_N2 256
int64_t abn_dtw_cost_max_n2(void);
int abn_dtw_cost_batched(const float* feats1, int64_t rows1, const float* feats2, int64_t rows2,
                         const int64_t* off1, const int32_t* n1, const int64_t* off2, const int32_t* n2,
                         int64_t npairs, int64_t D, double* total_cost, int32_t* path_len, void* stream);
int abn_kl_tables(const float* x, int64_t rows, int64_t D, float floor, float* P, float* L,
                  uint8_t* bad_row, void* stream);
int abn_dtw_cost_kl_batched(const float* P1, const float* L1, int64_t rows1, const float* P2,
                            const float* L2, int64_t rows2, const int64_t* off1, const int32_t* n1,
                            const int64_t* off2, const int32_t* n2, int64_t npairs, int64_t D,
                            const uint8_t* bad1, const uint8_t* bad2, double* total_cost,
                            int32_t* path_len, void* stream);
int abn_abx_score(const double* dist, int64_t ndist, const int64_t* a_off, const int32_t* a_len,
                  const int64_t* b_off, const int32_t* b_len, const int32_t* row_cell, int64_t nrows,
                  int64_t ncells, int64_t* score2, int64_t* count, int32_t* refused, void* stream);
int abn_cosine_distance(const float* x, int64_t N, const float* y, int64_t M,
                        int64_t D, double* d, int32_t* bad_flag, void* stream);
int abn_cosine_distance_f64(const double* x, int64_t N, const double* y, int64_t M,
                            int64_t D, double* d, int32_t* bad_flag, void* stream);

int abn_arccos_f32(const float* x, int64_t n, int over_pi, float* out, void* stream);

int abn_softmax_rows(const float* z, int64_t rows, int64_t n, float* out, void* stream);
int abn_softmax_rows_backward(const float* a, const float* da, int64_t rows, int64_t n,
                              float* dz, void* stream);

enum { ABN_INTEGRATE_SUM = 0, ABN_INTEGRATE_CONCAT = 1 };
enum { ABN_INTEGRATE_W_NONE = 0, ABN_INTEGRATE_W_FIXED = 1, ABN_INTEGRATE_W_SCALAR = 2, ABN_INTEGRATE_W_ATTENTION = 3 };
int64_t abn_integrate_ws_bytes(int64_t rows);
int abn_integrate_forward(const float* x1, int64_t d1, const float* x2, int64_t d2, int64_t rows, int mode,
                          int weight_kind, float w_fixed, float w_complement, const float* w_scalar,
                          const float* z1, const float* z2, int64_t K, int act, float* out, float* w_out,
                          void* stream);
int abn_integrate_backward(const float* x1, int64_t d1, const float* x2, int64_t d2, int64_t rows, int mode,
                           int weight_kind, float w_fixed, float w_complement, const float* w_scalar,
                           const float* w, int64_t K, int act, const float* g, float* dx1, float* dx2,
                           float* dz, float* dw, void* ws, void* stream);

int abn_gather_rows(const float* table, const int64_t* idx, int64_t n, int64_t D,
                    float* out, void* stream);

int abn_gather_pairs(const float* table, int64_t table_rows, int64_t D, const int64_t* idx1, const int64_t* idx2,
                     int64_t first, int64_t n, int64_t n_pad, const void* labels,
                     int32_t label_bytes, float* x12, void* y_out, int32_t* n_valid, void* stream);

int abn_stack_frames(const float* feats, int64_t T, int64_t D, int32_t nframes,
                     float* out, void* stream);
int abn_stack_frames_batched(const float* feats, const int64_t* utt_frame_off, int64_t n_utts,
                             int64_t T, int64_t D, int32_t nframes, float* out, void* stream);

int64_t abn_mvn_ws_bytes(int64_t T, int64_t D);
int abn_mvn_stats(const float* feats, int64_t T, int64_t D, int per_channel,
                  float* mean, float* stdv, void* ws, void* stream);
int abn_mvn_apply(const float* feats, int64_t T, int64_t D, const float* mean,
                  const float* stdv, int per_channel, float eps, float* out,
                  void* stream);

int abn_fbank(const void* samples, int sample_is_i16, int64_t nsamples,
              int32_t wlen, double fshift, int32_t nfft, int32_t nfilt,
              float alpha, const float* window, const float* melbank, const int32_t* band,
              int64_t nframes, float* out, void* stream);

int abn_fbank_batched(const void* samples, int sample_is_i16, const int64_t* utt_sample_off,
                      const int64_t* utt_frame_off, int64_t n_utts, int32_t wlen, double fshift,
                      int32_t nfft, int32_t nfilt, float alpha, const float* window,
                      const float* melbank, const int32_t* band, int64_t nframes, float* out,
                      void* stream);

int abn_deltas(const float* feats, int64_t T, int64_t D, float* out, void* stream);

int abn_deltas_batched(const float* feats, int64_t ld_in, const int64_t* utt_frame_off, int64_t n_utts,
                       int64_t T, int64_t D, float* out, int64_t ld_out, void* stream);

int abn_mfcc(const void* samples, int sample_is_i16, int64_t nsamples, int32_t wlen, double fshift,
             int32_t nfft, int32_t nfilt, int32_t ncep, float alpha, const float* window,
             const float* melbank, const int32_t* band, const float* dct, int64_t nframes,
             float* out, int64_t ld_out, void* stream);

int abn_mfcc_batched(const void* samples, int sample_is_i16, const int64_t* utt_sample_off,
                     const int64_t* utt_frame_off, int64_t n_utts, int32_t wlen, double fshift,
                     int32_t nfft, int32_t nfilt, int32_t ncep, float alpha, const float* window,
                     const float* melbank, const int32_t* band, const float* dct, int64_t nframes,
                     float* out, int64_t ld_out, void* stream);

enum {
// ... 18 lines not shown
```

Before: 25.67 million frame-pairs/s.

## Fuse forward, cosine loss and dgrad into one step-chain kernel launch

Adds a tower_step_chain kernel path that runs the operand-plane forward of both towers, the cosine loss and the data-gradient chain in a single launch. Weight gradients then follow through the existing wgrad pass. The trainer tries this path first for large enough batches without BatchNorm. It targets launch overhead and the round trips of activations and loss results through global memory between forward, loss and backward. The cost is a more complex kernel with higher LDS use, which may lower occupancy, plus a row-count threshold and a fallback path to keep in sync.

```diff
diff --git a/abnet3_amd/_lib.py b/abnet3_amd/_lib.py
--- a/abnet3_amd/_lib.py
+++ b/abnet3_amd/_lib.py
@@ -7,6 +7,7 @@
 LIB_PATH = os.environ.get('ABNET3_HIP_LIB') or os.path.join(HERE, 'lib', 'libabnet3_hip.so')
 ABI_VERSION = 20
 MAX_LAYERS = 16
+STEP_CHAIN_MIN_ROWS = 3073
 
 ACT = {'none': 0, None: 0, 'sigmoid': 1, 'relu': 2, 'tanh': 3}
 LOSS = {'coscos2': 0, 'cosmargin': 1, 'KLLoss': 2}
@@ -35,6 +36,7 @@
     'abn_tower_backward_launch': (C.c_int, [_vp, _vp, _vp, _vp, _i64, _i64, _vp, _vp, _i64, C.c_int, _vp]),
     'abn_tower_backward_loss_ws_bytes': (_i64, [_i64]),
     'abn_tower_backward_loss': (C.c_int, [_vp, _vp, _vp, _vp, C.c_int, C.c_int, _f32, C.c_int, _i64, _vp, _vp, _i64, _vp, _vp, _vp, _vp, _vp]),
+    'abn_tower_step_chain': (C.c_int, [_vp, _vp, _vp, _vp, C.c_int, C.c_int, _f32, C.c_int, _i64, _i64, _vp, _vp, _i64, _vp, _vp, _vp, _vp, _vp]),
     'abn_tower_reduce_step': (C.c_int, [_vp, _i64, _vp, _i64, C.c_int, _vp, _vp, _vp, _vp, _i64, _f32, _f32, _f32,
                                          _f32, _i64, _f32, _vp]),
     'abn_linear_forward': (C.c_int, [_vp, _vp, _vp, _i64, _i64, _i64, C.c_int, _vp, _vp]),
@@ -173,7 +175,7 @@
 MFCC_GENERAL, MFCC_WAVE512 = 0, 1
 
 trace_paths = False
-last_path = {'forward': -1, 'backward': -1, 'forward_precision': -1, 'backward_precision': -1}
+last_path = {'forward': -1, 'backward': -1, 'forward_precision': -1, 'backward_precision': -1, 'step_chain': False}
 
 
 def note_path(desc, x1, x2, rows, n_calls, train, ws, backward):
diff --git a/abnet3_amd/csrc/tower.hip b/abnet3_amd/csrc/tower.hip
--- a/abnet3_amd/csrc/tower.hip
+++ b/abnet3_amd/csrc/tower.hip
@@ -10,6 +10,7 @@
 #include "opt_rule.h"
 #include "tower_fused.h"
 #include "tower_planes.h"
+#include "tower_step_chain.h"
 #include "tower_bn_persist.h"
 #include "tower_wide.h"
 #include "tower_wgrad_step.h"
@@ -1359,13 +1360,11 @@
     return ABN_OK;
 }
 
-enum { PLANES_BWD_ALL = 0, PLANES_BWD_DGRAD = 1, PLANES_BWD_WGRAD = 2 };
-static int planes_backward(const abn_tower_desc* t, const float* d_out, const LossArgs* loss, int64_t rows, const Layout& L,
-                           const BwdLayout& B, const float* ws, float* scratch, float* dx, hipStream_t st, int part = PLANES_BWD_ALL)
-{
+static PlanesBwdP make_planes_bwd(const abn_tower_desc* t, const float* d_out, const LossArgs* loss, int64_t rows, const Layout& L,
+                                  const BwdLayout& B, const float* ws, float* scratch, float* dx)
+{
+    PlanesBwdP b = {};
     const int nl = t->n_layers;
-    const int np = planes_of(t);
-    PlanesBwdP b = {};
 #ifdef ABN_STAMPS
     b.stamps = getenv("ABN_DSTAMP_BUF") ? (unsigned long long*)strtoull(getenv("ABN_DSTAMP_BUF"), nullptr, 0) : nullptr;
 #endif
@@ -1374,8 +1373,6 @@
     b.d_out = d_out;
     b.d_out_is_dz = t->d_out_is_dz;
     b.tp_steps = pl_row_steps(rows);
-    ABN_REQUIRE((loss || t->wgrad_part == 2 || aligned16(d_out)) && aligned16(scratch) && (!dx || aligned16(dx)),
-                "tower_backward: d_out / scratch / dx must be 16-byte aligned");
     b.loss_kind = -1;
     b.B = (int)rows;
     if (loss) {
@@ -1406,6 +1403,17 @@
         b.amax_dz[l] = B.amax_dz[l] >= 0 ? scratch + B.amax_dz[l] : nullptr;
     }
     b.wbase = image; b.wbytes = PL.bytes;
+    return b;
+}
+
+enum { PLANES_BWD_ALL = 0, PLANES_BWD_DGRAD = 1, PLANES_BWD_WGRAD = 2 };
+static int planes_backward(const abn_tower_desc* t, const float* d_out, const LossArgs* loss, int64_t rows, const Layout& L,
+                           const BwdLayout& B, const float* ws, float* scratch, float* dx, hipStream_t st, int part = PLANES_BWD_ALL)
+{
+    const int np = planes_of(t);
+    ABN_REQUIRE((loss || t->wgrad_part == 2 || aligned16(d_out)) && aligned16(scratch) && (!dx || aligned16(dx)),
+                "tower_backward: d_out / scratch / dx must be 16-byte aligned");
+    const PlanesBwdP b = make_planes_bwd(t, d_out, loss, rows, L, B, ws, scratch, dx);
     int l_first, l_end;
     { const int rc = wgrad_range(t, &l_first, &l_end); if (rc != ABN_OK) return rc; }
     if (t->wgrad_part == 2) part = PLANES_BWD_WGRAD;
@@ -1630,6 +1638,63 @@
     return make_bwd_layout(t, rows).total;
 }
 
+static PlanesFwdP make_planes_fwd(const abn_tower_desc* t, const float* x1, const float* x2, int64_t rows, int64_t rpc, int train, float* ws,
+                                  const Layout& L, PackTable& pk)
+{
+    PlanesFwdP f = {};
+    pk = PackTable{};
+    f.n_layers = t->n_layers;
+    f.rows = (int)rows;
+    f.rows_call = (int)rpc;
+    f.x1 = x1; f.x2 = x2;
+    f.x_copy = nullptr;
+    const PackLayout PL = make_pack_layout(t);
+    char* const image = t->wpack ? reinterpret_cast<char*>(t->wpack) : reinterpret_cast<char*>(ws + L.wpack);
+    pk.base = image;
+    f.wbase = image; f.wbytes = PL.bytes;
+    for (int l = 0; l <= t->n_layers; ++l) f.dims[l] = (int)t->dims[l];
+    for (int l = 0; l < t->n_layers; ++l) {
+        f.act[l] = (l == t->n_layers - 1) ? t->last_act : t->act;
+        f.b[l] = t->b[l];
+        f.mask[l] = train ? t->drop_mask[l] : nullptr;
+        f.out[l] = l == t->n_layers - 1 ? ws + L.a[l] : nullptr;
+        f.wp[l] = image + PL.wp[l];
+        PackJob& J = pk.job[pk.n_jobs++];
+        J.W = t->W[l]; J.N = (int)t->dims[l + 1]; J.K = (int)t->dims[l]; J.transposed = 0;
+        J.nblk = pl_blocks(J.N); J.nsteps = pl_steps(J.K);
+        J.tile0 = pk.n_tiles; J.dst = PL.wp[l];
+        J.blk0 = pk.n_blocks;
+        pk.n_tiles += J.nblk * J.nsteps;
+        pk.n_blocks += J.nblk;
+        {
+            PackJob& T = pk.job[pk.n_jobs++];
+            T.W = t->W[l]; T.N = J.N; T.K = J.K; T.transposed = 1;
+            T.nblk = pl_blocks(T.K); T.nsteps = pl_steps(T.N);
+            T.tile0 = pk.n_tiles; T.dst = PL.wpt[l];
+            T.blk0 = pk.n_blocks;
+            pk.n_tiles += T.nblk * T.nsteps;
+            pk.n_blocks += T.nblk;
+        }
+        f.tp[l] = (t->forward_only || t->batch_norm) ? nullptr : reinterpret_cast<char*>(ws + L.tp[l]);
+        f.amax[l] = f.tp[l] && L.amax[l] >= 0 ? ws + L.amax[l] : nullptr;
+        if (t->batch_norm) { f.bn_rm[l] = t->bn_rm[l]; f.bn_rv[l] = t->bn_rv[l]; f.bn_w[l] = t->bn_w[l]; f.bn_b[l] = t->bn_b[l]; }
+    }
+    f.tp_steps = pl_row_steps(rows);
+    f.drop_seed = train ? reinterpret_cast<const unsigned long long*>(t->drop_seed) : nullptr;
+    f.drop_p = t->drop_p;
+    f.bn_eps = BN_EPS;
+#ifdef ABN_STAMPS
+    f.stamps = getenv("ABN_STAMP_BUF") ? (unsigned long long*)strtoull(getenv("ABN_STAMP_BUF"), nullptr, 0) : nullptr;
+#endif
+    return f;
+}
+static void launch_pack(int np, const PackTable& pk, hipStream_t st)
+{
+    if (np == 3) hipLaunchKernelGGL(pack_planes_kernel<3>, dim3((unsigned)((pk.n_tiles + 3) / 4)), dim3(256), 0, st, pk);
+    else if (np == 2) hipLaunchKernelGGL(pack_planes_scaled_kernel, dim3((unsigned)pk.n_blocks), dim3(PL_NT), 0, st, pk);
+    else hipLaunchKernelGGL(pack_planes_kernel<1>, dim3((unsigned)((pk.n_tiles + 3) / 4)), dim3(256), 0, st, pk);
+}
+
 int abn_tower_forward(const abn_tower_desc* t, const float* x1, const float* x2, int64_t rows,
                       int64_t n_calls, int train, float* ws, void* stream)
 {
@@ -1669,64 +1734,17 @@
     }
     if (bn_train || kind != PLANES_NONE) {
         const int np = planes_of(t);
-        PackTable pk = {};
-        PlanesFwdP f = {};
-        f.n_layers = t->n_layers;
-        f.rows = (int)rows;
-        f.rows_call = (int)rpc;
-        f.x1 = x1; f.x2 = x2;
-        f.x_copy = nullptr;
-        const PackLayout PL = make_pack_layout(t);
+        PackTable pk;
         char* const image = t->wpack ? reinterpret_cast<char*>(t->wpack) : reinterpret_cast<char*>(ws + L.wpack);
         const bool repack = !(t->wpack && t->wpack_valid);
         ABN_REQUIRE(aligned16(image), "tower_forward: wpack must be 16-byte aligned");
-        pk.base = image;
-        f.wbase = image; f.wbytes = PL.bytes;
-        for (int l = 0; l <= t->n_layers; ++l) f.dims[l] = (int)t->dims[l];
-        for (int l = 0; l < t->n_layers; ++l) {
-            f.act[l] = (l == t->n_layers - 1) ? t->last_act : t->act;
-            f.b[l] = t->b[l];
-            f.mask[l] = train ? t->drop_mask[l] : nullptr;
-            f.out[l] = l == t->n_layers - 1 ? ws + L.a[l] : nullptr;
-            f.wp[l] = image + PL.wp[l];
-            PackJob& J = pk.job[pk.n_jobs++];
-            J.W = t->W[l]; J.N = (int)t->dims[l + 1]; J.K = (int)t->dims[l]; J.transposed = 0;
-            J.nblk = pl_blocks(J.N); J.nsteps = pl_steps(J.K);
-            J.tile0 = pk.n_tiles; J.dst = PL.wp[l];
-            J.blk0 = pk.n_blocks;
-            pk.n_tiles += J.nblk * J.nsteps;
-            pk.n_blocks += J.nblk;
-            {
-                PackJob& T = pk.job[pk.n_jobs++];
-                T.W = t->W[l]; T.N = J.N; T.K = J.K; T.transposed = 1;
-                T.nblk = pl_blocks(T.K); T.nsteps = pl_steps(T.N);
-                T.tile0 = pk.n_tiles; T.dst = PL.wpt[l];
-                T.blk0 = pk.n_blocks;
-                pk.n_tiles += T.nblk * T.nsteps;
-                pk.n_blocks += T.nblk;
-            }
-            f.tp[l] = (t->forward_only || t->batch_norm) ? nullptr : reinterpret_cast<char*>(ws + L.tp[l]);
-            f.amax[l] = f.tp[l] && L.amax[l] >= 0 ? ws + L.amax[l] : nullptr;
-            if (t->batch_norm) { f.bn_rm[l] = t->bn_rm[l]; f.bn_rv[l] = t->bn_rv[l]; f.bn_w[l] = t->bn_w[l]; f.bn_b[l] = t->bn_b[l]; }
-        }
-        f.tp_steps = pl_row_steps(rows);
-        f.drop_seed = train ? reinterpret_cast<const unsigned long long*>(t->drop_seed) : nullptr;
-        f.drop_p = t->drop_p;
-        f.bn_eps = BN_EPS;
-#ifdef ABN_STAMPS
-        f.stamps = getenv("ABN_STAMP_BUF") ? (unsigned long long*)strtoull(getenv("ABN_STAMP_BUF"), nullptr, 0) : nullptr;
-#endif
+        PlanesFwdP f = make_planes_fwd(t, x1, x2, rows, rpc, train, ws, L, pk);
         static bool pl_attr_set[16] = {};
         int dev = 0;
         (void)hipGetDevice(&dev);
         dev = (dev >= 0 && dev < 16) ? dev : 0;
-        const dim3 pgrid((unsigned)((pk.n_tiles + 3) / 4));
         const dim3 fgrid((unsigned)((rows + PL_ROWS - 1) / PL_ROWS));
-        if (repack) {
-            if (np == 3) hipLaunchKernelGGL(pack_planes_kernel<3>, pgrid, dim3(256), 0, st, pk);
-            else if (np == 2) hipLaunchKernelGGL(pack_planes_scaled_kernel, dim3((unsigned)pk.n_blocks), dim3(PL_NT), 0, st, pk);
-            else hipLaunchKernelGGL(pack_planes_kernel<1>, pgrid, dim3(256), 0, st, pk);
-        }
+        if (repack) launch_pack(np, pk, st);
         if (!bn_train && kind == PLANES_WIDE) {
             static bool wd_attr_set[16] = {};
             if (!wd_attr_set[dev]) {
@@ -2158,6 +2176,52 @@
     return planes_backward(t, nullptr, &la, rows, L, B, ws, scratch, nullptr, (hipStream_t)stream);
 }
 
+int abn_tower_step_chain(const abn_tower_desc* t, const float* x1, const float* x2, const void* y, int y_dtype, int loss_kind,
+                         float margin, int avg, int64_t rows, int64_t n_calls, float* ws, float* scratch, int64_t scratch_floats,
+                         float* loss_out, void* loss_ws, const int32_t* n_valid, double* loss_accum, void* stream)
+{
+    int rc = check_desc(t, rows, n_calls == 2 ? 2 : 1);
+    if (rc != ABN_OK) return rc;
+    ABN_REQUIRE(x1 && y && ws && scratch && loss_out && loss_ws, "tower_step_chain: null pointer");
+    ABN_REQUIRE(y_dtype >= ABN_Y_I8 && y_dtype <= ABN_Y_F64, "tower_step_chain: unknown label dtype %d", y_dtype);
+    ABN_REQUIRE(loss_kind != ABN_LOSS_COSMARGIN || (margin >= 0.0f && margin <= 1.0f), "tower_step_chain: margin outside [0,1]");
+    for (int l = 0; l < t->n_layers; ++l) ABN_REQUIRE(t->dW[l] && t->db[l], "tower_step_chain: layer %d has null gradient buffers", l);
+    bool forced_masks = false;
+    for (int l = 0; l < t->n_layers; ++l) forced_masks = forced_masks || t->drop_mask[l] != nullptr;
+    const bool ok = (loss_kind == ABN_LOSS_COSCOS2 || loss_kind == ABN_LOSS_COSMARGIN) && n_calls == 2 &&
+                    !t->batch_norm && !t->source && !t->forward_only && (t->wgrad_part == 0 || t->wgrad_part == 1) && !forced_masks && rows >= ABN_STEP_CHAIN_MIN_ROWS &&
+                    rows % PL_ROWS == 0 && t->dims[t->n_layers] % 4 == 0 &&
+                    planes_kind(t, rows, 2, x1, x2, ws, PLANES_TRAIN) == PLANES_CHAIN;
+    if (!ok) {
+        set_error("tower_step_chain: only for the single-launch operand-plane chains of a tower without BatchNorm, two calls of a multiple of "
+                  "16 rows each (%d rows or more in all), the cosine losses, dropout by seed or none: use abn_tower_forward + abn_tower_backward_loss", ABN_STEP_CHAIN_MIN_ROWS);
+        return ABN_E_UNSUPPORTED;
+    }
+    hipStream_t st = (hipStream_t)stream;
+    const Layout L = make_layout(t, rows, 2);
+    const BwdLayout B = make_bwd_layout(t, rows);
+    if (scratch_floats < B.total) { set_error("tower_step_chain: scratch too small"); return ABN_E_WORKSPACE; }
+    const int np = planes_of(t);
+    char* const image = t->wpack ? reinterpret_cast<char*>(t->wpack) : reinterpret_cast<char*>(ws + L.wpack);
+    ABN_REQUIRE(aligned16(image) && aligned16(scratch), "tower_step_chain: wpack / scratch must be 16-byte aligned");
+    PackTable pk;
+    const PlanesFwdP f = make_planes_fwd(t, x1, x2, rows, rows / 2, 1, ws, L, pk);
+    LossArgs la = {y, y_dtype, loss_kind, avg, margin, loss_out, loss_ws, n_valid, loss_accum};
+    const PlanesBwdP b = make_planes_bwd(t, nullptr, &la, rows, L, B, ws, scratch, nullptr);
+    static bool sc_attr_set[16] = {};
+    int dev = 0;
+    (void)hipGetDevice(&dev);
+    dev = (dev >= 0 && dev < 16) ? dev : 0;
+    if (!sc_attr_set[dev]) {
+        PL_LDS_ATTR(tower_step_chain_kernel, step_chain_lds_bytes);
+        sc_attr_set[dev] = true;
+    }
+    if (!(t->wpack && t->wpack_valid)) launch_pack(np, pk, st);
+    PL_LAUNCH(np, tower_step_chain_kernel, dim3((unsigned)(rows / PL_ROWS)), dim3(PL_NT), step_chain_lds_bytes(np), st, f, b);
+    ABN_CHECK_LAUNCH("tower_step_chain");
+    return planes_backward(t, nullptr, &la, rows, L, B, ws, scratch, nullptr, st, PLANES_BWD_WGRAD);
+}
+
 int abn_tower_reduce_step(const abn_tower_desc* t, int64_t rows, const float* scratch, int64_t scratch_floats, int kind,
                           float* params, float* grads, float* state1, float* state2, int64_t n, float lr, float hp0,
                           float hp1, float eps, int64_t step, float grad_scale, void* stream)
diff --git a/abnet3_amd/csrc/tower_planes.h b/abnet3_amd/csrc/tower_planes.h
--- a/abnet3_amd/csrc/tower_planes.h
+++ b/abnet3_amd/csrc/tower_planes.h
@@ -1415,25 +1415,44 @@
     DSTAMP(7 + 4 * (p.n_layers - 1 - l));
 }
 
-template <int NP>
-__global__ __launch_bounds__(PL_NT) void tower_dgrad_planes_kernel(PlanesBwdP p)
-{
-    extern __shared__ __attribute__((aligned(16))) char pl_smem[];
-    char* const img = pl_smem;
-    float* const part = reinterpret_cast<float*>(pl_smem + PL_MAXSTEPS * NP * 1024);
-    const int lane = threadIdx.x & 63;
-    const int wave = __builtin_amdgcn_readfirstlane(threadIdx.x >> 6);
+template <bool PAIRS>
+__device__ __forceinline__ int chain_row(int i, int B)
+{
+    if constexpr (PAIRS) return (i < 16 ? 0 : B - 16) + 16 * (int)blockIdx.x + i;
+    else return (int)blockIdx.x * PL_ROWS + i;
+}
+__device__ __forceinline__ double loss_scale(const PlanesBwdP& p)
+{
+    const int Bv = p.n_valid ? *p.n_valid : p.B;
+    return p.n_valid && p.scale != 1.0 ? 1.0 / (double)(Bv > 0 ? Bv : 1) : p.scale;
+}
+__device__ __forceinline__ void loss_ticket_finish(const PlanesBwdP& p, int lane)
+{
+    double sum = 0.0;
+    for (int i = lane; i < (int)gridDim.x; i += 64) sum += abn_ticket_partial(&p.loss_partial[i]);
+#pragma unroll
+    for (int o = 32; o >= 1; o >>= 1) sum += __shfl_xor(sum, o, 64);
+    if (lane == 0) {
+        const float lv = (float)(sum * loss_scale(p));
+        *p.loss_out = lv;
+        if (p.loss_accum) *p.loss_accum += (double)lv;
+        __hip_atomic_store(p.loss_counter, 0u, __ATOMIC_RELAXED, __HIP_MEMORY_SCOPE_AGENT);
+    }
+}
+__device__ __forceinline__ void loss_ticket_deferred(const PlanesBwdP& p, double sum, int lane)
+{
+    int last = 0;
+    if (lane == 0) last = abn_ticket_publish(&p.loss_partial[blockIdx.x], sum, p.loss_counter, gridDim.x) ? 1 : 0;
+    if (__builtin_amdgcn_readfirstlane(last)) loss_ticket_finish(p, lane);
+}
+
+template <int NP, bool PAIRS>
+__device__ __forceinline__ void planes_dgrad_head(const PlanesBwdP& p, char* __restrict__ img, float* __restrict__ part, const bf16x8* idf,
+                                                  int wave, int lane, float& ainv, double* term_keep)
+{
     const int r = lane & 31, h = lane >> 5;
-    const int row0 = blockIdx.x * PL_ROWS;
     const int top = p.n_layers - 1;
     const int NT = p.dims[top + 1];
-    bf16x8 idf[2];
-    make_identity<NP>(idf, lane);
-#ifdef PL_EXP_PRIO
-    if ((PL_EXP_PRIO == 1) == (wave >= 4)) __builtin_amdgcn_s_setprio(1);
-#endif
-    DSTAMP(0);
-
     double* const coef = reinterpret_cast<double*>(part);
     double* const term_s = coef + 64;
     int* const is_last_s = reinterpret_cast<int*>(term_s + 32);
@@ -1441,11 +1460,11 @@
     if (with_loss) {
         const int B = p.B;
         const int Bv = p.n_valid ? *p.n_valid : B;
-        const double lscale = p.n_valid && p.scale != 1.0 ? 1.0 / (double)(Bv > 0 ? Bv : 1) : p.scale;
+        const double lscale = loss_scale(p);
 #pragma unroll
         for (int it = 0; it < 2; ++it) {
             const int lr = 4 * wave + 2 * it + (lane >> 5), l = lane & 31;
-            const int g = row0 + lr;
+            const int g = chain_row<PAIRS>(lr, B);
             double inv = 0.0, kself = 0.0, term = 0.0;
             const int tower = g < p.rows && g >= B ? 1 : 0, pi_ = g < p.rows ? g - tower * B : 0;
             const bool ok = g < p.rows && pi_ < Bv;
@@ -1502,26 +1521,18 @@
         if (threadIdx.x == 0) {
             double sum = 0.0;
             for (int i = 0; i < 32; ++i) sum += term_s[i];
-            *is_last_s = abn_ticket_publish(&p.loss_partial[blockIdx.x], sum, p.loss_counter, gridDim.x);
-        }
-        __syncthreads();
-        if (*is_last_s && wave == 0) {
-            double sum = 0.0;
-            for (int i = lane; i < (int)gridDim.x; i += 64) sum += abn_ticket_partial(&p.loss_partial[i]);
-#pragma unroll
-            for (int o = 32; o >= 1; o >>= 1) sum += __shfl_xor(sum, o, 64);
-            if (lane == 0) {
-                const float lv = (float)(sum * lscale);
-                *p.loss_out = lv;
-                if (p.loss_accum) *p.loss_accum += (double)lv;
-                __hip_atomic_store(p.loss_counter, 0u, __ATOMIC_RELAXED, __HIP_MEMORY_SCOPE_AGENT);
-            }
+            if constexpr (PAIRS) *term_keep = sum;
+            else *is_last_s = abn_ticket_publish(&p.loss_partial[blockIdx.x], sum, p.loss_counter, gridDim.x);
+        }
+        if constexpr (!PAIRS) {
+            __syncthreads();
+            if (*is_last_s && wave == 0) loss_ticket_finish(p, lane);
         }
     }
 
     DSTAMP(1);
     const int steps_t = pl_steps(NT), blocks_t = steps_t / 2;
-    const int gr = row0 + r;
+    const int gr = chain_row<PAIRS>(r, p.B);
     const bool row_ok = gr < p.rows;
     const float* __restrict__ mask = p.mask[top];
     const DropGen drop_top = make_drop(mask ? nullptr : p.drop_seed, p.drop_p, top);
@@ -1565,7 +1576,7 @@
             }
         }
     };
-    float ainv = 1.0f;
+    ainv = 1.0f;
     if constexpr (NP == 2) {
         float* const sc = part + PL_PART_BYTES / 4;
         f32x4 v[2][2][2];
@@ -1615,6 +1626,26 @@
     }
     __syncthreads();
     DSTAMP(2);
+}
+
+template <int NP>
+__global__ __launch_bounds__(PL_NT) void tower_dgrad_planes_kernel(PlanesBwdP p)
+{
+    extern __shared__ __attribute__((aligned(16))) char pl_smem[];
+    char* const img = pl_smem;
+    float* const part = reinterpret_cast<float*>(pl_smem + PL_MAXSTEPS * NP * 1024);
+    const int lane = threadIdx.x & 63;
+    const int wave = __builtin_amdgcn_readfirstlane(threadIdx.x >> 6);
+    const int row0 = blockIdx.x * PL_ROWS;
+    const int top = p.n_layers - 1;
+    bf16x8 idf[2];
+    make_identity<NP>(idf, lane);
+#ifdef PL_EXP_PRIO
+    if ((PL_EXP_PRIO == 1) == (wave >= 4)) __builtin_amdgcn_s_setprio(1);
+#endif
+    DSTAMP(0);
+    float ainv;
+    planes_dgrad_head<NP, false>(p, img, part, idf, wave, lane, ainv, nullptr);
 
     WeightRing<NP> ring;
     ring_open(ring, p.wbase, p.wbytes);
diff --git a/abnet3_amd/csrc/tower_step_chain.h b/abnet3_amd/csrc/tower_step_chain.h
--- /dev/null
+++ b/abnet3_amd/csrc/tower_step_chain.h
@@ -0,0 +1,73 @@
+#pragma once
+#include <stddef.h>
+
+#include "tower_planes.h"
+
+namespace abn {
+
+static inline size_t step_chain_lds_bytes(int np) { return pl_lds_bytes(np) + 16; }
+
+#ifdef ABN_STAMPS
+#define SCSTAMP(st, slot) do { if ((st) && threadIdx.x == 0) (st)[(size_t)blockIdx.x * 64 + (slot)] = __builtin_amdgcn_s_memtime(); } while (0)
+#else
+#define SCSTAMP(st, slot) do {} while (0)
+#endif
+
+template <class P>
+__device__ __forceinline__ const P& kernarg_block(size_t off)
+{
+    const char __attribute__((address_space(4)))* p = (const char __attribute__((address_space(4)))*)__builtin_amdgcn_kernarg_segment_ptr() + off;
+    asm volatile("" : "+s"(p));
+    return *reinterpret_cast<const P*>((const char*)p);
+}
+
+template <int NP>
+__global__ __launch_bounds__(PL_NT) void tower_step_chain_kernel(PlanesFwdP f_arg, PlanesBwdP b_arg)
+{
+    constexpr size_t B_OFF = (sizeof(PlanesFwdP) + alignof(PlanesBwdP) - 1) / alignof(PlanesBwdP) * alignof(PlanesBwdP);
+    extern __shared__ __attribute__((aligned(16))) char pl_smem[];
+    char* const img = pl_smem;
+    float* const part = reinterpret_cast<float*>(pl_smem + PL_MAXSTEPS * NP * 1024);
+    double* const term_keep = reinterpret_cast<double*>(pl_smem + pl_lds_bytes(NP));
+    const int lane = threadIdx.x & 63;
+    const int wave = __builtin_amdgcn_readfirstlane(threadIdx.x >> 6);
+    const int row0 = chain_row<true>(lane & 31, f_arg.rows_call) - (lane & 31);
+    bf16x8 idf[2];
+    make_identity<NP>(idf, lane);
+#ifdef ABN_STAMPS
+    unsigned long long* const stamps = b_arg.stamps;
+#endif
+    SCSTAMP(stamps, 56);
+
+    float ainv = 1.0f;
+    WeightRing<NP> ring;
+    ring_open(ring, f_arg.wbase, f_arg.wbytes);
+    planes_input_stage<NP, false>(f_arg, img, part, idf, wave, lane, row0, ainv);
+    __syncthreads();
+    for (int l = 0; l < f_arg.n_layers; ++l) {
+        const PlanesFwdP& f = kernarg_block<PlanesFwdP>(0);
+        const int nblk = (f.dims[l + 1] + 31) / 32;
+        if (nblk > PL_WAVES) planes_layer<NP, 2, 1, PL_TRAIN>(f, l, img, part, idf, wave, lane, row0, ainv, ring);
+        else if (nblk > PL_WAVES / 2 || pl_steps(f.dims[l]) % (2 * PL_DEPTH) != 0) planes_layer<NP, 1, 1, PL_TRAIN>(f, l, img, part, idf, wave, lane, row0, ainv, ring);
+        else planes_layer<NP, 1, 2, PL_TRAIN>(f, l, img, part, idf, wave, lane, row0, ainv, ring);
+    }
+    SCSTAMP(stamps, 57);
+    wait_vmcnt<0>();
+    __syncthreads();
+    SCSTAMP(stamps, 58);
+
+    const PlanesBwdP& b = kernarg_block<PlanesBwdP>(B_OFF);
+    planes_dgrad_head<NP, true>(b, img, part, idf, wave, lane, ainv, term_keep);
+    ring_open(ring, b.wbase, b.wbytes);
+    for (int l = b.n_layers - 1; l >= 1; --l) {
+        const int nblk = (b.dims[l] + 31) / 32;
+        if (nblk > PL_WAVES) planes_dgrad_layer<NP, 2, 1>(b, l, img, part, idf, wave, lane, row0, ainv, ring);
+        else if (nblk > PL_WAVES / 2 || pl_steps(b.dims[l + 1]) % (2 * PL_DEPTH) != 0) planes_dgrad_layer<NP, 1, 1>(b, l, img, part, idf, wave, lane, row0, ainv, ring);
+        else planes_dgrad_layer<NP, 1, 2>(b, l, img, part, idf, wave, lane, row0, ainv, ring);
+    }
+    SCSTAMP(stamps, 59);
+    if (b.loss_kind >= 0 && wave == 0) loss_ticket_deferred(b, lane == 0 ? *term_keep : 0.0, lane);
+    SCSTAMP(stamps, 60);
+}
+
+}
diff --git a/abnet3_amd/model.py b/abnet3_amd/model.py
--- a/abnet3_amd/model.py
+++ b/abnet3_amd/model.py
@@ -613,7 +613,7 @@
 
     _HIP_STATE = ('_flat', '_last_grad_flat', '_offsets', '_segs', '_mask_override',
                   '_generation', '_live_cache', '_weights_epoch', '_pending_reduce', '_fused_loss_refused',
-                  '_pending_lower', 'bn_sync', '_bn_sync_agreed')
+                  '_pending_lower', 'bn_sync', '_bn_sync_agreed', '_step_chain_ws', '_step_chain_refused', '_step_chain_probed')
 
     def whoami(self):
         params = {k: v for k, v in self.__dict__.items() if k not in self._HIP_STATE}
@@ -716,6 +716,7 @@
         rows = 2 * x1.shape[0]
         masks = self._draw_dropout_masks(rows, x1.device) if self.training else None
         out, sv = _segment_forward(seg, masks, 2, x1, x2, forward_only=forward_only, n_valid=n_valid, source=source)
+        _lib.last_path['step_chain'] = False
         return out, (seg, sv, _GradPass(self))
 
     def takes_padded_batch_norm(self, x12, npad):
@@ -816,6 +817,76 @@
         return loss
 
     _fused_loss_refused = None
+    _step_chain_refused = None
+    _step_chain_probed = None
+    _step_chain_ws = None
+
+    def direct_step_chain(self, x1, x2, y, loss_kind, margin, avg, defer_reduce=False, n_valid=None, loss_accum=None, loss_ws=None,
+                          wgrad_split=None):
+        if (os.environ.get('ABN_STEP_CHAIN') == '0' or os.environ.get('ABN_LOSS_IN_BACKWARD') == '0'
+                or not self.training or loss_kind not in ('coscos2', 'cosmargin') or self.batch_norm or self._last_act == 'softmax'
+                or self._mask_override is not None or x2 is None or x1.shape[0] % 16 != 0 or 2 * x1.shape[0] < _lib.STEP_CHAIN_MIN_ROWS
+                or self._step_chain_refused == (2 * x1.shape[0], self.precision)):
+            return None
+        p = float(self.p_dropout)
+        if p > 0.0 and os.environ.get('ABN_DROPOUT_IN_KERNEL') == '0':
+            return None
+        seg = self._segment_list()[0]
+        rows = 2 * x1.shape[0]
+        if (not x1.is_cuda or x1.dtype != torch.float32 or x2.dtype != torch.float32 or x1.dim() != 2 or x1.shape[1] != seg.input_dim
+                or x2.shape != x1.shape or y.dtype not in _lib.Y_DTYPE or y.numel() * 2 != rows):
+            return None
+        from .loss import _scratch
+        lib = _lib.load()
+        x1, x2, y = x1.contiguous(), x2.contiguous(), y.contiguous()
+        _lib.require_device(x1, x2, y)
+        key = (rows, self.precision, self._generation)
+        if self._step_chain_probed != key:
+            probe = seg.descriptor(with_grads=False)
+            if lib.abn_tower_path(_lib.C.byref(probe), _lib.ptr(x1), _lib.ptr(x2), rows, 2, 1, _lib.ptr(x1), 0, None) != _lib.PATH_PLANES:
+                return None
+            self._step_chain_probed = key
+        masks = _DropSeed(p, x1.device) if p > 0.0 else None
+        grad_pass = _GradPass(self)
+        grad_buf, grads = grad_pass.views(seg)
+        desc = seg.descriptor(with_grads=True, grad_buf=grad_buf, masks=masks, d_out_is_dz=True, defer_reduce=defer_reduce)
+        if wgrad_split is not None:
+            desc.wgrad_part, desc.wgrad_split = 1, int(wgrad_split)
+        ws_floats = lib.abn_tower_ws_floats(_lib.C.byref(desc), rows, 2)
+        scratch_floats = lib.abn_tower_bwd_scratch_floats(_lib.C.byref(desc), rows)
+        if ws_floats < 0 or scratch_floats < 0:
+            return None
+        ws = torch.empty(max(ws_floats, 1), dtype=torch.float32, device=x1.device)
+        scratch = torch.empty(max(scratch_floats, 1), dtype=torch.float32, device=x1.device)
+        loss = torch.empty((), dtype=torch.float32, device=x1.device)
+        need = lib.abn_tower_backward_loss_ws_bytes(rows)
+        lws = loss_ws if loss_ws is not None and loss_ws.numel() >= need else _scratch(need, x1.device)
+        rc = lib.abn_tower_step_chain(
+            _lib.C.byref(desc), _lib.ptr(x1), _lib.ptr(x2), _lib.ptr(y), _lib.Y_DTYPE[y.dtype], _lib.LOSS[loss_kind], float(margin),
+            int(bool(avg)), rows, 2, _lib.ptr(ws), _lib.ptr(scratch), scratch_floats, _lib.ptr(loss), _lib.ptr(lws), _lib.ptr(n_valid),
+            _lib.ptr(loss_accum), _lib.stream())
+        if rc == _lib.E_UNSUPPORTED:
+            self._step_chain_refused = (rows, self.precision)
+            return None
+        _lib.check(rc, 'abn_tower_step_chain')
+        _lib.note_path(desc, x1, x2, rows, 2, True, ws, backward=False)
+        _lib.note_path(desc, x1, x2, rows, 2, True, ws, backward=True)
+        _lib.last_path['step_chain'] = True
+        if desc.wpack and not desc.wpack_valid and seg._key_at_descriptor is not None:
+            seg.wpack_matches(seg._key_at_descriptor)
+        off = lib.abn_tower_out_offset(_lib.C.byref(desc), rows, 2)
+        emb = ws[off:off + rows * seg.output_dim].view(rows, seg.output_dim)
+        self._pending_reduce = (desc, rows, scratch, scratch_floats, grad_buf, seg) if defer_reduce else None
+        self._pending_lower = None
+        if wgrad_split is not None:
+            sv = _Saved()
+            sv.x1, sv.x2, sv.ws, sv.masks, sv.n_calls, sv.train, sv.rows = x1, x2, ws, masks, 2, True, rows
+            sv.bn_synced, sv.n_valid, sv.source = False, None, None
+            self._pending_lower = (desc, rows, scratch, scratch_floats, sv)
+        self._step_chain_ws = ws
+        for p_, g in zip(seg.params, grads):
+            p_.grad = g
+        return emb, loss
 
     def direct_backward_lower(self):
         desc, rows, scratch, scratch_floats, sv = self._pending_lower
diff --git a/abnet3_amd/trainer.py b/abnet3_amd/trainer.py
--- a/abnet3_amd/trainer.py
+++ b/abnet3_amd/trainer.py
@@ -345,10 +345,29 @@
             X_batch1 = X_batch1.cuda(non_blocking=True)
             X_batch2 = X_batch2.cuda(non_blocking=True)
             y_batch = y_batch.cuda(non_blocking=True)
+            self.optimizer.zero_grad()
+            net = self.network
+            seg_only = (net._segment_list()[0],)
+            split = self._overlap_split(seg_only) if self.dp else None
+            done = net.direct_step_chain(X_batch1, X_batch2, y_batch, type(self.loss).__name__, getattr(self.loss, 'margin', 0.0),
+                                         self.loss.avg, defer_reduce=not self.dp and net.can_defer_reduce(seg_only), wgrad_split=split)
+            if done is not None:
+                if split is not None:
+                    flat = net.flat_grad()
+                    cut = net.grad_split_offset(seg_only, split)
+                    work = [torch.distributed.all_reduce(flat[cut:], op=torch.distributed.ReduceOp.SUM, async_op=True)]
+                    net.direct_backward_lower()
+                    work.append(torch.distributed.all_reduce(flat[:cut], op=torch.distributed.ReduceOp.SUM, async_op=True))
+                    for w in work:
+                        w.wait()
+                    self.optimizer.grad_scale = 1.0 / self.world_size if self._loss_is_mean() else 1.0
+                elif self.dp:
+                    self.optimizer.grad_scale = parallel.all_reduce_gradients(net.flat_grad(), self._loss_is_mean(), self.oneshot)
+                self.optimizer.step()
+                return done[1].detach()
             emb, state = self.network.direct_forward(X_batch1, X_batch2)
             n = X_batch1.shape[0]
             info = self.network.direct_dz_info(state)
-            self.optimizer.zero_grad()
             defer = not self.dp and self.network.can_defer_reduce(state)
             split = self._overlap_split(state) if self.dp else None
             loss_value = self.network.direct_backward_loss(
@@ -538,6 +557,13 @@
         net, opt, npad = self.network, self.optimizer, b['npad']
         x12 = b['x12']
         src = b.get('source')
+        if src is None and hasattr(net, 'direct_step_chain'):
+            opt.zero_grad()
+            done = net.direct_step_chain(x12[:npad], x12[npad:], b['y'], type(self.loss).__name__, getattr(self.loss, 'margin', 0.0),
+                                         self.loss.avg, defer_reduce=not self.dp and net.can_defer_reduce((net._segment_list()[0],)), n_valid=b['nv'],
+                                         loss_accum=self._loss_acc, loss_ws=self._loss_ws)
+            if done is not None:
+                return done[1]
         emb, state = net.direct_forward(x12[:npad], x12[npad:], n_valid=b['nv'] if getattr(net, 'batch_norm', False) else None,
                                         source=src['src'] if src is not None else None)
         opt.zero_grad()
diff --git a/include/abnet3_hip.h b/include/abnet3_hip.h
--- a/include/abnet3_hip.h
+++ b/include/abnet3_hip.h
@@ -132,6 +132,12 @@
                             float* loss_out, void* loss_ws, const int32_t* n_valid,
                             double* loss_accum, void* stream);
 
+#define ABN_STEP_CHAIN_MIN_ROWS 3073
+int abn_tower_step_chain(const abn_tower_desc* t, const float* x1, const float* x2, const void* y,
+                         int y_dtype, int loss_kind, float margin, int avg, int64_t rows, int64_t n_calls,
+                         float* ws, float* scratch, int64_t scratch_floats, float* loss_out,
+                         void* loss_ws, const int32_t* n_valid, double* loss_accum, void* stream);
+
 int abn_tower_reduce_step(const abn_tower_desc* t, int64_t rows, const float* scratch,
                           int64_t scratch_floats, int kind, float* params, float* grads,
                           float* state1, float* state2, int64_t n, float lr, float hp0,
```

Result: faster. 26.29 million frame-pairs/s (median of 6 runs) (+2.4%).
